# IRVLab/so_dso_place_recognition

Hardware: AMD Instinct MI355X
Metric: queries/sec over 100k-signature DB (SC 20x60, z-score fusion, top-1) (higher is better)
Workload: dtype f16x2 (fp32 carried as f16 hi + lo, fp32 accumulate); binary intensity channel: one f16 product per term, rounded to its exact integer count; 1 GPU; sc_match_100k; db_signatures=100000, descriptor=SC 20x60 x 2 channels, mask_width=0, k=1, db_rows_per_gpu=100000

## Files before the change

include/place_recognition.h:

```cpp
#ifndef PLACE_RECOGNITION_H
#define PLACE_RECOGNITION_H

#include <stdint.h>

#ifdef __cplusplus
extern "C" {
#endif

typedef struct pr_ctx pr_ctx;
typedef struct pr_sigset pr_sigset;
typedef struct pr_clouds pr_clouds;
typedef struct pr_bow_vocab pr_bow_vocab;
typedef struct pr_bow_db pr_bow_db;

enum { PR_OK = 0, PR_EINVAL = -1, PR_ENOMEM = -2, PR_EHIP = -3, PR_EIO = -4, PR_ENAN = -5 };
enum { PR_TYPE_SC = 0, PR_TYPE_M2DP = 1, PR_TYPE_DELIGHT = 2, PR_TYPE_GIST = 3, PR_TYPE_BOW = 4 };
enum { PR_ROLE_QUERY = 0, PR_ROLE_DB = 1 };
enum { PR_F64 = 0, PR_F32 = 1, PR_U8 = 2 };
enum { PR_HOST = 0, PR_DEVICE = 1 };
#define PR_F16_DISTANCE_BOUND 2e-3
#define PR_F16_SIGMA_REL 2e-4
#define PR_F16_DIST_ERR 2e-4
#define PR_F32_SIGMA_REL 5e-7
#define PR_F32_DIST_ERR 2e-7
// ... 64 lines not shown
int pr_match_topk(pr_ctx* ctx, int type, const double* h1, int32_t m, const double* h2, int32_t n,
                  int32_t mask_width, double p_weight, int32_t k, int32_t* idx, float* score);
int pr_match_topk_f64(pr_ctx* ctx, int type, const double* h1, int32_t m, const double* h2, int32_t n,
                      int32_t mask_width, double p_weight, int32_t k, int32_t* idx, double* score);

int pr_gist_distance(pr_ctx* ctx, const double* h1, int32_t m, const double* h2, int32_t n, int32_t cols, float* dist);
int pr_bow_distance(pr_ctx* ctx, const double* h1, int32_t m, const double* h2, int32_t n, int32_t cols, float* dist);
int pr_match_topk_cols(pr_ctx* ctx, int type, const double* h1, int32_t m, const double* h2, int32_t n, int32_t cols,
                       int32_t mask_width, int32_t k, int32_t* idx, float* score);

int pr_bow_db_create(pr_ctx* ctx, int32_t max_sigs, int32_t cols, int32_t n_words, int64_t max_postings, pr_bow_db** out);
void pr_bow_db_destroy(pr_ctx* ctx, pr_bow_db* db);
int pr_bow_db_set(pr_ctx* ctx, pr_bow_db* db, const double* rows, int where, int32_t n);
int pr_bow_db_append(pr_ctx* ctx, pr_bow_db* db, const double* rows, int where, int32_t n_new);
int32_t pr_bow_db_count(const pr_bow_db* db);
int pr_bow_match_topk_dev(pr_ctx* ctx, const pr_bow_db* db, const double* q, int32_t m, int32_t q_row0, int32_t db_row0,
                          int32_t mask_width, int32_t k, int32_t* idx, double* score);
int pr_bow_match_topk_f64(pr_ctx* ctx, const double* h1, int32_t m, const double* h2, int32_t n, int32_t cols,
                          int32_t mask_width, int32_t k, int32_t* idx, double* score);
int pr_bow_distance_f64(pr_ctx* ctx, const double* h1, int32_t m, const double* h2, int32_t n, int32_t cols, double* dist);

typedef struct pr_gist_db pr_gist_db;
int pr_gist_db_create(pr_ctx* ctx, int32_t max_sigs, int32_t cols, pr_gist_db** out);
void pr_gist_db_destroy(pr_ctx* ctx, pr_gist_db* db);
int pr_gist_db_set(pr_ctx* ctx, pr_gist_db* db, const double* rows, int where, int32_t n);
int pr_gist_db_append(pr_ctx* ctx, pr_gist_db* db, const double* rows, int where, int32_t n_new);
int32_t pr_gist_db_count(const pr_gist_db* db);
int64_t pr_gist_db_bytes(const pr_gist_db* db);
void pr_gist_db_set_exact(pr_gist_db* db, int on);
int pr_gist_match_topk_dev(pr_ctx* ctx, const pr_gist_db* db, const double* q, int32_t m, int32_t q_row0, int32_t db_row0,
                           int32_t mask_width, int32_t k, int32_t* idx, double* score);
int pr_gist_flagged_count(pr_ctx* ctx, int32_t m, int32_t* count);
int pr_gist_match_topk_f64(pr_ctx* ctx, const double* h1, int32_t m, const double* h2, int32_t n, int32_t cols,
                           int32_t mask_width, int32_t k, int32_t* idx, double* score);
int pr_gist_distance_f64(pr_ctx* ctx, const double* h1, int32_t m, const double* h2, int32_t n, int32_t cols, double* dist);

typedef struct pr_delight_db pr_delight_db;
int pr_delight_db_create(pr_ctx* ctx, int32_t max_sigs, pr_delight_db** out);
void pr_delight_db_destroy(pr_ctx* ctx, pr_delight_db* db);
int pr_delight_db_set(pr_ctx* ctx, pr_delight_db* db, const double* rows, int where, int32_t n);
int pr_delight_db_append(pr_ctx* ctx, pr_delight_db* db, const double* rows, int where, int32_t n_new);
int32_t pr_delight_db_count(const pr_delight_db* db);
int64_t pr_delight_db_bytes(const pr_delight_db* db);
void pr_delight_db_set_exact(pr_delight_db* db, int on);
int pr_delight_match_topk_dev(pr_ctx* ctx, const pr_delight_db* db, const double* q, int32_t m, int32_t q_row0, int32_t db_row0,
                              int32_t mask_width, int32_t k, int32_t* idx, double* score);
int pr_delight_flagged_count(pr_ctx* ctx, int32_t m, int32_t* count);
int pr_delight_match_topk_f64(pr_ctx* ctx, const double* h1, int32_t m, const double* h2, int32_t n, int32_t mask_width, int32_t k,
                              int32_t* idx, double* score);
int pr_delight_distance_f64(pr_ctx* ctx, const double* h1, int32_t m, const double* h2, int32_t n, double* dist);

int pr_match_topk_fused(pr_ctx* ctx, const double* sc1, const double* m2dp1, int32_t m, const double* sc2, const double* m2dp2,
                        int32_t n, int32_t mask_width, double p_weight, int32_t k, int32_t* idx, float* score);
int pr_match_topk_fused_f64(pr_ctx* ctx, const double* sc1, const double* m2dp1, int32_t m, const double* sc2, const double* m2dp2,
                            int32_t n, int32_t mask_width, double p_weight, int32_t k, int32_t* idx, double* score);
int pr_match_align(pr_ctx* ctx, int type, const double* h1, int32_t m, const double* h2, int32_t n, int32_t k, const int32_t* idx,
                   int32_t* variant, double* dist);
int pr_match_align_fused(pr_ctx* ctx, const double* sc1, const double* m2dp1, int32_t m, const double* sc2, const double* m2dp2,
                         int32_t n, int32_t k, const int32_t* idx, int32_t* variant, double* dist);
int pr_fuse_select2_dev(pr_ctx* ctx, const float* d_p, const float* d_i, const float* e_p, const float* e_i, int32_t m, int32_t n,
                        const double* mom_all, const double* mom2_all, int32_t G, int32_t q_row0, int32_t db_row0,
                        int32_t mask_width, double p_weight, int32_t k, int32_t* idx, float* score);


#define PR_MAX_SIGS 4000000
int pr_sigset_create(pr_ctx* ctx, int type, int role, int32_t max_sigs, pr_sigset** out);
void pr_sigset_destroy(pr_ctx* ctx, pr_sigset* s);
int pr_sigset_pack(pr_ctx* ctx, pr_sigset* s, const void* sig, int dtype, int where, int32_t n_sigs);
int32_t pr_sigset_count(const pr_sigset* s);
int pr_sigset_reserve(pr_ctx* ctx, pr_sigset* s);
int pr_sigset_append(pr_ctx* ctx, pr_sigset* s, const void* sig, int dtype, int where, int32_t n_new);
int pr_sigset_image(const pr_sigset* s, const void** image, size_t* bytes, int32_t* channel_stride_groups);

int pr_distances_dev(pr_ctx* ctx, const pr_sigset* q, const pr_sigset* db, float* d_p, float* d_i);

int pr_row_moments_dev(pr_ctx* ctx, const float* d_p, const float* d_i, int32_t m, int32_t n, double* mom);

int pr_fuse_select_dev(pr_ctx* ctx, const float* d_p, const float* d_i, int32_t m, int32_t n,
                       const double* mom_all, int32_t G, int32_t q_row0, int32_t db_row0, int32_t mask_width,
                       double p_weight, int32_t k, int32_t* idx, float* score);
int pr_fuse_select_f64_dev(pr_ctx* ctx, const float* d_p, const float* d_i, int32_t m, int32_t n,
                           const double* mom_all, int32_t G, int32_t q_row0, int32_t db_row0, int32_t mask_width,
                           double p_weight, int32_t k, int32_t* idx, float* score, double* score64);
int pr_fuse_select2_f64_dev(pr_ctx* ctx, const float* d_p, const float* d_i, const float* e_p, const float* e_i, int32_t m, int32_t n,
                            const double* mom_all, const double* mom2_all, int32_t G, int32_t q_row0, int32_t db_row0,
                            int32_t mask_width, double p_weight, int32_t k, int32_t* idx, float* score, double* score64);

int pr_rerank_width(const pr_ctx* ctx, int32_t k);
int pr_f16_margin_dev(pr_ctx* ctx, const double* mom_sc, const double* mom_m2, int32_t m, int32_t G, double p_weight, int32_t k_in,
                      const double* cand_score, int32_t k, const double* score, int32_t* flags, int32_t* count);
int pr_rerank_dev(pr_ctx* ctx, const void* q_sc, const void* db_sc, int sc_dtype, const void* q_m2, const void* db_m2, int m2_dtype,
                  const double* mom_sc, const double* mom_m2, int32_t m, int32_t n_local, int32_t G, int32_t q_row0, int32_t db_row0,
                  int32_t mask_width, double p_weight, int32_t k_in, const int32_t* idx_in, const double* score_in, int32_t k, int32_t* idx,
                  double* score);
int pr_rerank_partial_dev(pr_ctx* ctx, const void* q_sc, const void* db_sc, int sc_dtype, const void* q_m2, const void* db_m2, int m2_dtype,
                          const double* mom_sc, const double* mom_m2, int32_t m, int32_t n_local, int32_t G, int32_t q_row0, int32_t db_row0,
                          int32_t mask_width, double p_weight, int32_t k_in, const int32_t* cand_idx, const double* cand_score, int32_t k,
                          double* p5);
int pr_rerank_finish_dev(pr_ctx* ctx, const double* mom_sc, const double* mom_m2, int32_t G_mom, const int32_t* cand_idx, const double* cand_score,
                         const double* p5_all, int32_t G, int32_t m, int32_t k_in, int32_t k, double p_weight, int32_t* idx, double* score);
int pr_order_resolve_async_dev(pr_ctx* ctx, const void* q_sc, const void* db_sc, int sc_dtype, const void* q_m2, const void* db_m2, int m2_dtype,
                               double* mom_sc, double* mom_m2, int32_t m, int32_t n, int32_t q_row0, int32_t mask_width, double p_weight,
                               int32_t k, int32_t* idx, double* score);
int pr_order_resolve_dev(pr_ctx* ctx, const void* q_sc, const void* db_sc, int sc_dtype, const void* q_m2, const void* db_m2, int m2_dtype,
                         double* mom_sc, double* mom_m2, int32_t m, int32_t n, int32_t q_row0, int32_t mask_width, double p_weight, int32_t k,
                         int32_t* idx, double* score, int32_t* resolved);
int pr_order_flagged_count(pr_ctx* ctx, int32_t m, int32_t* count);
int pr_order_exact_moments_dev(pr_ctx* ctx, const void* q_sc, const void* db_sc, int sc_dtype, const void* q_m2, const void* db_m2, int m2_dtype,
                               const double* mom_sc, const double* mom_m2, int32_t G_mom, int32_t m, int32_t n_local, int32_t offset,
                               int32_t last_pass , double* exact);
int pr_order_exact_select_dev(pr_ctx* ctx, const double* exact_all, int32_t G, int32_t m, int32_t n_local, int32_t q_row0, int32_t db_row0,
                              int32_t mask_width, double p_weight, int has_sc, int has_m2, int32_t k, int32_t offset, double* sel);
int pr_order_exact_merge_dev(pr_ctx* ctx, const double* sel_all, int32_t G, int32_t m, int32_t k, int32_t offset, int32_t* idx, double* score);
int pr_widen_scores_dev(pr_ctx* ctx, const float* score32, int64_t count, double* score64);
int pr_merge_topk_dev(pr_ctx* ctx, const int32_t* idx_all, const double* score_all, int32_t G, int32_t m, int32_t k,
                      int32_t* idx, double* score);
int pr_align_pairs_dev(pr_ctx* ctx, const void* q_sc, const void* db_sc, int sc_dtype, const void* q_m2, const void* db_m2, int m2_dtype,
                       int32_t m, int32_t n_local, int32_t db_row0, int32_t k, const int32_t* idx, int32_t* variant, double* dist);
int pr_delight_align_pairs_dev(pr_ctx* ctx, const void* q, const void* db, int dtype, int32_t m, int32_t n_local, int32_t db_row0, int32_t k,
                               const int32_t* idx, int32_t* variant, double* dist);

typedef struct pr_group pr_group;
int pr_group_create(const int32_t* device_ids, int32_t G, pr_group** out);
void pr_group_destroy(pr_group* g);
const char* pr_group_last_error(const pr_group* g);
int32_t pr_group_size(const pr_group* g);
int pr_group_uses_rccl(const pr_group* g);
int32_t pr_group_rccl_ranks(const pr_group* g);
int pr_group_set_exact_statistics(pr_group* g, int on);
int32_t pr_group_last_flagged(const pr_group* g);
#define PR_GROUP_PHASES 10
int pr_group_set_timing(pr_group* g, int on);
int pr_group_last_timing(pr_group* g, float* ms, int32_t cap);
int pr_group_set_database(pr_group* g, int type, const double* h2, int32_t n);
int pr_group_set_database_growable(pr_group* g, int type, const double* h2, int32_t n, int32_t extra_capacity);
int pr_group_append_database(pr_group* g, const double* hist_new, int32_t n_new);
int32_t pr_group_database_rows(const pr_group* g);
int pr_group_take_warnings(pr_group* g);
int pr_group_match_topk(pr_group* g, const double* h1, int32_t m, int32_t mask_width, double p_weight, int32_t k, int32_t* idx,
                        double* score);

int pr_sc_generate_dev(pr_ctx* ctx, const double* xyz, const float* inten, const int64_t* offs, int32_t N,
                       double max_rho, double* out);
int pr_m2dp_generate_dev(pr_ctx* ctx, const double* xyz, const float* inten, const int64_t* offs, int32_t N,
                         double max_rho, double* out);
int pr_delight_generate_dev(pr_ctx* ctx, const double* xyz, const float* inten, const int64_t* offs, int32_t N, double* out);
int pr_cloud_frames_dev(pr_ctx* ctx, const double* xyz, const float* inten , const int64_t* offs, int32_t N, double* frames);
int pr_sc_generate_frames_dev(pr_ctx* ctx, const double* xyz, const float* inten, const int64_t* offs, int32_t N, double max_rho,
                              const double* frames, int frames_have_ave, double* out);
int pr_m2dp_generate_frames_dev(pr_ctx* ctx, const double* xyz, const float* inten, const int64_t* offs, int32_t N, double max_rho,
                                const double* frames, int frames_have_ave, double* out);
int pr_delight_generate_frames_dev(pr_ctx* ctx, const double* xyz, const float* inten, const int64_t* offs, int32_t N,
                                   const double* frames, double* out);

int pr_sc_relative_pose(const double* frames_q, const double* frames_db, const int32_t* variant, int32_t c, double* T);

int pr_pts_preprocess(const char* poses_file, const char* pts_file, const char* incoming_id_file, double lidarRange,
                      int polar_filter, int verbose, pr_clouds** out);
int pr_pts_preprocess_gpu(pr_ctx* ctx, const char* poses_file, const char* pts_file, const char* incoming_id_file,
                          double lidarRange, int polar, int verbose, pr_clouds** out);
int pr_hash_order(const int32_t* keys, int32_t K, int32_t* order);
int64_t pr_clouds_count(const pr_clouds* c);
const int64_t* pr_clouds_offs(const pr_clouds* c);
const double* pr_clouds_xyz(const pr_clouds* c);
const float* pr_clouds_inten(const pr_clouds* c);
const int32_t* pr_clouds_ids(const pr_clouds* c);
// ... 191 lines not shown
```

so_dso_place_recognition_amd/_lib.py:

```python
from __future__ import annotations

import ctypes as C
import os

PR_OK, PR_EINVAL, PR_ENOMEM, PR_EHIP, PR_EIO, PR_ENAN = 0, -1, -2, -3, -4, -5
TYPE_SC, TYPE_M2DP, TYPE_DELIGHT, TYPE_GIST, TYPE_BOW = 0, 1, 2, 3, 4
SC_ARITH_F16X2, SC_ARITH_F32, SC_ARITH_F16 = 0, 1, 2
NAN_EXCLUDE, NAN_FAIL = 0, 1
WARN_NAN_ROWS, WARN_M2DP_SVD, WARN_F16_FALLBACK, WARN_ORDER_RESOLVED, WARN_ORDER_UNRESOLVED = 1, 2, 4, 8, 16
WARN_BOW_TRUNCATED = 32
WARN_BOW_ROWS = 64
ROLE_QUERY, ROLE_DB = 0, 1
F64, F32 = 0, 1
U8 = 2
HOST, DEVICE = 0, 1
ICP_CONVERGED, ICP_MAX_ITER, ICP_TOO_FEW, ICP_DEGENERATE, ICP_NO_PAIR = 0, 1, 2, 3, 4
ICP_SEARCH_BRUTE, ICP_SEARCH_GRID = 0, 1
POSE_SC, POSE_M2DP, POSE_DELIGHT = 0, 1, 2
WINDOW_OVERFLOW, WINDOW_ORDER_GLOBAL = 1, 2
MAP_OVERFLOW, MAP_DROPPED = 1, 2
ONLINE_OVERFLOW = 1
ONLINE_NB = 512
ONLINESET_FUSED, ONLINESET_DELIGHT = 0, 1
ONLINESET_NB_FUSED, ONLINESET_NB_DELIGHT = 512, 64
# ... 48 lines not shown
    "pr_group_last_flagged": (_i32, [_vp]),
    "pr_group_set_exact_statistics": (C.c_int, [_vp, C.c_int]),
    "pr_group_set_timing": (C.c_int, [_vp, C.c_int]),
    "pr_group_last_timing": (C.c_int, [_vp, _vp, _i32]),
    "pr_group_set_database": (C.c_int, [_vp, C.c_int, _vp, _i32]),
    "pr_group_set_database_growable": (C.c_int, [_vp, C.c_int, _vp, _i32, _i32]),
    "pr_group_append_database": (C.c_int, [_vp, _vp, _i32]),
    "pr_group_database_rows": (_i32, [_vp]),
    "pr_group_take_warnings": (C.c_int, [_vp]),
    "pr_group_match_topk": (C.c_int, [_vp, _vp, _i32, _i32, _dbl, _i32, _vp, _vp]),
    "pr_destroy": (None, [_vp]),
    "pr_last_error": (C.c_char_p, [_vp]),
    "pr_version": (C.c_char_p, []),
    "pr_set_sc_arith": (C.c_int, [_vp, C.c_int]),
    "pr_get_sc_arith": (C.c_int, [_vp]),
    "pr_sync": (C.c_int, [_vp]),
    "pr_stream": (_vp, [_vp]),
    "pr_sc_generate": (C.c_int, [_vp, _vp, _vp, _vp, _i32, _dbl, _vp]),
    "pr_m2dp_generate": (C.c_int, [_vp, _vp, _vp, _vp, _i32, _dbl, _vp]),
    "pr_m2dp_svd_rows": (C.c_int, [_vp, _vp, _i32, _vp]),
    "pr_delight_generate": (C.c_int, [_vp, _vp, _vp, _vp, _i32, _vp]),
    "pr_gist_signature_size": (C.c_int, [_i32, _i32, _vp]),
    "pr_gist_generate": (C.c_int, [_vp, _vp, C.c_int, _i32, _i32, _i32, _i32, _i32, _vp, _vp]),
    "pr_gist_generate_dev": (C.c_int, [_vp, _vp, C.c_int, _i32, _i32, _i32, _i32, _i32, _vp, _vp]),
    "pr_bow_vocab_load": (C.c_int, [C.c_char_p, C.POINTER(_vp)]),
    "pr_bow_vocab_save_bin": (C.c_int, [_vp, C.c_char_p]),
    "pr_bow_vocab_create": (C.c_int, [_i32, _i32, _i32, _i32, C.c_int64, _vp, _vp, _vp, _vp, C.POINTER(_vp)]),
    "pr_bow_vocab_info": (C.c_int, [_vp, _vp, C.POINTER(C.c_int64), C.POINTER(C.c_int64)]),
    "pr_bow_vocab_export": (C.c_int, [_vp, _vp, _vp, _vp, _vp]),
    "pr_bow_vocab_destroy": (None, [_vp]),
    "pr_bow_generate": (C.c_int, [_vp, _vp, _vp, _vp, _i32, _i32, _vp, _vp]),
    "pr_bow_generate_dev": (C.c_int, [_vp, _vp, _vp, C.c_int64, _vp, _i32, _i32, _vp, _vp, _vp]),
    "pr_delight_distance": (C.c_int, [_vp, _vp, _i32, _vp, _i32, _vp]),
    "pr_gist_distance": (C.c_int, [_vp, _vp, _i32, _vp, _i32, _i32, _vp]),
    "pr_bow_distance": (C.c_int, [_vp, _vp, _i32, _vp, _i32, _i32, _vp]),
    "pr_match_topk_fused": (C.c_int, [_vp, _vp, _vp, _i32, _vp, _vp, _i32, _i32, _dbl, _i32, _vp, _vp]),
    "pr_fuse_select2_dev": (C.c_int, [_vp, _vp, _vp, _vp, _vp, _i32, _i32, _vp, _vp, _i32, _i32, _i32, _i32, _dbl, _i32, _vp, _vp]),
    "pr_fuse_select2_f64_dev": (C.c_int, [_vp, _vp, _vp, _vp, _vp, _i32, _i32, _vp, _vp, _i32, _i32, _i32, _i32, _dbl, _i32, _vp, _vp, _vp]),
    "pr_fuse_select_f64_dev": (C.c_int, [_vp, _vp, _vp, _i32, _i32, _vp, _i32, _i32, _i32, _i32, _dbl, _i32, _vp, _vp, _vp]),
    "pr_match_topk_cols": (C.c_int, [_vp, C.c_int, _vp, _i32, _vp, _i32, _i32, _i32, _i32, _vp, _vp]),
    "pr_bow_db_create": (C.c_int, [_vp, _i32, _i32, _i32, C.c_int64, C.POINTER(_vp)]),
    "pr_bow_db_destroy": (None, [_vp, _vp]),
    "pr_bow_db_set": (C.c_int, [_vp, _vp, _vp, C.c_int, _i32]),
    "pr_bow_db_append": (C.c_int, [_vp, _vp, _vp, C.c_int, _i32]),
    "pr_bow_db_count": (_i32, [_vp]),
    "pr_bow_match_topk_dev": (C.c_int, [_vp, _vp, _vp, _i32, _i32, _i32, _i32, _i32, _vp, _vp]),
    "pr_bow_match_topk_f64": (C.c_int, [_vp, _vp, _i32, _vp, _i32, _i32, _i32, _i32, _vp, _vp]),
    "pr_bow_distance_f64": (C.c_int, [_vp, _vp, _i32, _vp, _i32, _i32, _vp]),
    "pr_gist_db_create": (C.c_int, [_vp, _i32, _i32, C.POINTER(_vp)]),
    "pr_gist_db_destroy": (None, [_vp, _vp]),
    "pr_gist_db_set": (C.c_int, [_vp, _vp, _vp, C.c_int, _i32]),
    "pr_gist_db_append": (C.c_int, [_vp, _vp, _vp, C.c_int, _i32]),
    "pr_gist_db_count": (_i32, [_vp]),
    "pr_gist_db_bytes": (C.c_int64, [_vp]),
    "pr_gist_db_set_exact": (None, [_vp, C.c_int]),
    "pr_gist_match_topk_dev": (C.c_int, [_vp, _vp, _vp, _i32, _i32, _i32, _i32, _i32, _vp, _vp]),
    "pr_gist_flagged_count": (C.c_int, [_vp, _i32, C.POINTER(_i32)]),
    "pr_gist_match_topk_f64": (C.c_int, [_vp, _vp, _i32, _vp, _i32, _i32, _i32, _i32, _vp, _vp]),
    "pr_gist_distance_f64": (C.c_int, [_vp, _vp, _i32, _vp, _i32, _i32, _vp]),
    "pr_delight_db_create": (C.c_int, [_vp, _i32, C.POINTER(_vp)]),
    "pr_delight_db_destroy": (None, [_vp, _vp]),
    "pr_delight_db_set": (C.c_int, [_vp, _vp, _vp, C.c_int, _i32]),
    "pr_delight_db_append": (C.c_int, [_vp, _vp, _vp, C.c_int, _i32]),
    "pr_delight_db_count": (_i32, [_vp]),
    "pr_delight_db_bytes": (C.c_int64, [_vp]),
    "pr_delight_db_set_exact": (None, [_vp, C.c_int]),
    "pr_delight_match_topk_dev": (C.c_int, [_vp, _vp, _vp, _i32, _i32, _i32, _i32, _i32, _vp, _vp]),
    "pr_delight_flagged_count": (C.c_int, [_vp, _i32, C.POINTER(_i32)]),
    "pr_delight_match_topk_f64": (C.c_int, [_vp, _vp, _i32, _vp, _i32, _i32, _i32, _vp, _vp]),
    "pr_delight_distance_f64": (C.c_int, [_vp, _vp, _i32, _vp, _i32, _vp]),
    "pr_delight_generate_dev": (C.c_int, [_vp, _vp, _vp, _vp, _i32, _vp]),
    "pr_sc_distance": (C.c_int, [_vp, _vp, _i32, _vp, _i32, _vp, _vp]),
    "pr_m2dp_distance": (C.c_int, [_vp, _vp, _i32, _vp, _i32, _vp, _vp]),
    "pr_match_topk": (C.c_int, [_vp, C.c_int, _vp, _i32, _vp, _i32, _i32, _dbl, _i32, _vp, _vp]),
    "pr_sigset_create": (C.c_int, [_vp, C.c_int, C.c_int, _i32, C.POINTER(_vp)]),
    "pr_sigset_destroy": (None, [_vp, _vp]),
    "pr_sigset_pack": (C.c_int, [_vp, _vp, _vp, C.c_int, C.c_int, _i32]),
    "pr_sigset_count": (_i32, [_vp]),
    "pr_sigset_reserve": (C.c_int, [_vp, _vp]),
    "pr_sigset_append": (C.c_int, [_vp, _vp, _vp, C.c_int, C.c_int, _i32]),
    "pr_sigset_image": (C.c_int, [_vp, C.POINTER(_vp), C.POINTER(C.c_size_t), C.POINTER(_i32)]),
    "pr_distances_dev": (C.c_int, [_vp, _vp, _vp, _vp, _vp]),
    "pr_row_moments_dev": (C.c_int, [_vp, _vp, _vp, _i32, _i32, _vp]),
    "pr_fuse_select_dev": (C.c_int, [_vp, _vp, _vp, _i32, _i32, _vp, _i32, _i32, _i32, _i32, _dbl, _i32, _vp, _vp]),
    "pr_sc_generate_dev": (C.c_int, [_vp, _vp, _vp, _vp, _i32, _dbl, _vp]),
    "pr_m2dp_generate_dev": (C.c_int, [_vp, _vp, _vp, _vp, _i32, _dbl, _vp]),
    "pr_cloud_frames_dev": (C.c_int, [_vp, _vp, _vp, _vp, _i32, _vp]),
    "pr_sc_generate_frames_dev": (C.c_int, [_vp, _vp, _vp, _vp, _i32, _dbl, _vp, C.c_int, _vp]),
    "pr_m2dp_generate_frames_dev": (C.c_int, [_vp, _vp, _vp, _vp, _i32, _dbl, _vp, C.c_int, _vp]),
    "pr_delight_generate_frames_dev": (C.c_int, [_vp, _vp, _vp, _vp, _i32, _vp, _vp]),
    "pr_generate_clouds": (C.c_int, [_vp, C.c_int, _vp, _dbl, _vp]),
    "pr_clouds_dev_xyz": (_vp, [_vp]),
    "pr_clouds_dev_inten": (_vp, [_vp]),
    "pr_clouds_dev_offs": (_vp, [_vp]),
    "pr_clouds_dev_frames": (_vp, [_vp]),
    "pr_pts_preprocess": (C.c_int, [C.c_char_p, C.c_char_p, C.c_char_p, _dbl, C.c_int, C.c_int, C.POINTER(_vp)]),
    "pr_pts_preprocess_gpu": (C.c_int, [_vp, C.c_char_p, C.c_char_p, C.c_char_p, _dbl, C.c_int, C.c_int, C.POINTER(_vp)]),
    "pr_hash_order": (C.c_int, [_vp, _i32, _vp]),
    "pr_window_create": (C.c_int, [_vp, _dbl, C.c_int, _i32, _i32, _i32, C.POINTER(_vp)]),
    "pr_window_destroy": (None, [_vp]),
    "pr_window_reset": (C.c_int, [_vp]),
    "pr_window_count": (C.c_int, [_vp, C.POINTER(_i32)]),
    "pr_window_push_dev": (C.c_int, [_vp, _vp, _vp, _vp, _vp, _i32, _vp, _vp, _vp, _vp, _vp]),
    "pr_window_push": (C.c_int, [_vp, _vp, _vp, _vp, _i32, _vp, _vp, C.POINTER(_i32), _vp, _vp]),
    "pr_clouds_avg_ms": (C.c_double, [_vp]),
    "pr_clouds_avg_pts": (C.c_double, [_vp]),
    "pr_clouds_count": (C.c_int64, [_vp]),
    "pr_clouds_offs": (C.POINTER(C.c_int64), [_vp]),
    "pr_clouds_xyz": (C.POINTER(C.c_double), [_vp]),
    "pr_clouds_inten": (C.POINTER(C.c_float), [_vp]),
    "pr_clouds_ids": (C.POINTER(C.c_int32), [_vp]),
    "pr_clouds_free": (None, [_vp]),
    "pr_write_signatures": (C.c_int, [C.c_char_p, _vp, C.c_int64, C.c_int64]),
    "pr_read_signatures": (C.c_int, [C.c_char_p, C.POINTER(_vp), C.POINTER(C.c_int64), C.POINTER(C.c_int64)]),
    "pr_free": (None, [_vp]),
    "pr_write_signatures_bin": (C.c_int, [C.c_char_p, _vp, C.c_int64, C.c_int64, C.c_int]),
    "pr_read_signatures_bin": (C.c_int, [C.c_char_p, C.POINTER(_vp), C.POINTER(C.c_int64), C.POINTER(C.c_int64)]),
    "pr_write_poses": (C.c_int, [C.c_char_p, _vp, _vp, C.c_int64]),
    "pr_write_points": (C.c_int, [C.c_char_p, _vp, _vp, _vp, C.c_int64]),
    "pr_precision_recall": (C.c_int, [_vp, _vp, _i32, _vp, _vp, _i32, _i32, _dbl, _i32, C.POINTER(_dbl), C.POINTER(_dbl), _vp,
                                      C.POINTER(_i32)]),
    "pr_ground_truth_pairs_dev": (C.c_int, [_vp, _vp, _i32, _vp, _i32, _i32, _dbl, _i32, _vp, _vp, _vp, _vp]),
    "pr_precision_recall_dev": (C.c_int, [_vp, _vp, _vp, _i32, _i32, _vp, _vp, _i32, _i32, _dbl, _i32, _vp, _vp, _vp, _vp, _vp]),
    "pr_trapz_dev": (C.c_int, [_vp, _vp, _vp, _i32, _vp]),
    "pr_ground_truth_pairs": (C.c_int, [_vp, _vp, _i32, _vp, _i32, _i32, _dbl, _i32, _vp, _vp, _vp, _vp]),
    "pr_precision_recall_gpu": (C.c_int, [_vp, _vp, _vp, _i32, _vp, _vp, _i32, _i32, _dbl, _i32, C.POINTER(_dbl), C.POINTER(_dbl), _vp,
                                          C.POINTER(_i32), _vp, C.POINTER(_i32), _vp, _vp]),
    "pr_eval_tile_rows": (_i32, []),
    "pr_set_eval_path": (C.c_int, [_vp, C.c_int, C.c_int]),
    "pr_icp_nn_dev": (C.c_int, [_vp, _vp, _vp, _i32, _vp, _vp, _i32, _vp, _vp, _i32, _vp, _i32, _i32, _vp, _vp, _vp]),
    "pr_icp_pairs_dev": (C.c_int, [_vp, _vp, _vp, _i32, _vp, _vp, _i32, _vp, _vp, _i32, _vp, _i32, _i32, _i32, _dbl, _dbl, _dbl, _i32, _vp, _vp]),
    "pr_icp_nn": (C.c_int, [_vp, _vp, _vp, _i32, _vp, _vp, _i32, _vp, _vp, _i32, _vp, _vp, _vp, _vp]),
    "pr_icp_pairs": (C.c_int, [_vp, _vp, _vp, _i32, _vp, _vp, _i32, _vp, _vp, _i32, _vp, _i32, _dbl, _dbl, _dbl, _i32, _vp, _vp]),
    "pr_icp_tile_rows": (_i32, []),
    "pr_set_icp_path": (C.c_int, [_vp, C.c_int]),
    "pr_set_icp_search": (C.c_int, [_vp, C.c_int]),
    "pr_get_icp_search": (C.c_int, [_vp]),
    "pr_icp_nn_radius_dev": (C.c_int, [_vp, _vp, _vp, _i32, _vp, _vp, _i32, _vp, _vp, _i32, _vp, _i32, _i32, _dbl, _vp, _vp, _vp]),
    "pr_icp_nn_radius": (C.c_int, [_vp, _vp, _vp, _i32, _vp, _vp, _i32, _vp, _vp, _i32, _vp, _dbl, _vp, _vp, _vp]),
    "pr_relative_pose": (C.c_int, [C.c_int, _vp, _vp, _vp, _i32, _vp]),
    "pr_relative_pose_dev": (C.c_int, [_vp, C.c_int, _vp, _i32, _vp, _i32, _i32, _i32, _vp, _vp, _i32, _i32, _vp, _vp, _vp]),
    "pr_verify_select_dev": (C.c_int, [_vp, _vp, _vp, _i32, _i32, _dbl, _dbl, _vp, _vp, _vp, _vp]),
    "pr_verify_pairs_dev": (C.c_int, [_vp, C.c_int, _vp, _vp, _i32, _vp, _vp, _i32, _vp, _vp, _i32, _i32, _i32, _i32, _vp, _vp, _i32, _i32, _i32, _i32,
                                      _i32, _dbl, _dbl, _dbl, _i32, _dbl, _dbl, _vp, _vp, _vp, _vp]),
    "pr_map_create": (C.c_int, [_vp, _vp, _i32, C.c_int64, _i32, _i32, C.POINTER(_vp)]),
    "pr_map_destroy": (None, [_vp]),
    "pr_map_reset": (C.c_int, [_vp]),
    "pr_map_count": (C.c_int, [_vp, C.POINTER(_i32), C.POINTER(C.c_int64), C.POINTER(_i32)]),
    "pr_map_append_dev": (C.c_int, [_vp, _vp, _vp, _vp, _vp, _vp, _vp, _vp, _i32, C.c_int64, _vp]),
    "pr_map_append": (C.c_int, [_vp, _vp, _vp, _vp, _vp, _vp, _vp, _vp, _i32, _vp]),
    "pr_map_verify_dev": (C.c_int, [_vp, C.c_int, _vp, _vp, _i32, _vp, _i32, _i32, _vp, _vp, _i32, _i32, _i32, _i32, _dbl, _dbl, _dbl, _i32, _dbl,
                                    _dbl, _vp, _vp, _vp, _vp]),
    "pr_online_create": (C.c_int, [_vp, C.c_int, _vp, _i32, _i32, C.POINTER(_vp)]),
    "pr_online_destroy": (None, [_vp]),
    "pr_online_reset": (C.c_int, [_vp]),
    "pr_online_count": (C.c_int, [_vp, C.POINTER(_i32), C.POINTER(_i32)]),
    "pr_online_match_dev": (C.c_int, [_vp, _vp, _vp, _i32, _dbl, _i32, _vp, _vp, _vp]),
    "pr_online_append_dev": (C.c_int, [_vp, _vp, _vp, _vp]),
    "pr_online_append": (C.c_int, [_vp, _vp, _vp]),
    "pr_onlineset_create": (C.c_int, [_vp, C.c_int, _vp, _i32, _i32, C.POINTER(_vp)]),
    "pr_onlineset_destroy": (None, [_vp]),
    "pr_onlineset_reset": (C.c_int, [_vp]),
    "pr_onlineset_count": (C.c_int, [_vp, C.POINTER(_i32), C.POINTER(_i32)]),
    "pr_onlineset_match_dev": (C.c_int, [_vp, _vp, _vp, _vp, _vp, _i32, _dbl, _i32, _vp, _vp, _vp]),
    "pr_onlineset_append_dev": (C.c_int, [_vp, _vp, _vp, _vp, _vp, _vp]),
    "pr_onlineset_append": (C.c_int, [_vp, _vp, _vp, _vp, _vp]),
# ... 110 lines not shown
```

so_dso_place_recognition_amd/csrc/fuse_select.hip:

```cpp
#include <cstdlib>

#include "div_rn.hpp"
#include "kernels.hpp"

namespace pr {
namespace {

typedef float f32x4 __attribute__((ext_vector_type(4)));

__device__ __forceinline__ double block_sum(double v, double* red, int tid) {
  red[tid] = v;
  __syncthreads();
  for (int s = 128; s > 0; s >>= 1) {
    if (tid < s) red[tid] += red[tid + s];
    __syncthreads();
  }
  double r = red[0];
  __syncthreads();
  return r;
}

__global__ __launch_bounds__(256) void row_moments_kernel(const float* __restrict__ d_p, const float* __restrict__ d_i,
                                                           int n, double* __restrict__ mom) {
  __shared__ double red[256];
  const int tid = threadIdx.x, q = blockIdx.x;
  for (int ch = 0; ch < 2; ch++) {
    const float* row = (ch ? d_i : d_p) + (size_t)q * n;
    const float r0 = row[0];
    const double c = (r0 == r0) ? (double)r0 : 0.5;
    double s1 = 0.0, s2 = 0.0, cnt = 0.0;
    auto acc = [&](float v) { if (v == v) { const double d = (double)v - c; s1 += d; s2 += d * d; cnt += 1.0; } };
    int head = (int)((4 - ((reinterpret_cast<size_t>(row) >> 2) & 3)) & 3);
    if (head > n) head = n;
    const int nv = (n - head) >> 2;
    if (tid < head) acc(row[tid]);
    const f32x4* rv4 = reinterpret_cast<const f32x4*>(row + head);
    int j = tid;
    for (; j + 768 < nv; j += 1024) {
      const f32x4 a = rv4[j], b = rv4[j + 256], c4 = rv4[j + 512], d4 = rv4[j + 768];
      acc(a[0]); acc(a[1]); acc(a[2]); acc(a[3]);
      acc(b[0]); acc(b[1]); acc(b[2]); acc(b[3]);
      acc(c4[0]); acc(c4[1]); acc(c4[2]); acc(c4[3]);
      acc(d4[0]); acc(d4[1]); acc(d4[2]); acc(d4[3]);
    }
    for (; j < nv; j += 256) { const f32x4 a = rv4[j]; acc(a[0]); acc(a[1]); acc(a[2]); acc(a[3]); }
    for (int t = head + 4 * nv + tid; t < n; t += 256) acc(row[t]);
    const double S1 = block_sum(s1, red, tid);
    const double S2 = block_sum(s2, red, tid);
    const double N = block_sum(cnt, red, tid);
    if (tid == 0) {
      double* o = mom + ((size_t)q * 2 + ch) * 3;
      o[0] = N;
      o[1] = N > 0.0 ? c + S1 / N : 0.0;
      o[2] = N > 0.0 ? S2 - S1 * S1 / N : 0.0;
    }
  }
}

__global__ __launch_bounds__(256) void row_moments_slice_kernel(const float* __restrict__ d_p, const float* __restrict__ d_i, int n, int m, int P,
                                                                 double* __restrict__ part ) {
  __shared__ double red[6][256];
  const int tid = threadIdx.x, q = blockIdx.x, sl = blockIdx.y;
  const int c0 = (int)((long long)n * sl / P), c1 = (int)((long long)n * (sl + 1) / P);
  const float* rp = d_p + (size_t)q * n;
  const float* ri = d_i + (size_t)q * n;
  const float p0 = rp[0], i0 = ri[0];
  const double cp = (p0 == p0) ? (double)p0 : 0.5, ci = (i0 == i0) ? (double)i0 : 0.5;
  double s[6] = {0.0, 0.0, 0.0, 0.0, 0.0, 0.0};
  auto acc = [&](float v, double c, int o) { if (v == v) { const double d = (double)v - c; s[o] += d; s[o + 1] += d * d; s[o + 2] += 1.0; } };
  int j = c0 + tid;
  for (; j + 768 < c1; j += 1024) {
    const float a0 = rp[j], a1 = rp[j + 256], a2 = rp[j + 512], a3 = rp[j + 768];
    const float b0 = ri[j], b1 = ri[j + 256], b2 = ri[j + 512], b3 = ri[j + 768];
    acc(a0, cp, 0); acc(a1, cp, 0); acc(a2, cp, 0); acc(a3, cp, 0);
    acc(b0, ci, 3); acc(b1, ci, 3); acc(b2, ci, 3); acc(b3, ci, 3);
  }
  for (; j < c1; j += 256) { acc(rp[j], cp, 0); acc(ri[j], ci, 3); }
#pragma unroll
  for (int o = 0; o < 6; o++) red[o][tid] = s[o];
  __syncthreads();
  for (int st = 128; st > 0; st >>= 1) {
    if (tid < st) {
#pragma unroll
      for (int o = 0; o < 6; o++) red[o][tid] += red[o][tid + st];
    }
    __syncthreads();
  }
  if (tid < 2) {
    double* o = part + (((size_t)sl * m + q) * 2 + tid) * 3;
    o[0] = red[3 * tid + 2][0]; o[1] = red[3 * tid][0]; o[2] = red[3 * tid + 1][0];
  }
}
__global__ __launch_bounds__(64) void moments_finish_kernel(const float* __restrict__ d_p, const float* __restrict__ d_i, int n, int m, int P,
                                                             const double* __restrict__ part, double* __restrict__ mom) {
  const int t = blockIdx.x * 64 + threadIdx.x;
  if (t >= 2 * m) return;
  const int q = t >> 1, ch = t & 1;
  const float r0 = ((ch ? d_i : d_p) + (size_t)q * n)[0];
  const double c = (r0 == r0) ? (double)r0 : 0.5;
  double N = 0.0, S1 = 0.0, S2 = 0.0;
  const size_t step = (size_t)m * 6;
  const double* o = part + ((size_t)q * 2 + ch) * 3;
  int sl = 0;
  for (; sl + 8 <= P; sl += 8) {
    double a[8][3];
#pragma unroll
    for (int u = 0; u < 8; u++) { a[u][0] = o[(sl + u) * step]; a[u][1] = o[(sl + u) * step + 1]; a[u][2] = o[(sl + u) * step + 2]; }
#pragma unroll
    for (int u = 0; u < 8; u++) { N += a[u][0]; S1 += a[u][1]; S2 += a[u][2]; }
  }
  for (; sl < P; sl++) { N += o[sl * step]; S1 += o[sl * step + 1]; S2 += o[sl * step + 2]; }
  double* w = mom + ((size_t)q * 2 + ch) * 3;
  w[0] = N;
  w[1] = N > 0.0 ? c + S1 / N : 0.0;
  w[2] = N > 0.0 ? S2 - S1 * S1 / N : 0.0;
}

__device__ __forceinline__ bool cand_less(double av, int aj, double bv, int bj) {
  return av < bv || (av == bv && aj < bj);
}

__device__ __forceinline__ void block_argmin(double* rv, int* rj, int tid) {
  double v = rv[tid];
  int j = rj[tid];
#pragma unroll
  for (int s = 32; s > 0; s >>= 1) {
    const double ov = __shfl_xor(v, s, 64);
    const int oj = __shfl_xor(j, s, 64);
    if (oj >= 0 && (j < 0 || cand_less(ov, oj, v, j))) { v = ov; j = oj; }
  }
  __syncthreads();
  if ((tid & 63) == 0) { rv[tid >> 6] = v; rj[tid >> 6] = j; }
  __syncthreads();
  if (tid == 0) {
    for (int w = 1; w < 4; w++) {
      const int oj = rj[w];
      if (oj >= 0 && (j < 0 || cand_less(rv[w], oj, v, j))) { v = rv[w]; j = oj; }
    }
// ... 17 lines not shown
    unsigned long long prefix = 0ull;
    int krem = k, below_total = 0, shd = -1;
    for (int d = 0; d < 8 && shd < 0; d++) {
      const int sh = 56 - 8 * d;
      hist[tid] = 0u;
      __syncthreads();
      for (int s = tid; s < L; s += 256) {
        const unsigned long long key = order_key((double)lv[s]);
        if (d == 0 || (key >> (sh + 8)) == prefix) atomicAdd(&hist[(key >> sh) & 255ull], 1u);
      }
      __syncthreads();
      if (tid < 64) {
        const unsigned c0 = hist[4 * tid], c1 = hist[4 * tid + 1], c2 = hist[4 * tid + 2], c3 = hist[4 * tid + 3];
        const unsigned own = (c0 + c1) + (c2 + c3);
        unsigned incl = own;
#pragma unroll
        for (int o = 1; o < 64; o <<= 1) {
          const unsigned up = __shfl_up(incl, o, 64);
          if (tid >= o) incl += up;
        }
        const unsigned excl = incl - own;
        if (excl < (unsigned)krem && (unsigned)krem <= incl) {
          unsigned b = excl;
          int bin = 4 * tid;
          unsigned cb = c0;
          if (b + c0 < (unsigned)krem) { b += c0; bin++; cb = c1;
            if (b + c1 < (unsigned)krem) { b += c1; bin++; cb = c2;
              if (b + c2 < (unsigned)krem) { b += c2; bin++; cb = c3; } } }
          ctl[0] = bin; ctl[1] = (int)b; ctl[2] = (int)cb;
        }
      }
      __syncthreads();
      prefix = (prefix << 8) | (unsigned long long)ctl[0];
      below_total += ctl[1];
      krem -= ctl[1];
      if (below_total + ctl[2] <= 256) shd = sh;
      __syncthreads();
    }
    if (shd < 0) return false;
    if (tid == 0) ctl[3] = 0;
    __syncthreads();
    for (int s = tid; s < L; s += 256) {
      const double v = (double)lv[s];
      if ((order_key(v) >> shd) <= prefix) {
        const int slot = atomicAdd(&ctl[3], 1);
        rv[slot] = v; rj[slot] = lj[s];
      }
    }
    __syncthreads();
    C = ctl[3];
  } else {
    if (tid < L) { rv[tid] = (double)lv[tid]; rj[tid] = lj[tid]; }
  }
  if (tid >= C) { rv[tid] = __builtin_inf(); rj[tid] = NONE_J; }
  __syncthreads();
  for (int size = 2; size <= 256; size <<= 1)
    for (int stride = size >> 1; stride > 0; stride >>= 1) {
      if (tid < 128) {
        const int pos = 2 * tid - (tid & (stride - 1)), par = pos + stride;
        const bool up = (pos & size) == 0;
        const double a = rv[pos], b = rv[par];
        const int aj = rj[pos], bj = rj[par];
        if (cand_less(b, bj, a, aj) == up) { rv[pos] = b; rj[pos] = bj; rv[par] = a; rj[par] = aj; }
      }
      __syncthreads();
    }
  return true;
}

template <int CAP>
struct SelLds {
  double st[8];
  double rv[256];
  int rj[256];
  double lv[CAP];
  int lj[CAP];
  int lcnt;
  unsigned hist[256];
  int ctl[4];
  double tau_s;
  int last;
};

template <int CAP>
__device__ __forceinline__ void select_row(const float* __restrict__ d_p, const float* __restrict__ d_i,
                                           const float* __restrict__ e_p, const float* __restrict__ e_i,
                                           const double* __restrict__ mom2_all,
                                           int m, int n, const double* __restrict__ mom_all, int G,
                                           int q_row0, int db_row0, int mask_width, double p_weight,
                                           int k, int32_t* __restrict__ idx, float* __restrict__ score, int P,
                                           double* __restrict__ score64, SelLds<CAP>& W) {
  double* st = W.st;
  double* rv = W.rv;
  int* rj = W.rj;
  double* lv = W.lv;
  int* lj = W.lj;
  int& lcnt = W.lcnt;
  unsigned* hist = W.hist;
  int* ctl = W.ctl;
  const int tid = threadIdx.x, q = blockIdx.x;
  const bool plain = (d_i == nullptr);
  const bool two = (e_p != nullptr);
  if (!plain && tid < (two ? 4 : 2)) {
    double cn = 0.0, mean = 0.0, m2 = 0.0;
    for (int g = 0; g < G; g++) {
      const double* o = (tid < 2 ? mom_all : mom2_all) + (((size_t)g * m + q) * 2 + (tid & 1)) * 3;
      const double nb = o[0], mb = o[1], m2b = o[2];
      if (nb <= 0.0) continue;
      const double tot = cn + nb, delta = mb - mean;
      mean += delta * (nb / tot);
      m2 += m2b + delta * delta * (cn * nb / tot);
      cn = tot;
    }
    st[tid * 2] = mean;
    st[tid * 2 + 1] = sqrt(m2 / (cn - 1.0));
  }
  if (tid == 0) lcnt = 0;
  __syncthreads();
  const double mp = plain ? 0.0 : st[0], sp = plain ? 1.0 : st[1], mi = plain ? 0.0 : st[2], si = plain ? 1.0 : st[3];
  const int n_row = n;
  if (P > 1) {
    const int c0 = (int)((long long)n_row * blockIdx.y / P), c1 = (int)((long long)n_row * (blockIdx.y + 1) / P);
    const size_t ro = (size_t)q * n_row + c0;
    d_p += ro - (size_t)q * (c1 - c0);
    if (d_i) d_i += ro - (size_t)q * (c1 - c0);
    if (e_p) { e_p += ro - (size_t)q * (c1 - c0); e_i += ro - (size_t)q * (c1 - c0); }
    db_row0 += c0;
    n = c1 - c0;
    idx += (size_t)blockIdx.y * m * k;
    score += (size_t)blockIdx.y * m * k;
  }
  const float* rp = d_p + (size_t)q * n;
  const float* ri = plain ? rp : d_i + (size_t)q * n;
  const int ig = q_row0 + q;
  const bool fastdiv = !plain && sp > 1e-290 && sp < 1e290 && si > 1e-290 && si < 1e290;
  const double rsp = 1.0 / sp, rsi = 1.0 / si;
  const bool fastdiv2 = two && st[5] > 1e-290 && st[5] < 1e290 && st[7] > 1e-290 && st[7] < 1e290;
  const double m2p = two ? st[4] : 0.0, s2p = two ? st[5] : 1.0, m2i = two ? st[6] : 0.0, s2i = two ? st[7] : 1.0;
  const double rs2p = 1.0 / s2p, rs2i = 1.0 / s2i;
  int head = (int)((4 - ((reinterpret_cast<size_t>(rp) >> 2) & 3)) & 3);
  if (head > n) head = n;
  const bool coaligned = !((reinterpret_cast<size_t>(rp) ^ reinterpret_cast<size_t>(ri)) & 15) &&
                         !(e_p && (((reinterpret_cast<size_t>(rp) ^ reinterpret_cast<size_t>(e_p + (size_t)q * n)) |
                                    (reinterpret_cast<size_t>(rp) ^ reinterpret_cast<size_t>(e_i + (size_t)q * n))) & 15));
  if (!coaligned) head = 0;
  const int nv = coaligned ? (n - head) >> 2 : 0;
  const f32x4* rp4 = reinterpret_cast<const f32x4*>(rp + head);
  const f32x4* ri4 = reinterpret_cast<const f32x4*>(ri + head);

  const float* rep = two ? e_p + (size_t)q * n : rp;
  const float* rei = two ? e_i + (size_t)q * n : rp;
  auto fused4 = [&](float vp, float vi, float wp, float wi, int j) -> double {
    const int jg = db_row0 + j;
    double f;
    if (plain) f = (double)vp;
    else if (fastdiv) f = p_weight * div_rn((double)vp - mp, sp, rsp) + div_rn((double)vi - mi, si, rsi);
    else f = p_weight * (((double)vp - mp) / sp) + ((double)vi - mi) / si;
    if (two) {
      const double xp = (double)wp - m2p, xi = (double)wi - m2i;
      f += fastdiv2 ? p_weight * div_rn(xp, s2p, rs2p) + div_rn(xi, s2i, rs2i) : p_weight * (xp / s2p) + xi / s2i;
    }
    int dij = ig - jg;
    if (dij < 0) dij = -dij;
    if (dij < mask_width) f = __builtin_inf();
    return f;
  };
  auto fused = [&](float vp, float vi, int j) -> double { return fused4(vp, vi, two ? rep[j] : 0.f, two ? rei[j] : 0.f, j); };
  const f32x4* ep4 = reinterpret_cast<const f32x4*>(rep + head);
  const f32x4* ei4 = reinterpret_cast<const f32x4*>(rei + head);
  auto sweep_if = [&](auto&& maybe, auto&& visit) {
    if (tid < head && maybe(rp[tid], ri[tid], two ? rep[tid] : 0.f, two ? rei[tid] : 0.f)) visit(tid, fused(rp[tid], ri[tid], tid));
    const f32x4 z4 = {0.f, 0.f, 0.f, 0.f};
    auto four = [&](const f32x4& a, const f32x4& b, const f32x4& c, const f32x4& d, int j) {
      const int j0 = head + 4 * j;
#pragma unroll
      for (int e = 0; e < 4; e++)
        if (maybe(a[e], b[e], c[e], d[e])) visit(j0 + e, fused4(a[e], b[e], c[e], d[e], j0 + e));
    };
    int j = tid;
    if (two) {
      for (; j + 768 < nv; j += 1024) {
        const f32x4 a0 = rp4[j], a1 = rp4[j + 256], a2 = rp4[j + 512], a3 = rp4[j + 768];
        const f32x4 b0 = ri4[j], b1 = ri4[j + 256], b2 = ri4[j + 512], b3 = ri4[j + 768];
        const f32x4 c0 = ep4[j], c1 = ep4[j + 256], c2 = ep4[j + 512], c3 = ep4[j + 768];
        const f32x4 d0 = ei4[j], d1 = ei4[j + 256], d2 = ei4[j + 512], d3 = ei4[j + 768];
        four(a0, b0, c0, d0, j); four(a1, b1, c1, d1, j + 256); four(a2, b2, c2, d2, j + 512); four(a3, b3, c3, d3, j + 768);
// ... 45 lines not shown
    double mv = 0.0;
    int mj = -1;
    const int r = k + 7 > 16 ? k + 7 : 16;
    long long want = (long long)n * r / 1024;
    const int ns = (int)(want < 4096 ? (n < 4096 ? n : 4096) : (want < n ? want : n));
    auto take = [&](float vp, float vi, int j) {
      const double f = fused(vp, vi, j);
      const int jg = db_row0 + j;
      if (f == f && (mj < 0 || cand_less(f, jg, mv, mj))) { mv = f; mj = jg; }
    };
    int j = tid;
    for (; j + 768 < ns; j += 1024) {
      const float p0 = rp[j], p1 = rp[j + 256], p2 = rp[j + 512], p3 = rp[j + 768];
      const float i0 = ri[j], i1 = ri[j + 256], i2 = ri[j + 512], i3 = ri[j + 768];
      take(p0, i0, j); take(p1, i1, j + 256); take(p2, i2, j + 512); take(p3, i3, j + 768);
    }
    for (; j < ns; j += 256) take(rp[j], ri[j], j);
    rv[tid] = mv; rj[tid] = mj;
    __syncthreads();
    int before = 0;
    for (int u = 0; u < 256; u++) {
      const int oj = rj[u];
      if (oj >= 0 && (mj < 0 || cand_less(rv[u], oj, mv, mj))) before++;
    }
    if (tid == 0) W.tau_s = __builtin_inf();
    __syncthreads();
    if (mj >= 0 && before == r - 1) W.tau_s = mv;
    __syncthreads();
    tau = W.tau_s;
  }
  const bool whole = n <= CAP && !(tau < __builtin_inf());
  if (whole)
    sweep([&](int j, double f) {
      const bool ok = f == f;
      lv[j] = ok ? f : __builtin_inf();
      lj[j] = ok ? db_row0 + j : NONE_J;
    });
  else {
    const bool pre = !plain && fastdiv && (!two || fastdiv2) && tau < __builtin_inf();
    const double a1 = p_weight / sp, b1 = 1.0 / si, c1 = -(p_weight * mp / sp + mi / si);
    const double a2 = two ? p_weight / s2p : 0.0, b2 = two ? 1.0 / s2i : 0.0, c2 = two ? -(p_weight * m2p / s2p + m2i / s2i) : 0.0;
    const double tauE = tau + 1e-10 * (1.0 + fabs(a1) + fabs(b1) + fabs(c1) + fabs(a2) + fabs(b2) + fabs(c2) + fabs(tau));
    auto collect = [&](int j, double f) {
      if (f <= tau) {
        const int slot = atomicAdd(&lcnt, 1);
        if (slot < CAP) { lv[slot] = f; lj[slot] = db_row0 + j; }
      }
    };
    if (pre)
      sweep_if([&](float vp, float vi, float wp, float wi) {
        double fa = __builtin_fma(a1, (double)vp, __builtin_fma(b1, (double)vi, c1));
        if (two) fa += __builtin_fma(a2, (double)wp, __builtin_fma(b2, (double)wi, c2));
        return fa <= tauE;
      }, collect);
    else
      sweep(collect);
  }
  __syncthreads();
  const int L = whole ? n : lcnt;
  if (L <= CAP && (k > 12 || whole)) {
    if (k <= 249 && list_topk(lv, lj, L, k, rv, rj, hist, ctl, tid)) {
      for (int t = tid; t < k; t += 256) emit(t, rv[t], rj[t] == NONE_J ? -1 : rj[t]);
      return;
    }
    int N = 2;
    while (N < L) N <<= 1;
    for (int s = L + tid; s < N; s += 256) { lv[s] = __builtin_inf(); lj[s] = NONE_J; }
    __syncthreads();
    for (int size = 2; size <= N; size <<= 1)
      for (int stride = size >> 1; stride > 0; stride >>= 1) {
        for (int i = tid; i < (N >> 1); i += 256) {
          const int pos = 2 * i - (i & (stride - 1)), par = pos + stride;
          const bool up = (pos & size) == 0;
          const double a = lv[pos], b = lv[par];
          const int aj = lj[pos], bj2 = lj[par];
          if (cand_less(b, bj2, a, aj) == up) { lv[pos] = b; lj[pos] = bj2; lv[par] = a; lj[par] = aj; }
        }
        __syncthreads();
      }
    for (int t = tid; t < k; t += 256) emit(t, lv[t < L ? t : 0], (t < L && lj[t] != NONE_J) ? lj[t] : -1);
    return;
  }
  if (L <= CAP) {
    for (int t = 0; t < k; t++) {
      double cv = 0.0;
      int cj = -1, cs = -1;
      for (int s = tid; s < L; s += 256)
        if (lj[s] >= 0 && (cj < 0 || cand_less(lv[s], lj[s], cv, cj))) { cv = lv[s]; cj = lj[s]; cs = s; }
      rv[tid] = cv; rj[tid] = cj;
      block_argmin(rv, rj, tid);
      const double wv = rv[0];
      const int wj = rj[0];
      __syncthreads();
      if (cs >= 0 && cj == wj) lj[cs] = -1;
      if (tid == 0) emit(t, wv, wj);
      if (wj < 0) {
        if (tid == 0) for (int u = t + 1; u < k; u++) emit(u, 0.0, -1);
        break;
      }
      __syncthreads();
    }
    return;
  }
  double pv = -__builtin_inf(), bv = 0.0;
  int pj = -1, bj = -1;
  for (int t = 0; t < k; t++) {
    bv = 0.0; bj = -1;
    sweep([&](int j, double f) {
      const int jg = db_row0 + j;
      if (f != f) return;
      if (!cand_less(pv, pj, f, jg)) return;
      if (bj < 0 || cand_less(f, jg, bv, bj)) { bv = f; bj = jg; }
    });
    rv[tid] = bv; rj[tid] = bj;
    block_argmin(rv, rj, tid);
    pv = rv[0];
    pj = rj[0];
    __syncthreads();
    if (tid == 0) emit(t, pv, pj);
    if (pj < 0) {
      if (tid == 0) for (int u = t + 1; u < k; u++) emit(u, 0.0, -1);
      break;
    }
  }
}

constexpr int WS_CAP = 1024;
__device__ __forceinline__ void wave_argmin(double& v, int& j) {
#pragma unroll
  for (int s2 = 32; s2 > 0; s2 >>= 1) {
    const double ov = __shfl_xor(v, s2, 64);
    const int oj = __shfl_xor(j, s2, 64);
    if (oj >= 0 && (j < 0 || cand_less(ov, oj, v, j))) { v = ov; j = oj; }
  }
}
__global__ __launch_bounds__(256) void fuse_select_wave_kernel(const float* __restrict__ d_p, const float* __restrict__ d_i, int m, int n,
                                                                const double* __restrict__ mom_all, int G, int q_row0, int db_row0,
                                                                int mask_width, double p_weight, int k, int32_t* __restrict__ idx,
                                                                float* __restrict__ score, double* __restrict__ score64) {
  __shared__ double lv_[4][WS_CAP];
  __shared__ int lj_[4][WS_CAP];
  const int lane = threadIdx.x & 63, w = threadIdx.x >> 6;
  const int q = blockIdx.x * 4 + w;
  if (q >= m) return;
  double* lv = lv_[w];
  int* lj = lj_[w];
  const bool plain = (d_i == nullptr);
  double st0 = 0.0, st1 = 1.0;
  if (!plain && lane < 2) {
    double cn = 0.0, mean = 0.0, m2 = 0.0;
    for (int g = 0; g < G; g++) {
      const double* o = mom_all + (((size_t)g * m + q) * 2 + lane) * 3;
      const double nb = o[0], mb = o[1], m2b = o[2];
      if (nb <= 0.0) continue;
      const double tot = cn + nb, delta = mb - mean;
      mean += delta * (nb / tot);
      m2 += m2b + delta * delta * (cn * nb / tot);
      cn = tot;
    }
    st0 = mean;
    st1 = sqrt(m2 / (cn - 1.0));
  }
  const double mp = plain ? 0.0 : __shfl(st0, 0, 64), sp = plain ? 1.0 : __shfl(st1, 0, 64);
  const double mi = plain ? 0.0 : __shfl(st0, 1, 64), si = plain ? 1.0 : __shfl(st1, 1, 64);
  const float* rp = d_p + (size_t)q * n;
  const float* ri = plain ? rp : d_i + (size_t)q * n;
  const int ig = q_row0 + q;
  const bool fastdiv = !plain && sp > 1e-290 && sp < 1e290 && si > 1e-290 && si < 1e290;
  const double rsp = 1.0 / sp, rsi = 1.0 / si;
  auto fusedw = [&](float vp, float vi, int j) -> double {
    const int jg = db_row0 + j;
    double f;
    if (plain) f = (double)vp;
    else if (fastdiv) f = p_weight * div_rn((double)vp - mp, sp, rsp) + div_rn((double)vi - mi, si, rsi);
    else f = p_weight * (((double)vp - mp) / sp) + ((double)vi - mi) / si;
    int dij = ig - jg;
    if (dij < 0) dij = -dij;
    if (dij < mask_width) f = __builtin_inf();
    return f;
  };
  auto emit = [&](int t, double v, int jg) {
    idx[(size_t)q * k + t] = jg;
    const float f32 = (jg >= 0) ? (float)v : __builtin_nanf("");
    score[(size_t)q * k + t] = f32;
// ... 105 lines not shown
    });
    wave_argmin(bv, bj);
    if (lane == 0) emit(t, bv, bj);
    if (bj < 0) {
      if (lane == 0) for (int u = t + 1; u < k; u++) emit(u, 0.0, -1);
      break;
    }
    pv = bv; pj = bj;
  }
}

__device__ void merge_slices(const int32_t* sidx, const float* sscore, int P, int m, int k, int q, float* lv, int* lj, double* rv, int* rj,
                             unsigned* hist, int* ctl, int32_t* __restrict__ idx, float* __restrict__ score, double* __restrict__ score64,
                             int tid) {
  const int T = P * k;
  int N = 2;
  while (N < T) N <<= 1;
  for (int s = tid; s < N; s += 256) {
    int j = -1;
    float v = 0.f;
    if (s < T) {
      const size_t o = ((size_t)(s / k) * m + q) * k + (s % k);
      j = sidx[o]; v = sscore[o];
    }
    const bool ok = j >= 0 && v == v;
    lv[s] = ok ? v : __builtin_inff();
    lj[s] = ok ? j : NONE_J;
  }
  __syncthreads();
  auto put = [&](int t, bool ok, float v, int j) {
    idx[(size_t)q * k + t] = ok ? j : -1;
    const float f32 = ok ? v : __builtin_nanf("");
    score[(size_t)q * k + t] = f32;
    if (score64) score64[(size_t)q * k + t] = (double)f32;
  };
  if (k <= 249 && list_topk(lv, lj, T, k, rv, rj, hist, ctl, tid)) {
    for (int t = tid; t < k; t += 256) put(t, rj[t] != NONE_J, (float)rv[t], rj[t]);
    return;
  }
  for (int size = 2; size <= N; size <<= 1)
    for (int stride = size >> 1; stride > 0; stride >>= 1) {
      for (int i = tid; i < (N >> 1); i += 256) {
        const int pos = 2 * i - (i & (stride - 1)), par = pos + stride;
        const bool up = (pos & size) == 0;
        const float a = lv[pos], b = lv[par];
        const int aj = lj[pos], bj = lj[par];
        if (cand_less((double)b, bj, (double)a, aj) == up) { lv[pos] = b; lj[pos] = bj; lv[par] = a; lj[par] = aj; }
      }
      __syncthreads();
    }
  for (int t = tid; t < k; t += 256) put(t, lj[t] != NONE_J, lv[t], lj[t]);
}

__global__ __launch_bounds__(256) void slice_merge_kernel(const int32_t* __restrict__ sidx, const float* __restrict__ sscore, int P, int m, int k,
                                                           int32_t* __restrict__ idx, float* __restrict__ score, double* __restrict__ score64) {
  extern __shared__ __attribute__((aligned(8))) char smem[];
  int N = 2;
  while (N < P * k) N <<= 1;
  __shared__ double rv[256];
  __shared__ int rj[256];
  __shared__ unsigned hist[256];
  __shared__ int ctl[4];
  merge_slices(sidx, sscore, P, m, k, blockIdx.x, reinterpret_cast<float*>(smem), reinterpret_cast<int*>(smem) + N, rv, rj, hist, ctl, idx, score,
                      score64, threadIdx.x);
}

template <int CAP>
#ifdef FS_NOLB
#define FS_BOUNDS __launch_bounds__(256)
#else
#define FS_BOUNDS __launch_bounds__(256, 3)
#endif
__global__ FS_BOUNDS void fuse_select_kernel(const float* __restrict__ d_p, const float* __restrict__ d_i,
                                                           const float* __restrict__ e_p, const float* __restrict__ e_i,
                                                           const double* __restrict__ mom2_all,
                                                           int m, int n, const double* __restrict__ mom_all, int G,
                                                           int q_row0, int db_row0, int mask_width, double p_weight,
                                                           int k, int32_t* __restrict__ idx, float* __restrict__ score, int P,
                                                           double* __restrict__ score64) {
  __shared__ SelLds<CAP> L;
  select_row<CAP>(d_p, d_i, e_p, e_i, mom2_all, m, n, mom_all, G, q_row0, db_row0, mask_width, p_weight, k, idx, score, P, score64, L);
}

}

int select_slices(int m, int n) {
  if (m > 64 || n < 16384) return 1;
  static const int forced = getenv("PR_SLICE_COLS") ? atoi(getenv("PR_SLICE_COLS")) : 0;
  const int cols = forced > 0 ? forced : (m <= 8 ? FS_CAP / 2 : FS_CAP);
  int P = (n + cols - 1) / cols;
  if (P > 64) P = 64;
  while (P > 1 && m * P > 1024) P >>= 1;
  return P;
}
size_t select_scratch_bytes() { return (size_t)64 * 16 * 128 * 8 + (size_t)64 * 16 * 6 * 8; }

void launch_row_moments(hipStream_t st, const float* d_p, const float* d_i, int m, int n, double* mom, void* scratch) {
  if (m <= 0) return;
  const int P = scratch ? select_slices(m, n) : 1;
  if (P > 1) {
    double* part = reinterpret_cast<double*>(static_cast<char*>(scratch) + (size_t)64 * 16 * 128 * 8);
    hipLaunchKernelGGL(row_moments_slice_kernel, dim3(m, P), dim3(256), 0, st, d_p, d_i, n, m, P, part);
    hipLaunchKernelGGL(moments_finish_kernel, dim3((2 * m + 63) / 64), dim3(64), 0, st, d_p, d_i, n, m, P, part, mom);
    return;
  }
  hipLaunchKernelGGL(row_moments_kernel, dim3(m), dim3(256), 0, st, d_p, d_i, n, mom);
}

void launch_fuse_select(hipStream_t st, const float* d_p, const float* d_i, int m, int n, const double* mom_all,
                        int G, int q_row0, int db_row0, int mask_width, double p_weight, int k, int32_t* idx,
                        float* score, const float* e_p, const float* e_i, const double* mom2_all, void* scratch, double* score64) {
  if (m <= 0) return;
  int P = (scratch && k <= 128) ? select_slices(m, n) : 1;
  if ((size_t)P * m * k > (size_t)64 * 16 * 128) P = 1;
  if (P > 1) {
    int32_t* sidx = static_cast<int32_t*>(scratch);
    float* ssc = reinterpret_cast<float*>(sidx + (size_t)64 * 16 * 128);
    int N = 2;
    while (N < P * k) N <<= 1;
    hipLaunchKernelGGL(fuse_select_kernel<FS_CAP>, dim3(m, P), dim3(256), 0, st, d_p, d_i, e_p, e_i, mom2_all, m, n, mom_all, G, q_row0, db_row0,
                       mask_width, p_weight, k, sidx, ssc, P, nullptr);
    if ((size_t)N * 8 > 40 * 1024)
      (void)hipFuncSetAttribute(reinterpret_cast<const void*>(slice_merge_kernel), hipFuncAttributeMaxDynamicSharedMemorySize, (int)((size_t)N * 8));
    hipLaunchKernelGGL(slice_merge_kernel, dim3(m), dim3(256), (size_t)N * 8, st, sidx, ssc, P, m, k, idx, score, score64);
    return;
  }
  static const bool wave_rows = !(getenv("PR_SELECT_WAVE") && atoi(getenv("PR_SELECT_WAVE")) == 0);
  static const int wave_max_n = getenv("PR_SELECT_WAVE_N") ? atoi(getenv("PR_SELECT_WAVE_N")) : 32768;
  if (wave_rows && !e_p && n <= wave_max_n && k <= 16 && m >= 64) {
    hipLaunchKernelGGL(fuse_select_wave_kernel, dim3((m + 3) / 4), dim3(256), 0, st, d_p, d_i, m, n, mom_all, G, q_row0, db_row0, mask_width,
                       p_weight, k, idx, score, score64);
    return;
  }
  hipLaunchKernelGGL(fuse_select_kernel<FS_CAP>, dim3(m), dim3(256), 0, st, d_p, d_i, e_p, e_i, mom2_all, m, n, mom_all, G, q_row0, db_row0,
                     mask_width, p_weight, k, idx, score, 1, score64);
}

}
```

so_dso_place_recognition_amd/csrc/kernels.hpp:

```cpp
#pragma once
#include <hip/hip_runtime.h>
#include <stdint.h>

struct pr_ctx;

namespace pr {

constexpr int SC_NF = 31;
constexpr int SC_NSLOT = 16;
constexpr int SC_QIMG = SC_NF * 320;
constexpr int SC_DSTEP = 640;
constexpr int SC_DIMG = 2 * SC_NSLOT * SC_DSTEP;
__host__ __device__ inline int sc_fpos(int f) { return f == 0 ? 0 : (f == 30 ? 1 : f + 1); }
constexpr int SCH_QROW = 80;
constexpr int SCH_QBLK = 16 * SCH_QROW;
constexpr int SCH_QIMG = SC_NF * SCH_QBLK;
__host__ __device__ constexpr int sch_qrow_pos(int row) { return (int)((0xedbafc9865327410ull >> (4 * row)) & 15); }
__host__ __device__ constexpr int sch_qrow_byte(int row) { return SCH_QROW * sch_qrow_pos(row); }
static_assert(SCH_QROW % 16 == 0 && SCH_QBLK % 16 == 0 && SCH_QIMG % 16 == 0, "ds_read_b128 needs 16-byte aligned query tiles");
constexpr int SCH_DTILE = 768;
constexpr int SCH_DFREQ = 4 * SCH_DTILE;
constexpr int SCH_DIMG = SC_NF * SCH_DFREQ;
__host__ __device__ constexpr int sch_qlo_byte(int ring) { return 40 + ((ring + 4) % 20) * 2; }
__host__ __device__ constexpr int sch_a1_byte(int k) { return k == 3 ? 0 : 16 * k; }
__host__ __device__ constexpr int sch_a2_byte(int k) { return k == 0 ? 48 : k == 1 ? 64 : k == 2 ? 32 : 16; }
__host__ __device__ constexpr int sch_b1_byte(int lane) { return lane < 48 ? lane * 16 : SCH_DTILE + (lane - 48) * 16; }
__host__ __device__ constexpr int sch_b2_byte(int lane) { return lane < 32 ? lane * 16 : lane < 48 ? SCH_DTILE + lane * 16 : SCH_DTILE + (lane - 32) * 16; }
constexpr int SCF_QBLK = 640;
constexpr int SCF_QIMG = SC_NF * SCF_QBLK;
constexpr int SCF_DFREQ = 2 * SCH_DTILE;
constexpr int SCF_DIMG = SC_NF * SCF_DFREQ;
constexpr int M2_TILE = 96 * 64;

inline int sc_qgroups8(int m) { return ((m + 31) / 32) * 4; }
inline int sc_qgroups8_f16(int m) { return ((m + 63) / 64) * 8; }
inline int sc_dgroups(int n) { return (n + 15) / 16; }
inline int m2_tiles(int sigs) { return (sigs + 7) / 8; }
inline int m2_qtiles(int sigs) { return ((m2_tiles(sigs) + 11) / 12) * 12; }

constexpr int SC_BSTAT_INTS = 8;
struct ScBin {
  const int* qstat; const int* dstat;
  const float* qinfo; const float* dinfo;
  int* viol;
  int gen;
  float bconst;
  float pair_scale;
  int gate;
  int chsel;
};
#ifdef __HIPCC__
__device__ __forceinline__ bool sc_bin_bound(const ScBin& b, float& bound) {
  const int q0 = b.qstat[0], q1 = b.qstat[1], d0 = b.dstat[0], d1 = b.dstat[1];
  const float eq = __builtin_sqrtf(((__int_as_float(b.qstat[2]) + __int_as_float(b.qstat[3])) + __int_as_float(b.qstat[4])) + __int_as_float(b.qstat[5]));
  const float ed = __builtin_sqrtf(((__int_as_float(b.dstat[2]) + __int_as_float(b.dstat[3])) + __int_as_float(b.dstat[4])) + __int_as_float(b.dstat[5]));
  bound = (eq + ed + eq * ed + b.bconst * (1.f + eq) * (1.f + ed)) * 1.001f;
  return q0 == 0 && d0 == 0 && bound * __builtin_sqrtf((float)q1 * (float)d1) < 0.72f;
}
#endif
void launch_sc_pack(hipStream_t st, const void* sig, int dtype, int rows, int role, float* packed, int groups,
                    const double* twiddle, int* flags, int* bad);
void launch_sc_match(hipStream_t st, const float* qpk, int m, const float* dpk, int n, const float* cst,
                     float* d_p, float* d_i, int nsplit_override);
size_t sc_match_lds_bytes();
void launch_zero_ints(hipStream_t st, int* p, int n);
void launch_fill_ints(hipStream_t st, int* p, int n, int v);
void launch_sc_pack_h(hipStream_t st, const void* sig, int dtype, int rows, int role, void* packed, int groups,
                      const double* twiddle, int* flags, int* bad, int single = 0,
                      float* binfo = nullptr, int* bstat = nullptr);
void launch_sc_pack_h_rows(hipStream_t st, const void* sig, int dtype, int rows, int row0, void* packed, int groups, const double* twiddle,
                           int* flags, int* bad, int single, float* binfo, int* bstat);
void launch_sc_match_h(hipStream_t st, const void* qpk, int m, const void* dpk, int n, const void* cst, float* d_p,
                       float* d_i, int nsplit_override, const struct ScBin* bin = nullptr);
size_t sc_match_h_lds_bytes();
void launch_sc_match_e(hipStream_t st, const void* qpk, int m, const void* dpk, int n, const void* cst, float* d_p, float* d_i,
                       int nsplit_override, int single, int dgs = 0 );
void launch_sc_match_e_bin(hipStream_t st, const void* qpk, int m, const void* dpk, int n, const void* cst, float* d_p, float* d_i,
                           int nsplit_override, ScBin bin, hipEvent_t* ev, int online_h = 0 , int dgs = 0 );

void launch_m2dp_pack(hipStream_t st, const void* sig, int dtype, int sigs, float* packed, int tiles);
void launch_m2dp_match(hipStream_t st, const float* qpk, int m, const float* dpk, int n, float* d_p, float* d_i);
void launch_m2dp_pack_h(hipStream_t st, const void* sig, int dtype, int sigs, void* packed, int tiles, int sg0 = 0 );
void launch_m2dp_match_h(hipStream_t st, const void* qpk, int m, const void* dpk, int n, float* d_p, float* d_i, int single = 0 ,
                         int dts = 0 );

size_t select_scratch_bytes();
void launch_row_moments(hipStream_t st, const float* d_p, const float* d_i, int m, int n, double* mom, void* scratch = nullptr);
void launch_fuse_select(hipStream_t st, const float* d_p, const float* d_i, int m, int n, const double* mom_all,
                        int G, int q_row0, int db_row0, int mask_width, double p_weight, int k, int32_t* idx,
                        float* score, const float* e_p = nullptr, const float* e_i = nullptr, const double* mom2_all = nullptr, void* scratch = nullptr,
                        double* score64 = nullptr );

void launch_nan_fixup(hipStream_t st, float* d_p, float* d_i, int m, int n, const int* qbad, const int* dbad);
void launch_rerank(hipStream_t st, const void* q_sc, const void* db_sc, int sc_dt, const void* q_m2, const void* db_m2, int m2_dt,
                   const double* mom_sc, const double* mom_m2, int m, int n_local, int G, int q_row0, int db_row0, int mask_width,
                   double p_weight, int kin, const int32_t* idx_in, double* p5, unsigned* tick , size_t tick_cap , int k, int32_t* idx, double* score,
                   float* score32, const double* cand_sc32, double eps_d = 0.0, double order_floor = 0.0,
                   double order_noise = 0.0, int32_t* order_flags = nullptr);
void launch_rerank_partial(hipStream_t st, const void* q_sc, const void* db_sc, int sc_dt, const void* q_m2, const void* db_m2, int m2_dt,
                           const double* mom_sc, const double* mom_m2, int m, int n_local, int G, int q_row0, int db_row0, int mask_width,
                           double p_weight, int kin, const int32_t* idx_in, double* p5, unsigned* tick, size_t tick_cap, const double* cand_sc32, int k,
                           double eps_d = 0.0);
void launch_margin_check(hipStream_t st, const double* mom_sc, const double* mom_m2, int G, int m, double p_weight, int kin,
                         const double* cand_sc, int k, const double* score, double eps_d, int32_t* flags, int32_t* count,
                         const int32_t* order_flags, double eps_floor, double noise );
void launch_order_check(hipStream_t st, const double* mom_sc, const double* mom_m2, int Gmom, const int32_t* cand_idx, const double* p5_all,
                        int G, int m, int kin, int k, const int32_t* idx_sel, double p_weight, double eps_floor, double noise, int32_t* flags,
                        const double* cand_sc = nullptr, const double* score_sel = nullptr);
constexpr int RESOLVE_SLOTS = 64;
constexpr int RESOLVE_NB = 2048;
constexpr int RESOLVE_SMALL_M = 1024;
int exact_partial_blocks(int n_local);
void launch_flag_compact(hipStream_t st, const int32_t* flags, int m, int32_t* list, int32_t* cnt);
void launch_xrow(hipStream_t st, const void* q_sc, const void* db_sc, int sc_dt, const void* q_m2, const void* db_m2, int m2_dt,
                 const double* mom_sc, const double* mom_m2, int G, int m, int n_local, const int32_t* flags, int32_t* list, int32_t* cnt,
                 int offset, bool compacted, double* partial, double* exact, double* rows, unsigned* tick, int* dflags,
                 int last_pass , double* qspec , const double* tw ,
                 int direct );
size_t xrow_qspec_doubles();
hipError_t xrow_set_twiddles(const double* cos60, const double* sin60);
void launch_xrow_select(hipStream_t st, const int32_t* flags, const int32_t* list, const int32_t* cnt, int offset, const double* exact_all, int G,
                        int m, int n_local, int q_row0, int db_row0, int mask_width, double p_weight, int has_sc, int has_m2, int k,
                        const double* rows, double* part , double* sel, int32_t* idx,
                        double* score, double* out_mom_sc, double* out_mom_m2);
size_t xrow_select_part_doubles(int m, int k);
void launch_xrow_merge(hipStream_t st, const int32_t* flags, const int32_t* list, const int32_t* cnt, int offset, const double* sel_all, int G, int m,
                       int k, int32_t* idx, double* score);
void launch_rerank_finish(hipStream_t st, const int32_t* cand_idx, const double* p5_all, int G, int m, int kin, int k, int32_t* idx,
                          double* score);
void launch_widen(hipStream_t st, const float* a, long long n, double* b);
void launch_merge_topk(hipStream_t st, const int32_t* idx_all, const double* score_all, int G, int m, int k, int32_t* idx, double* score);

void launch_align(hipStream_t st, const void* q_sc, const void* db_sc, int sc_dt, const void* q_m2, const void* db_m2, int m2_dt, int m,
                  int n_local, int db_row0, int k, const int32_t* idx, int32_t* variant , double* dist );
void launch_delight_align(hipStream_t st, const void* q, const void* db, int dt, int m, int n_local, int db_row0, int k, const int32_t* idx,
                          int32_t* variant , double* dist );

void launch_ave_chain(hipStream_t st, const float* inten, const int64_t* offs, int N, float* ave ,
                      double* frames = nullptr );
void launch_cloud_frames(hipStream_t st, const double* xyz, const int64_t* offs, int N, double* frames);
constexpr int SC_MAX_W = 16;
constexpr int SC_MAX_SPLIT_CLOUDS = 1024;
constexpr size_t SC_SCRATCH_PER_STREAM = (size_t)2 * SC_MAX_SPLIT_CLOUDS * 4 + (size_t)SC_MAX_SPLIT_CLOUDS * SC_MAX_W * 9 * 8 +
                                         (size_t)768 * (1200 * 4 + 3 * 1200 * 8);
size_t sc_generate_scratch_bytes();
void launch_sc_batch(hipStream_t st, const double* xyz, const float* inten, const int64_t* offs, int c0, int c1, int W, double max_rho,
                     double* frames, char* scratch, double* out);
size_t sc_cluster_scratch_bytes(int ncl, int CW);
int sc_cluster_points_per_workgroup();
int* launch_sc_cluster(hipStream_t st, const double* xyz, const float* inten, const int64_t* offs, int N, double max_rho, int CW, int ncu,
                       char* scratch, double* frames, double* out);
void launch_sc_finish(hipStream_t st, const float* ave, int N, double* out);
void launch_sc_bin(hipStream_t st, const double* xyz, const float* inten, const int64_t* offs, int N, double max_rho,
                   const double* frames, const float* ave , double* out,
                   int ave_in_frames = 0 );
void launch_m2dp_bin_svd(hipStream_t st, const double* xyz, const float* inten, const int64_t* offs, int N,
                         double max_rho, const double* frames, const float* ave, const double* planes, double* mats,
                         double* out, int* flags ,
                         int* svd_rows ,
                         hipStream_t st2 = nullptr, hipEvent_t* ev_bin = nullptr, hipEvent_t* ev_svd = nullptr );
constexpr int M2DP_SVD_ROWS_CAP = 1024;
constexpr double M2DP_SVD_TIE_TRACE = 1.001;
size_t m2dp_generate_scratch_bytes(int N);

void launch_gist_distance(hipStream_t st, const double* h1, int m, const double* h2, int n, int cols, float* dist);
void launch_bow_distance(hipStream_t st, const double* h1, int m, const double* h2, int n, int cols, float* dist);
void launch_delight_gen(hipStream_t st, const double* xyz, const float* inten, const int64_t* offs, int N,
                        const double* frames, double* out);
void launch_delight_pack(hipStream_t st, const void* sig, int dtype, int sigs, float* packed, unsigned* mask);
void launch_delight_match(hipStream_t st, const float* q, int m, const float* db, const unsigned* dbmask, int n, float* dist);
constexpr int GIST_LD = 272;
constexpr int GIST_PAIRS = 128;
size_t gist_scratch_floats(int chunk, int nf, int nb);
void launch_gist(hipStream_t st, const void* img, bool u8, int n, int nb, int nf, const float* circ, const float* gabor,
// ... 196 lines not shown
```

so_dso_place_recognition_amd/csrc/pr_api.cpp:

```cpp
#include <hip/hip_runtime.h>

#include <cmath>
#include <algorithm>
#include <cstdio>
#include <cstdlib>
#include <cstring>
#include <new>
#include <string>
#include <type_traits>
#include <vector>

#include "../../include/place_recognition.h"
#include "../../include/pr_m2dp_table.h"
#include "kernels.hpp"
#include "hash_order.hpp"
#include "records.hpp"
#include <chrono>
#include <unordered_map>

struct pr_ctx {
  int device = -1;
  hipStream_t stream = nullptr;
  bool own_stream = true;
  int nan_policy = PR_NAN_EXCLUDE;
  int warnings = 0;
  hipStream_t side = nullptr;
  hipStream_t side2 = nullptr;
  hipEvent_t ev_b = nullptr;
  char* sc_scratch = nullptr;
  void* sel_scratch = nullptr;
  double* rr_scratch = nullptr;
  size_t rr_cap = 0;
  hipEvent_t ev_fork = nullptr, ev_join = nullptr;
  hipEvent_t ev_m2[4] = {nullptr, nullptr, nullptr, nullptr};
  std::string err;
  int* d_svd_rows = nullptr;
  int* d_flags = nullptr;
  bool sc_online_h = false;
  double* d_twiddle = nullptr;
  float* d_cst = nullptr;
  int32_t* d_margin = nullptr;
  int32_t* d_order = nullptr;
  size_t order_cap = 0;
  int32_t order_m = -1;
  unsigned* rr_tick = nullptr;
  size_t tick_cap = 0;
  double* res_partial = nullptr;
  double* res_exact = nullptr;
  size_t res_exact_cap = 0;
  double* xrows = nullptr;
  size_t xrows_cap = 0;
  double* xqspec = nullptr;
  double* xpart = nullptr;
  size_t xpart_cap = 0;
  bool xrow_direct = false;
  void* d_cst_h = nullptr;
  int sc_kernel = 2;
  int sc_mode = PR_SC_ARITH_F16X2;
  double* d_planes = nullptr;
  int sc_nsplit = 0;
  bool force_order = false;
  bool sc_binary = true;
  float sc_bconst = 0.f;
  int bin_gen = 0;
  float sc_pair_scale = 1.f;
  bool timing = false;
  hipEvent_t ev_t[4] = {nullptr, nullptr, nullptr, nullptr};
  int timing_valid = 0;
  void* gist = nullptr;
  void* bow = nullptr;
  void* eval = nullptr;
  void* icp = nullptr;
  void* pose = nullptr;
};

struct pr_sigset {
  int type = 0, role = 0;
  int32_t max_sigs = 0, count = 0;
  int groups = 0;
  int sc_mode = 0;
  float* packed = nullptr;
  size_t floats = 0;
  int* bad = nullptr;
  float* binfo = nullptr;
  int32_t hw = 0;
  int packed_groups = -1;
  bool cap_geom = false;
};

static thread_local std::string g_err;

#define PR_FAIL(ctx, code, ...)                                   \
  do {                                                            \
    char _b[512];                                                 \
    snprintf(_b, sizeof _b, __VA_ARGS__);                         \
    if (ctx) (ctx)->err = _b; else g_err = _b;                    \
    return (code);                                                \
  } while (0)

#define PR_HIP(ctx, call)                                                                     \
  do {                                                                                        \
    hipError_t _e = (call);                                                                   \
    if (_e != hipSuccess) PR_FAIL(ctx, (_e == hipErrorOutOfMemory ? PR_ENOMEM : PR_EHIP),     \
                                  "%s failed: %s", #call, hipGetErrorString(_e));            \
  } while (0)

namespace {

thread_local pr_ctx* g_scope_ctx = nullptr;
struct DevScope {
  pr_ctx* prev;
  explicit DevScope(pr_ctx* c) : prev(g_scope_ctx) { g_scope_ctx = c; }
  ~DevScope() { g_scope_ctx = prev; }
// ... 35 lines not shown
    *groups = pr::sc_dgroups(max_sigs);
    return (size_t)(2 * *groups + 9) * pr::SCF_DIMG / 4;
  }
  if (type == PR_TYPE_SC && sc_mode == 0) {
    if (role == PR_ROLE_QUERY) { *groups = pr::sc_qgroups8(max_sigs); return (size_t)2 * *groups * pr::SCH_QIMG / 4; }
    *groups = pr::sc_dgroups(max_sigs);
    return (size_t)(2 * *groups + 9) * pr::SCH_DIMG / 4;
  }
  if (type == PR_TYPE_SC) {
    if (role == PR_ROLE_QUERY) { *groups = pr::sc_qgroups8(max_sigs); return (size_t)2 * *groups * pr::SC_QIMG; }
    *groups = pr::sc_dgroups(max_sigs);
    return (size_t)2 * *groups * pr::SC_DIMG + 16 * pr::SC_DSTEP;
  }
  if (role == PR_ROLE_QUERY) { *groups = pr::m2_qtiles(max_sigs); return (size_t)2 * *groups * pr::M2_TILE; }
  *groups = pr::m2_tiles(max_sigs);
  return (size_t)(2 * *groups + 16) * pr::M2_TILE;
}

int check_flags(pr_ctx* ctx) {
  int h[7];
  PR_HIP(ctx, hipMemcpyAsync(h, ctx->d_flags, sizeof h, hipMemcpyDeviceToHost, ctx->stream));
  PR_HIP(ctx, hipStreamSynchronize(ctx->stream));
  if (h[0] || h[1] || h[2] || h[3]) PR_HIP(ctx, hipMemsetAsync(ctx->d_flags, 0, 4 * sizeof(int), ctx->stream));
  if (h[5]) {
    PR_HIP(ctx, hipMemsetAsync(ctx->d_flags + 5, 0, sizeof(int), ctx->stream));
    ctx->warnings |= PR_WARN_BOW_TRUNCATED;
  }
  if (h[6]) {
    PR_HIP(ctx, hipMemsetAsync(ctx->d_flags + 6, 0, sizeof(int), ctx->stream));
    ctx->warnings |= PR_WARN_BOW_ROWS;
  }
  if (h[1]) ctx->warnings |= PR_WARN_M2DP_SVD;
  if (h[2]) ctx->warnings |= PR_WARN_ORDER_RESOLVED;
  if (h[3]) ctx->warnings |= PR_WARN_ORDER_UNRESOLVED;
  if (h[0]) {
    if (ctx->nan_policy == PR_NAN_FAIL)
      PR_FAIL(ctx, PR_ENAN, "a signature row has zero L2 norm (MATLAB would produce NaN distances, processSC.m:16,19)");
    ctx->warnings |= PR_WARN_NAN_ROWS;
  }
  return PR_OK;
}

}

extern "C" {

const char* pr_version(void) { return "so_dso_place_recognition_amd 0.1 (gfx950)"; }

const char* pr_last_error(const pr_ctx* ctx) { return ctx ? ctx->err.c_str() : g_err.c_str(); }

static int create_common(int device_id, hipStream_t external, bool use_external, pr_ctx** out) {
  if (!out) PR_FAIL((pr_ctx*)nullptr, PR_EINVAL, "pr_create: out is NULL");
  *out = nullptr;
  int ndev = 0;
  hipError_t e = hipGetDeviceCount(&ndev);
  if (e != hipSuccess || ndev <= 0)
    PR_FAIL((pr_ctx*)nullptr, PR_EHIP, "pr_create: no HIP device available (%s); this library has no CPU fallback",
            e == hipSuccess ? "device count is 0" : hipGetErrorString(e));
  if (device_id < 0 || device_id >= ndev) PR_FAIL((pr_ctx*)nullptr, PR_EINVAL, "pr_create: device %d out of range [0,%d)", device_id, ndev);
  hipDeviceProp_t prop;
  PR_HIP((pr_ctx*)nullptr, hipGetDeviceProperties(&prop, device_id));
  if (strncmp(prop.gcnArchName, "gfx950", 6) != 0)
    PR_FAIL((pr_ctx*)nullptr, PR_EHIP, "pr_create: device %d is %s, this library is built for gfx950 only", device_id, prop.gcnArchName);
  pr_ctx* ctx = new (std::nothrow) pr_ctx;
  if (!ctx) PR_FAIL((pr_ctx*)nullptr, PR_ENOMEM, "pr_create: out of host memory");
  ctx->device = device_id;
  int rc = PR_OK;
  do {
#define TRY(call) if ((call) != hipSuccess) { g_err = std::string(#call) + " failed"; rc = PR_EHIP; break; }
    TRY(hipSetDevice(device_id));
    if (use_external) { ctx->stream = external; ctx->own_stream = false; }
    else TRY(hipStreamCreateWithFlags(&ctx->stream, hipStreamNonBlocking));
    {
      int plo = 0, phi = 0;
      TRY(hipDeviceGetStreamPriorityRange(&plo, &phi));
      TRY(hipStreamCreateWithPriority(&ctx->side, hipStreamNonBlocking, phi));
    }
    TRY(hipStreamCreateWithFlags(&ctx->side2, hipStreamNonBlocking));
    TRY(hipEventCreateWithFlags(&ctx->ev_b, hipEventDisableTiming));
    TRY(hipEventCreateWithFlags(&ctx->ev_fork, hipEventDisableTiming));
    TRY(hipEventCreateWithFlags(&ctx->ev_join, hipEventDisableTiming));
    for (auto& e : ctx->ev_m2) TRY(hipEventCreateWithFlags(&e, hipEventDisableTiming));
    TRY(hipMalloc(&ctx->sel_scratch, pr::select_scratch_bytes()));
    TRY(hipMalloc((void**)&ctx->d_flags, 8 * sizeof(int)));
    TRY(hipMemset(ctx->d_flags, 0, 8 * sizeof(int)));
    TRY(hipMalloc((void**)&ctx->d_svd_rows, (1 + pr::M2DP_SVD_ROWS_CAP) * sizeof(int)));
    TRY(hipMemset(ctx->d_svd_rows, 0, (1 + pr::M2DP_SVD_ROWS_CAP) * sizeof(int)));
    double tw[120 + 4 * 60 * 8];
    for (int t = 0; t < 60; t++) { tw[t] = std::cos(2.0 * M_PI * t / 60.0); tw[60 + t] = std::sin(2.0 * M_PI * t / 60.0); }
    tw[0] = 1; tw[15] = 0; tw[30] = -1; tw[45] = 0; tw[60] = 0; tw[75] = 1; tw[90] = 0; tw[105] = -1;
    for (int fb = 0; fb < 4; fb++)
      for (int sct = 0; sct < 60; sct++)
        for (int j = 0; j < 4; j++) {
          const int t = ((4 * fb + j) * sct) % 60;
          tw[120 + ((fb * 60 + sct) * 4 + j) * 2] = tw[t];
          tw[120 + ((fb * 60 + sct) * 4 + j) * 2 + 1] = tw[60 + t];
        }
    TRY(hipMalloc((void**)&ctx->d_twiddle, sizeof tw));
    TRY(hipMemcpy(ctx->d_twiddle, tw, sizeof tw, hipMemcpyHostToDevice));
    TRY(pr::xrow_set_twiddles(tw, tw + 60));
    std::vector<float> cst((size_t)pr::SC_NSLOT * 128);
    for (int sl = 0; sl < pr::SC_NSLOT; sl++)
      for (int l = 0; l < 64; l++) {
        const int half = l >> 5;
        int k = l & 31; if (k > 30) k = 0;
        const int f = (sl == 0) ? (half ? 30 : 0) : (sl == pr::SC_NSLOT - 1 ? 29 : 2 * sl - 1 + half);
        const int t = (f * k) % 60;
        const double w = (f == 0 || f == 30) ? 1.0 : 2.0;
        float ce = (float)(w * tw[t]), co = (float)(-w * tw[60 + t]);
        if (sl == pr::SC_NSLOT - 1) { if (half) ce = 0.f; else co = 0.f; }
        cst[(size_t)sl * 128 + l] = ce;
        cst[(size_t)sl * 128 + 64 + l] = co;
      }
    TRY(hipMalloc((void**)&ctx->d_cst, cst.size() * sizeof(float)));
    TRY(hipMemcpy(ctx->d_cst, cst.data(), cst.size() * sizeof(float), hipMemcpyHostToDevice));
    {
      std::vector<_Float16> ch((size_t)8 * 64 * 8);
      for (int eo = 0; eo < 2; eo++)
        for (int half = 0; half < 2; half++)
          for (int l = 0; l < 64; l++)
            for (int e = 0; e < 8; e++) {
              int k = l & 31; if (k > 30) k = 30;
              const int f = 16 * half + 8 * (l >> 5) + e;
              double v = 0.0;
              if (f < pr::SC_NF) {
                const int t = (f * k) % 60;
                const double w = (f == 0 || f == 30) ? 1.0 : 2.0;
                v = (eo == 0 ? w * tw[t] : -w * tw[60 + t]) * 1024.0;
              }
              const _Float16 hi = (_Float16)v;
              const _Float16 lo = (_Float16)(v - (double)hi);
              ch[((((size_t)eo * 2 + half) * 2 + 0) * 64 + l) * 8 + e] = hi;
              ch[((((size_t)eo * 2 + half) * 2 + 1) * 64 + l) * 8 + e] = lo;
            }
      TRY(hipMalloc(&ctx->d_cst_h, ch.size() * sizeof(_Float16)));
      TRY(hipMemcpy(ctx->d_cst_h, ch.data(), ch.size() * sizeof(_Float16), hipMemcpyHostToDevice));
      double gamma = 0.0;
      for (int k = 0; k <= 30; k++)
        for (int f = 0; f < pr::SC_NF; f++) {
          const int t = (f * k) % 60;
          const double w = (f == 0 || f == 30) ? 1.0 : 2.0;
          const double c = w * tw[t] * 1024.0, sn = -w * tw[60 + t] * 1024.0;
          const double dc = c - (double)(_Float16)c, ds = sn - (double)(_Float16)sn;
          gamma = std::max(gamma, std::sqrt(dc * dc + ds * ds) / (w * 1024.0));
        }
      const double u = 0x1p-11;
      ctx->sc_bconst = (float)(((u + gamma) * (1.0 + u) + 7e-5) * (1.0 + 1e-6));
    }
    double pl[2][64][3];
    for (int k = 0; k < 64; k++) {
      float nf[3]; memcpy(nf, PR_M2DP_VECN_BITS[k], 12);
      const double n[3] = {nf[0], nf[1], nf[2]};
      const double d = (1.0 * n[0] + 0.0 * n[1]) + 0.0 * n[2];
      const double xa[3] = {1.0, 0.0, 0.0};
      for (int a = 0; a < 3; a++) pl[0][k][a] = xa[a] - d * n[a];
      pl[1][k][0] = n[1] * pl[0][k][2] - n[2] * pl[0][k][1];
      pl[1][k][1] = n[2] * pl[0][k][0] - n[0] * pl[0][k][2];
      pl[1][k][2] = n[0] * pl[0][k][1] - n[1] * pl[0][k][0];
    }
    TRY(hipMalloc((void**)&ctx->d_planes, sizeof pl));
    TRY(hipMemcpy(ctx->d_planes, pl, sizeof pl, hipMemcpyHostToDevice));
#undef TRY
  } while (0);
  if (rc != PR_OK) { pr_destroy(ctx); return rc; }
  if (const char* s = getenv("PR_SC_NSPLIT")) ctx->sc_nsplit = atoi(s);
  if (const char* s = getenv("PR_FORCE_ORDER_FLAGS")) ctx->force_order = atoi(s) != 0;
  if (const char* s = getenv("PR_SC_MATCH")) ctx->sc_mode = (strcmp(s, "f32") == 0) ? PR_SC_ARITH_F32 : (strcmp(s, "f16") == 0) ? PR_SC_ARITH_F16 : PR_SC_ARITH_F16X2;
  if (const char* s = getenv("PR_ICP_SEARCH")) (void)pr_set_icp_search(ctx, strcmp(s, "grid") == 0 ? PR_ICP_SEARCH_GRID : PR_ICP_SEARCH_BRUTE);
  if (const char* s = getenv("PR_SC_KERNEL")) ctx->sc_kernel = (strcmp(s, "h") == 0) ? 0 : 2;
  if (const char* s = getenv("PR_SC_BINARY")) ctx->sc_binary = atoi(s) != 0;
  if (const char* s = getenv("PR_SC_BINARY_PAIR_SCALE")) ctx->sc_pair_scale = (float)atof(s);
  if (const char* s = getenv("PR_XROW")) ctx->xrow_direct = strcmp(s, "direct") == 0;
  if (const char* s = getenv("PR_SC_ONLINE")) ctx->sc_online_h = strcmp(s, "h") == 0;
  *out = ctx;
  return PR_OK;
}

int pr_create(int device_id, pr_ctx** out) { return create_common(device_id, nullptr, false, out); }

int pr_create_on_stream(int device_id, void* hip_stream, pr_ctx** out) {
  return create_common(device_id, static_cast<hipStream_t>(hip_stream), true, out);
}

void pr_destroy(pr_ctx* ctx) {
  if (!ctx) return;
  (void)hipSetDevice(ctx->device);
  if (ctx->stream || !ctx->own_stream) { (void)hipStreamSynchronize(ctx->stream); if (ctx->own_stream) (void)hipStreamDestroy(ctx->stream); }
  if (ctx->side) { (void)hipStreamSynchronize(ctx->side); (void)hipStreamDestroy(ctx->side); }
  if (ctx->side2) { (void)hipStreamSynchronize(ctx->side2); (void)hipStreamDestroy(ctx->side2); }
  if (ctx->ev_b) (void)hipEventDestroy(ctx->ev_b);
  if (ctx->sc_scratch) (void)hipFree(ctx->sc_scratch);
  if (ctx->rr_scratch) (void)hipFree(ctx->rr_scratch);
  if (ctx->d_order) (void)hipFree(ctx->d_order);
  if (ctx->rr_tick) (void)hipFree(ctx->rr_tick);
  if (ctx->res_partial) (void)hipFree(ctx->res_partial);
  if (ctx->res_exact) (void)hipFree(ctx->res_exact);
  if (ctx->xrows) (void)hipFree(ctx->xrows);
  if (ctx->xqspec) (void)hipFree(ctx->xqspec);
  if (ctx->xpart) (void)hipFree(ctx->xpart);
  if (ctx->sel_scratch) (void)hipFree(ctx->sel_scratch);
  if (ctx->ev_fork) (void)hipEventDestroy(ctx->ev_fork);
  if (ctx->ev_join) (void)hipEventDestroy(ctx->ev_join);
  for (auto& e : ctx->ev_m2) if (e) (void)hipEventDestroy(e);
  for (auto& e : ctx->ev_t) if (e) (void)hipEventDestroy(e);
  if (ctx->d_flags) (void)hipFree(ctx->d_flags);
  if (ctx->d_svd_rows) (void)hipFree(ctx->d_svd_rows);
  if (ctx->d_twiddle) (void)hipFree(ctx->d_twiddle);
  if (ctx->d_cst) (void)hipFree(ctx->d_cst);
  if (ctx->d_cst_h) (void)hipFree(ctx->d_cst_h);
  if (ctx->d_planes) (void)hipFree(ctx->d_planes);
  pr::gist_release(ctx->gist);
  pr::bow_release(ctx->bow);
  pr::eval_release(ctx->eval);
  pr::icp_release(ctx->icp);
  pr::pose_release(ctx->pose);
  delete ctx;
}

int pr_set_sc_arith(pr_ctx* ctx, int arith) {
  if (!ctx) return PR_EINVAL;
  if (arith != PR_SC_ARITH_F16X2 && arith != PR_SC_ARITH_F32 && arith != PR_SC_ARITH_F16) PR_FAIL(ctx, PR_EINVAL, "pr_set_sc_arith: unknown arithmetic %d", arith);
  ctx->sc_mode = arith;
  return PR_OK;
}

int pr_get_sc_arith(const pr_ctx* ctx) { return ctx ? ctx->sc_mode : PR_EINVAL; }

int pr_set_nan_policy(pr_ctx* ctx, int policy) {
  if (!ctx) return PR_EINVAL;
  if (policy != PR_NAN_EXCLUDE && policy != PR_NAN_FAIL) PR_FAIL(ctx, PR_EINVAL, "pr_set_nan_policy: unknown policy %d", policy);
  ctx->nan_policy = policy;
  return PR_OK;
}

int pr_get_nan_policy(const pr_ctx* ctx) { return ctx ? ctx->nan_policy : PR_EINVAL; }

int pr_set_exact_statistics(pr_ctx* ctx, int on) {
  if (!ctx) return PR_EINVAL;
  ctx->force_order = on != 0;
  return PR_OK;
}

int pr_take_warnings(pr_ctx* ctx) {
  if (!ctx) return 0;
  if (set_device(ctx) == PR_OK) (void)check_flags(ctx);
  const int w = ctx->warnings;
  ctx->warnings = 0;
  return w;
}

void* pr_stream(pr_ctx* ctx) { return ctx ? (void*)ctx->stream : nullptr; }

int pr_sync(pr_ctx* ctx) {
  if (!ctx) return PR_EINVAL;
  if (int rc = set_device(ctx)) return rc;
  PR_HIP(ctx, hipStreamSynchronize(ctx->stream));
  PR_HIP(ctx, hipGetLastError());
  return check_flags(ctx);
}


int pr_hash_order(const int32_t* keys, int32_t K, int32_t* order) {
  if (K < 0 || (K > 0 && (!keys || !order))) return PR_EINVAL;
  std::vector<int> cnt, nb;
  pr::probe_bucket_schedule(K, cnt, nb);
  std::vector<int> next((size_t)K + 1), bkt(nb.empty() ? 1 : (size_t)nb.back());
  pr::hash_order(keys, K, cnt.data(), nb.data(), (int)cnt.size(), next.data(), bkt.data(), order);
  return PR_OK;
}

int pr_pts_preprocess_gpu(pr_ctx* ctx, const char* poses_file, const char* pts_file, const char* incoming_id_file,
                          double lidarRange, int polar, int verbose, pr_clouds** out) {
  if (!ctx) return PR_EINVAL;
  if (!poses_file || !pts_file || !out || !(lidarRange > 0)) PR_FAIL(ctx, PR_EINVAL, "pr_pts_preprocess_gpu: bad arguments");
  if (int rc = set_device(ctx)) return rc;
  std::vector<pr_rec::PoseRec> poses;
  pr_rec::History h;
  pr_rec::read_records(poses_file, pts_file, poses, h);
  FILE* idf = nullptr;
  if (incoming_id_file) {
    idf = fopen(incoming_id_file, "w");
    if (!idf) PR_FAIL(ctx, PR_EIO, "cannot write %s", incoming_id_file);
  }
// ... 331 lines not shown
  return PR_OK;
}

int pr_set_kernel_timing(pr_ctx* ctx, int on) {
  if (!ctx) return PR_EINVAL;
  if (int rc = set_device(ctx)) return rc;
  if (on) for (auto& e : ctx->ev_t) if (!e) PR_HIP(ctx, hipEventCreate(&e));
  ctx->timing = on != 0;
  ctx->timing_valid = 0;
  return PR_OK;
}

int pr_last_distance_timing(pr_ctx* ctx, float* ms) {
  if (!ctx || !ms) return PR_EINVAL;
  if (!ctx->timing || !ctx->timing_valid) PR_FAIL(ctx, PR_EINVAL, "pr_last_distance_timing: no timed pr_distances_dev call (pr_set_kernel_timing)");
  if (int rc = set_device(ctx)) return rc;
  PR_HIP(ctx, hipEventSynchronize(ctx->ev_t[3]));
  ms[0] = ms[1] = ms[2] = 0.f;
  if (ctx->timing_valid == 3) {
    PR_HIP(ctx, hipEventElapsedTime(&ms[0], ctx->ev_t[0], ctx->ev_t[1]));
    PR_HIP(ctx, hipEventElapsedTime(&ms[1], ctx->ev_t[1], ctx->ev_t[2]));
    PR_HIP(ctx, hipEventElapsedTime(&ms[2], ctx->ev_t[2], ctx->ev_t[3]));
  } else {
    PR_HIP(ctx, hipEventElapsedTime(&ms[0], ctx->ev_t[0], ctx->ev_t[3]));
  }
  return PR_OK;
}

int pr_sc_binary_state(pr_ctx* ctx, const pr_sigset* q, const pr_sigset* db, int32_t* state) {
  if (!ctx || !q || !db || !state) return PR_EINVAL;
  if (int rc = set_device(ctx)) return rc;
  *state = 0;
  if (!q->binfo || !db->binfo || !ctx->sc_binary) return PR_OK;
  int hq[pr::SC_BSTAT_INTS], hd[pr::SC_BSTAT_INTS];
  PR_HIP(ctx, hipMemcpyAsync(hq, sigset_bstat(q), sizeof hq, hipMemcpyDeviceToHost, ctx->stream));
  PR_HIP(ctx, hipMemcpyAsync(hd, sigset_bstat(db), sizeof hd, hipMemcpyDeviceToHost, ctx->stream));
  PR_HIP(ctx, hipStreamSynchronize(ctx->stream));
  auto fl = [](int b) { float f; memcpy(&f, &b, 4); return f; };
  const float eq = std::sqrt(((fl(hq[2]) + fl(hq[3])) + fl(hq[4])) + fl(hq[5])), ed = std::sqrt(((fl(hd[2]) + fl(hd[3])) + fl(hd[4])) + fl(hd[5]));
  const float bound = (eq + ed + eq * ed + ctx->sc_bconst * (1.f + eq) * (1.f + ed)) * 1.001f;
  if (getenv("PR_AMD_VERBOSE"))
    fprintf(stderr, "pr_sc_binary_state: queries {nonbinary %d, max ones %d, eps %.3g} db {nonbinary %d, max ones %d, eps %.3g} bound %.4g x %.1f\n",
            hq[0], hq[1], eq, hd[0], hd[1], ed, bound, std::sqrt((float)hq[1] * (float)hd[1]));
  *state = (hq[0] == 0 && hd[0] == 0 && bound * std::sqrt((float)hq[1] * (float)hd[1]) < 0.72f) ? 1 : 0;
  if (*state) {
    int viol = 0;
    PR_HIP(ctx, hipMemcpyAsync(&viol, ctx->d_flags + 4, sizeof viol, hipMemcpyDeviceToHost, ctx->stream));
    PR_HIP(ctx, hipStreamSynchronize(ctx->stream));
    if (viol != 0) *state = 2;
  }
  return PR_OK;
}

int pr_row_moments_dev(pr_ctx* ctx, const float* d_p, const float* d_i, int32_t m, int32_t n, double* mom) {
  if (!ctx || !d_p || !d_i || !mom || m < 0 || n < 1) return PR_EINVAL;
  if (int rc = set_device(ctx)) return rc;
  pr::launch_row_moments(ctx->stream, d_p, d_i, m, n, mom, ctx->sel_scratch);
  PR_HIP(ctx, hipGetLastError());
  return PR_OK;
}

static int fuse_select_impl(pr_ctx* ctx, const float* d_p, const float* d_i, int32_t m, int32_t n, const double* mom_all,
                            int32_t G, int32_t q_row0, int32_t db_row0, int32_t mask_width, double p_weight, int32_t k,
                            int32_t* idx, float* score, double* score64) {
  if (!ctx || !d_p || (d_i && !mom_all) || !idx || !score || m < 0 || n < 1 || G < 1 || k < 1)
    return PR_EINVAL;
  if (int rc = set_device(ctx)) return rc;
  pr::launch_fuse_select(ctx->stream, d_p, d_i, m, n, mom_all, G, q_row0, db_row0, mask_width, p_weight, k, idx, score, nullptr, nullptr, nullptr, ctx->sel_scratch, score64);
  PR_HIP(ctx, hipGetLastError());
  return PR_OK;
}
int pr_fuse_select_dev(pr_ctx* ctx, const float* d_p, const float* d_i, int32_t m, int32_t n, const double* mom_all,
                       int32_t G, int32_t q_row0, int32_t db_row0, int32_t mask_width, double p_weight, int32_t k,
                       int32_t* idx, float* score) {
  return fuse_select_impl(ctx, d_p, d_i, m, n, mom_all, G, q_row0, db_row0, mask_width, p_weight, k, idx, score, nullptr);
}
int pr_fuse_select_f64_dev(pr_ctx* ctx, const float* d_p, const float* d_i, int32_t m, int32_t n, const double* mom_all,
                           int32_t G, int32_t q_row0, int32_t db_row0, int32_t mask_width, double p_weight, int32_t k,
                           int32_t* idx, float* score, double* score64) {
  if (!score64) return PR_EINVAL;
  return fuse_select_impl(ctx, d_p, d_i, m, n, mom_all, G, q_row0, db_row0, mask_width, p_weight, k, idx, score, score64);
}

static int fuse_select2_impl(pr_ctx* ctx, const float* d_p, const float* d_i, const float* e_p, const float* e_i, int32_t m, int32_t n,
                             const double* mom_all, const double* mom2_all, int32_t G, int32_t q_row0, int32_t db_row0,
                             int32_t mask_width, double p_weight, int32_t k, int32_t* idx, float* score, double* score64) {
  if (!ctx || !d_p || !d_i || !e_p || !e_i || !mom_all || !mom2_all || !idx || !score || m < 0 || n < 1 || G < 1 || k < 1) return PR_EINVAL;
  if (int rc = set_device(ctx)) return rc;
  pr::launch_fuse_select(ctx->stream, d_p, d_i, m, n, mom_all, G, q_row0, db_row0, mask_width, p_weight, k, idx, score, e_p, e_i, mom2_all, ctx->sel_scratch, score64);
  PR_HIP(ctx, hipGetLastError());
  return PR_OK;
}
int pr_fuse_select2_dev(pr_ctx* ctx, const float* d_p, const float* d_i, const float* e_p, const float* e_i, int32_t m, int32_t n,
                        const double* mom_all, const double* mom2_all, int32_t G, int32_t q_row0, int32_t db_row0,
                        int32_t mask_width, double p_weight, int32_t k, int32_t* idx, float* score) {
  return fuse_select2_impl(ctx, d_p, d_i, e_p, e_i, m, n, mom_all, mom2_all, G, q_row0, db_row0, mask_width, p_weight, k, idx, score, nullptr);
}
int pr_fuse_select2_f64_dev(pr_ctx* ctx, const float* d_p, const float* d_i, const float* e_p, const float* e_i, int32_t m, int32_t n,
                            const double* mom_all, const double* mom2_all, int32_t G, int32_t q_row0, int32_t db_row0,
                            int32_t mask_width, double p_weight, int32_t k, int32_t* idx, float* score, double* score64) {
  if (!score64) return PR_EINVAL;
  return fuse_select2_impl(ctx, d_p, d_i, e_p, e_i, m, n, mom_all, mom2_all, G, q_row0, db_row0, mask_width, p_weight, k, idx, score, score64);
}

static int rerank_width(int k, int mode) { const int w = k + (mode == PR_SC_ARITH_F16 ? 56 : 8); return w > 128 ? 128 : w; }

static double pass_eps(const pr_ctx* ctx) { return ctx->sc_mode == PR_SC_ARITH_F16 ? PR_F16_DISTANCE_BOUND : 0.0; }

int pr_f16_margin_dev(pr_ctx* ctx, const double* mom_sc, const double* mom_m2, int32_t m, int32_t G, double p_weight, int32_t k_in,
                      const double* cand_score, int32_t k, const double* score, int32_t* flags, int32_t* count) {
  if (!ctx) return PR_EINVAL;
  if ((!mom_sc && !mom_m2) || !cand_score || !score || !flags || !count || m < 0 || G < 1 || k < 1 || k_in < k || k_in > 128)
    PR_FAIL(ctx, PR_EINVAL, "pr_f16_margin_dev: bad arguments (m=%d, G=%d, k=%d, k_in=%d)", m, G, k, k_in);
  if (int rc = set_device(ctx)) return rc;
  pr::launch_zero_ints(ctx->stream, count, 1);
  pr::launch_margin_check(ctx->stream, mom_sc, mom_m2, G, m, p_weight, k_in, cand_score, k, score, PR_F16_DISTANCE_BOUND, flags, count,
                          ctx->order_m == m ? ctx->d_order : nullptr, PR_F16_SIGMA_REL, PR_F16_DIST_ERR);
  ctx->order_m = -1;
  PR_HIP(ctx, hipGetLastError());
  return PR_OK;
}

static int rerank_scratch(pr_ctx* ctx, size_t need, int32_t m) {
  if (need > ctx->rr_cap) {
    if (ctx->rr_scratch) { PR_HIP(ctx, hipStreamSynchronize(ctx->stream)); PR_HIP(ctx, hipFree(ctx->rr_scratch)); ctx->rr_scratch = nullptr; ctx->rr_cap = 0; }
    PR_HIP(ctx, hipMalloc((void**)&ctx->rr_scratch, need * sizeof(double)));
    ctx->rr_cap = need;
  }
  if ((size_t)m > ctx->order_cap) {
    if (ctx->d_order) { PR_HIP(ctx, hipStreamSynchronize(ctx->stream)); PR_HIP(ctx, hipFree(ctx->d_order)); ctx->d_order = nullptr; ctx->order_cap = 0; }
    PR_HIP(ctx, hipMalloc((void**)&ctx->d_order, ((size_t)2 * m + 2) * sizeof(int32_t)));
    ctx->order_cap = (size_t)m;
  }
  return PR_OK;
}
static int rerank_ticks(pr_ctx* ctx, size_t pairs) {
  if (pairs > ctx->tick_cap) {
    if (ctx->rr_tick) { PR_HIP(ctx, hipStreamSynchronize(ctx->stream)); PR_HIP(ctx, hipFree(ctx->rr_tick)); ctx->rr_tick = nullptr; ctx->tick_cap = 0; }
    PR_HIP(ctx, hipMalloc((void**)&ctx->rr_tick, (2 * pairs + 1) * sizeof(unsigned)));
    PR_HIP(ctx, hipMemsetAsync(ctx->rr_tick, 0, (2 * pairs + 1) * sizeof(unsigned), ctx->stream));
    ctx->tick_cap = pairs;
  }
  return PR_OK;
}
static int32_t* res_list(pr_ctx* ctx) { return ctx->d_order + ctx->order_cap; }
static int32_t* res_cnt(pr_ctx* ctx) { return ctx->d_order + 2 * ctx->order_cap; }
static unsigned* res_tick(pr_ctx* ctx) { return reinterpret_cast<unsigned*>(ctx->res_partial + (size_t)pr::RESOLVE_SLOTS * pr::RESOLVE_NB * 12); }
static int resolve_scratch_base(pr_ctx* ctx, int32_t m_exact) {
  if (!ctx->res_partial) {
    PR_HIP(ctx, hipMalloc((void**)&ctx->res_partial, ((size_t)pr::RESOLVE_SLOTS * pr::RESOLVE_NB * 12 + 1) * sizeof(double)));
    PR_HIP(ctx, hipMemsetAsync(ctx->res_partial + (size_t)pr::RESOLVE_SLOTS * pr::RESOLVE_NB * 12, 0, sizeof(double), ctx->stream));
  }
  if (!ctx->xqspec) PR_HIP(ctx, hipMalloc((void**)&ctx->xqspec, pr::xrow_qspec_doubles() * sizeof(double)));
  if ((size_t)m_exact > ctx->res_exact_cap) {
    if (ctx->res_exact) { PR_HIP(ctx, hipStreamSynchronize(ctx->stream)); PR_HIP(ctx, hipFree(ctx->res_exact)); ctx->res_exact = nullptr; ctx->res_exact_cap = 0; }
    PR_HIP(ctx, hipMalloc((void**)&ctx->res_exact, (size_t)m_exact * 12 * sizeof(double)));
    ctx->res_exact_cap = (size_t)m_exact;
  }
  return PR_OK;
}
static int resolve_scratch_rows(pr_ctx* ctx, int32_t slots, int32_t n_local) {
  const size_t need = (size_t)(slots < pr::RESOLVE_SLOTS ? slots : pr::RESOLVE_SLOTS) * 4 * (size_t)n_local;
  if (need > ctx->xrows_cap) {
    if (ctx->xrows) { PR_HIP(ctx, hipStreamSynchronize(ctx->stream)); PR_HIP(ctx, hipFree(ctx->xrows)); ctx->xrows = nullptr; ctx->xrows_cap = 0; }
    size_t cap = need + need / 8;
    if (hipMalloc((void**)&ctx->xrows, cap * sizeof(double)) != hipSuccess) { (void)hipGetLastError(); cap = need; PR_HIP(ctx, hipMalloc((void**)&ctx->xrows, cap * sizeof(double))); }
// ... 211 lines not shown
  return PR_OK;
}

int pr_widen_scores_dev(pr_ctx* ctx, const float* score32, int64_t count, double* score64) {
  if (!ctx) return PR_EINVAL;
  if (count < 0 || (count > 0 && (!score32 || !score64))) PR_FAIL(ctx, PR_EINVAL, "pr_widen_scores_dev: bad arguments");
  if (int rc = set_device(ctx)) return rc;
  pr::launch_widen(ctx->stream, score32, count, score64);
  PR_HIP(ctx, hipGetLastError());
  return PR_OK;
}

int pr_merge_topk_dev(pr_ctx* ctx, const int32_t* idx_all, const double* score_all, int32_t G, int32_t m, int32_t k, int32_t* idx,
                      double* score) {
  if (!ctx) return PR_EINVAL;
  if (!idx_all || !score_all || !idx || !score || G < 1 || G > 64 || m < 0 || k < 1 || k > 128)
    PR_FAIL(ctx, PR_EINVAL, "pr_merge_topk_dev: bad arguments (G=%d, m=%d, k=%d; G <= 64, k <= 128)", G, m, k);
  if (int rc = set_device(ctx)) return rc;
  pr::launch_merge_topk(ctx->stream, idx_all, score_all, G, m, k, idx, score);
  PR_HIP(ctx, hipGetLastError());
  return PR_OK;
}

int pr_align_pairs_dev(pr_ctx* ctx, const void* q_sc, const void* db_sc, int sc_dtype, const void* q_m2, const void* db_m2, int m2_dtype,
                       int32_t m, int32_t n_local, int32_t db_row0, int32_t k, const int32_t* idx, int32_t* variant, double* dist) {
  if (!ctx) return PR_EINVAL;
  const bool sc = q_sc || db_sc, m2 = q_m2 || db_m2;
  if ((!sc && !m2) || (sc && (!q_sc || !db_sc)) || (m2 && (!q_m2 || !db_m2)) || !idx || !variant || !dist || m < 0 || n_local < 0 ||
      db_row0 < 0 || k < 1 || (int64_t)m * k * 4 > INT32_MAX || (sc && sc_dtype != PR_F64 && sc_dtype != PR_F32) ||
      (m2 && m2_dtype != PR_F64 && m2_dtype != PR_F32))
    PR_FAIL(ctx, PR_EINVAL, "pr_align_pairs_dev: bad arguments (m=%d, n_local=%d, db_row0=%d, k=%d)", m, n_local, db_row0, k);
  if (m == 0) return PR_OK;
  if (int rc = set_device(ctx)) return rc;
  pr::launch_align(ctx->stream, q_sc, db_sc, sc_dtype, q_m2, db_m2, m2_dtype, m, n_local, db_row0, k, idx, variant, dist);
  PR_HIP(ctx, hipGetLastError());
  return PR_OK;
}

int pr_delight_align_pairs_dev(pr_ctx* ctx, const void* q, const void* db, int dtype, int32_t m, int32_t n_local, int32_t db_row0, int32_t k,
                               const int32_t* idx, int32_t* variant, double* dist) {
  if (!ctx) return PR_EINVAL;
  if (!q || !db || !idx || !variant || !dist || m < 0 || n_local < 0 || db_row0 < 0 || k < 1 || (int64_t)m * k > INT32_MAX ||
      (dtype != PR_F64 && dtype != PR_F32))
    PR_FAIL(ctx, PR_EINVAL, "pr_delight_align_pairs_dev: bad arguments (m=%d, n_local=%d, db_row0=%d, k=%d)", m, n_local, db_row0, k);
  if (m == 0) return PR_OK;
  if (int rc = set_device(ctx)) return rc;
  pr::launch_delight_align(ctx->stream, q, db, dtype, m, n_local, db_row0, k, idx, variant, dist);
  PR_HIP(ctx, hipGetLastError());
  return PR_OK;
}

}

namespace {

enum { CREATE, UPLOAD, PACK, DISTANCES, MOMENTS };

struct Desc {
  int type = -1;
  const double *hq = nullptr, *hdb = nullptr;
  const void* db = nullptr;
  SigSet sq, sdb;
  DevBuf rq, rdb, dp, di, mom;
  int step(pr_ctx* ctx, int s, int32_t m, int32_t n) {
    const size_t sig = sig_doubles(type);
    switch (s) {
      case CREATE:
        if (int rc = sq.create(ctx, type, PR_ROLE_QUERY, m)) return rc;
        return sdb.create(ctx, type, PR_ROLE_DB, n);
      case UPLOAD:
        PR_HIP(ctx, rq.alloc((size_t)m * sig * 8));
        PR_HIP(ctx, hipMemcpyAsync(rq.p, hq, (size_t)m * sig * 8, hipMemcpyHostToDevice, ctx->stream));
        if (!hdb) return PR_OK;
        PR_HIP(ctx, rdb.alloc((size_t)n * sig * 8));
        PR_HIP(ctx, hipMemcpyAsync(rdb.p, hdb, (size_t)n * sig * 8, hipMemcpyHostToDevice, ctx->stream));
        db = rdb.p;
        return PR_OK;
      case PACK:
        if (int rc = pr_sigset_pack(ctx, sq.s, rq.p, PR_F64, PR_DEVICE, m)) return rc;
        return pr_sigset_pack(ctx, sdb.s, db, PR_F64, PR_DEVICE, n);
      case DISTANCES:
        PR_HIP(ctx, dp.alloc((size_t)m * n * 4));
        if (type != PR_TYPE_DELIGHT) PR_HIP(ctx, di.alloc((size_t)m * n * 4));
        return pr_distances_dev(ctx, sq.s, sdb.s, dp.as<float>(), di.as<float>());
    }
    PR_HIP(ctx, mom.alloc((size_t)m * 6 * 8));
    return pr_row_moments_dev(ctx, dp.as<float>(), di.as<float>(), m, n, mom.as<double>());
  }
};

struct Types {
  Desc t[2];
  Desc& add(int type, const double* hq, const double* hdb) {
    Desc& d = t[type == PR_TYPE_M2DP ? 1 : 0];
    d.type = type; d.hq = hq; d.hdb = hdb;
    return d;
  }
  int prepare(pr_ctx* ctx, int32_t m, int32_t n, int last) {
    for (int s = CREATE; s <= last; s++)
      for (Desc& d : t)
        if (int rc = d.type < 0 ? PR_OK : d.step(ctx, s, m, n)) return rc;
    return PR_OK;
  }
  double* mom(int i, int32_t i0) { return t[i].type < 0 ? nullptr : t[i].mom.as<double>() + (size_t)i0 * 6; }
  template <typename F, typename... R> int dev(F f, pr_ctx* ctx, int32_t i0, R... rest) {
    const void* q[2] = {nullptr, nullptr};
    for (int i = 0; i < 2; i++)
      if (t[i].type >= 0) q[i] = t[i].rq.as<double>() + (size_t)i0 * sig_doubles(t[i].type);
    return f(ctx, q[0], t[0].db, PR_F64, q[1], t[1].db, PR_F64, mom(0, i0), mom(1, i0), rest...);
  }
};

struct TopkBufs {
  DevBuf idx, sc, sw, kidx, ksc;
  int alloc(pr_ctx* ctx, size_t rows, int width, int k) {
    PR_HIP(ctx, idx.alloc(rows * width * 4));
    PR_HIP(ctx, sc.alloc(rows * width * 4));
    PR_HIP(ctx, sw.alloc(rows * width * 8));
    PR_HIP(ctx, kidx.alloc(rows * k * 4));
    PR_HIP(ctx, ksc.alloc(rows * k * 8));
    return PR_OK;
  }
};

struct ArithScope {
  pr_ctx* ctx;
  int prev;
  ArithScope(pr_ctx* c, int mode) : ctx(c), prev(c->sc_mode) { c->sc_mode = mode; }
  ~ArithScope() { ctx->sc_mode = prev; }
};

template <typename I, typename S> int no_candidate(size_t count, I* idx, S* score) {
  for (size_t i = 0; i < count; i++) { idx[i] = -1; score[i] = NAN; }
  return PR_OK;
}

template <typename D, typename H> int download_topk(pr_ctx* ctx, const int32_t* didx, const D* dscore, size_t count, int32_t* idx, H* score) {
  constexpr bool direct = std::is_same<D, H>::value;
  std::vector<D> tmp(direct ? 0 : count);
  hipError_t e = hipMemcpyAsync(idx, didx, count * 4, hipMemcpyDeviceToHost, ctx->stream);
  if (e == hipSuccess) e = hipMemcpyAsync(direct ? (void*)score : (void*)tmp.data(), dscore, count * sizeof(D), hipMemcpyDeviceToHost, ctx->stream);
  if (e != hipSuccess) {
    (void)hipStreamSynchronize(ctx->stream);
    PR_FAIL(ctx, PR_EHIP, "top-k download failed: %s", hipGetErrorString(e));
  }
  if (int rc = pr_sync(ctx)) return rc;
  for (size_t i = 0; i < tmp.size(); i++) score[i] = (H)tmp[i];
  return PR_OK;
}

template <typename H>
int plain_topk(pr_ctx* ctx, const float* dist, int32_t m, int32_t n, int32_t mask_width, double p_weight, int32_t k, int32_t* idx, H* score) {
  DevBuf didx, dsc;
  PR_HIP(ctx, didx.alloc((size_t)m * k * 4));
  PR_HIP(ctx, dsc.alloc((size_t)m * k * 4));
  if (int rc = pr_fuse_select_dev(ctx, dist, nullptr, m, n, nullptr, 1, 0, 0, mask_width, p_weight, k, didx.as<int32_t>(), dsc.as<float>())) return rc;
  return download_topk(ctx, didx.as<int32_t>(), dsc.as<float>(), (size_t)m * k, idx, score);
}

int topk_core(pr_ctx* ctx, Types& T, int32_t i0, int32_t len, int32_t n, int32_t q_row0, int32_t mask_width, double p_weight, int32_t k,
              TopkBufs& b) {
  const int kin = rerank_width(k, ctx->sc_mode);
  const size_t o = (size_t)i0 * n;
  Desc &sc = T.t[0], &m2 = T.t[1], &one = sc.type >= 0 ? sc : m2;
  int rc = sc.type >= 0 && m2.type >= 0
      ? pr_fuse_select2_dev(ctx, sc.dp.as<float>() + o, sc.di.as<float>() + o, m2.dp.as<float>() + o, m2.di.as<float>() + o, len, n, T.mom(0, i0),
                            T.mom(1, i0), 1, q_row0, 0, mask_width, p_weight, kin, b.idx.as<int32_t>(), b.sc.as<float>())
      : pr_fuse_select_dev(ctx, one.dp.as<float>() + o, one.di.as<float>() + o, len, n, one.mom.as<double>() + (size_t)i0 * 6, 1, q_row0, 0,
                           mask_width, p_weight, kin, b.idx.as<int32_t>(), b.sc.as<float>());
  if (rc) return rc;
  if ((rc = pr_widen_scores_dev(ctx, b.sc.as<float>(), (int64_t)len * kin, b.sw.as<double>()))) return rc;
  if ((rc = T.dev(pr_rerank_dev, ctx, i0, len, n, 1, q_row0, 0, mask_width, p_weight, kin, b.idx.as<int32_t>(), b.sw.as<double>(), k,
                  b.kidx.as<int32_t>(), b.ksc.as<double>())))
    return rc;
  if (ctx->sc_mode == PR_SC_ARITH_F16) return PR_OK;
  return T.dev(pr_order_resolve_dev, ctx, i0, len, n, q_row0, mask_width, p_weight, k, b.kidx.as<int32_t>(), b.ksc.as<double>(), nullptr);
}

int f16_fallback(pr_ctx* ctx, Types& T, int32_t m, int32_t n, int32_t mask_width, double p_weight, int32_t k, TopkBufs& top) {
  int32_t cnt = 0;
  std::vector<int32_t> fl(m), F;
  std::vector<double> rows[2];
  DevBuf dflags, dcount;
  PR_HIP(ctx, dflags.alloc((size_t)m * 4));
  PR_HIP(ctx, dcount.alloc(4));
  if (int rc = pr_f16_margin_dev(ctx, T.mom(0, 0), T.mom(1, 0), m, 1, p_weight, rerank_width(k, ctx->sc_mode), top.sw.as<double>(), k,
                                 top.ksc.as<double>(), dflags.as<int32_t>(), dcount.as<int32_t>()))
    return rc;
  PR_HIP(ctx, hipMemcpyAsync(&cnt, dcount.p, 4, hipMemcpyDeviceToHost, ctx->stream));
  PR_HIP(ctx, hipStreamSynchronize(ctx->stream));
  if (cnt == 0) return PR_OK;
  PR_HIP(ctx, hipMemcpyAsync(fl.data(), dflags.p, (size_t)m * 4, hipMemcpyDeviceToHost, ctx->stream));
  PR_HIP(ctx, hipStreamSynchronize(ctx->stream));
  for (int32_t q = 0; q < m; q++) if (fl[q]) F.push_back(q);
  const int32_t mf = (int32_t)F.size();
  ctx->warnings |= PR_WARN_F16_FALLBACK;
  ArithScope split_(ctx, PR_SC_ARITH_F16X2);
  Types R;
  for (int i = 0; i < 2; i++) {
    if (T.t[i].type < 0) continue;
    const size_t sig = sig_doubles(T.t[i].type);
    rows[i].resize((size_t)mf * sig);
    for (int32_t r = 0; r < mf; r++) memcpy(rows[i].data() + (size_t)r * sig, T.t[i].hq + (size_t)F[r] * sig, sig * 8);
    Desc& d = R.add(T.t[i].type, rows[i].data(), nullptr);
    d.db = T.t[i].db;
    for (int s = CREATE; s <= MOMENTS; s++)
      if (int rc = d.step(ctx, s, mf, n)) return rc;
  }
  std::vector<int32_t> run_end;
  for (int32_t i = 1; i <= mf; i++)
    if (i == mf || (mask_width > 0 && F[i] != F[i - 1] + 1)) run_end.push_back(i);
  int32_t longest = 0;
  for (size_t r = 0, a0 = 0; r < run_end.size(); a0 = run_end[r++]) longest = std::max<int32_t>(longest, run_end[r] - (int32_t)a0);
  TopkBufs b;
  if (int rc = b.alloc(ctx, longest, rerank_width(k, ctx->sc_mode), k)) return rc;
  for (size_t r = 0, a0 = 0; r < run_end.size(); a0 = run_end[r++]) {
    const int32_t i0 = (int32_t)a0, len = run_end[r] - i0;
    if (int rc = topk_core(ctx, R, i0, len, n, mask_width > 0 ? F[i0] : 0, mask_width, p_weight, k, b)) return rc;
    for (int32_t i = 0; i < len;) {
      int32_t j = i + 1;
      while (j < len && F[i0 + j] == F[i0 + j - 1] + 1) j++;
      const size_t to = (size_t)F[i0 + i] * k, from = (size_t)i * k, nk = (size_t)(j - i) * k;
      PR_HIP(ctx, hipMemcpyAsync(top.kidx.as<int32_t>() + to, b.kidx.as<int32_t>() + from, nk * 4, hipMemcpyDeviceToDevice, ctx->stream));
      PR_HIP(ctx, hipMemcpyAsync(top.ksc.as<double>() + to, b.ksc.as<double>() + from, nk * 8, hipMemcpyDeviceToDevice, ctx->stream));
      i = j;
    }
  }
  PR_HIP(ctx, hipStreamSynchronize(ctx->stream));
  return PR_OK;
}

template <typename H>
int topk_host(pr_ctx* ctx, const char* who, int type, const double* a1, const double* b1, int32_t m, const double* a2, const double* b2,
              int32_t n, int32_t mask_width, double p_weight, int32_t k, int32_t* idx, H* score) {
  if (!ctx) return PR_EINVAL;
  const bool fused = type < 0, plain = type == PR_TYPE_DELIGHT;
  if (fused && (m < 0 || n < 2 || k < 1 || k > 120 || !idx || !score || (m > 0 && (!a1 || !b1)) || !a2 || !b2))
    PR_FAIL(ctx, PR_EINVAL, "%s: bad arguments (m=%d, n=%d, k=%d)", who, m, n, k);
  if (!fused) {
    if (type != PR_TYPE_SC && type != PR_TYPE_M2DP && !plain) PR_FAIL(ctx, PR_EINVAL, "%s: unknown type %d", who, type);
    if (!score) PR_FAIL(ctx, PR_EINVAL, "%s: score is NULL", who);
    if (m < 0 || n < 0 || (m > 0 && !a1) || (n > 0 && !a2)) PR_FAIL(ctx, PR_EINVAL, "%s: bad signature buffers (m=%d, n=%d)", who, m, n);
    if (k < 1 || (!plain && k > 120) || !idx)
      PR_FAIL(ctx, PR_EINVAL, "%s needs 1 <= k <= 120 (SC, M2DP) and output buffers", who);
    if (n == 0) return no_candidate((size_t)m * k, idx, score);
    if (!plain && n < 2) PR_FAIL(ctx, PR_EINVAL, "%s needs n >= 2 (N-1 standard deviation)", who);
  }
  if (m == 0) return PR_OK;
  if (int rc = set_device(ctx)) return rc;
  DevScope scope_(ctx);
  Types T;
  T.add(fused ? PR_TYPE_SC : type, a1, a2);
  if (fused) T.add(PR_TYPE_M2DP, b1, b2);
  if (int rc = T.prepare(ctx, m, n, plain ? DISTANCES : MOMENTS)) return rc;
  if (plain) return plain_topk(ctx, T.t[0].dp.as<float>(), m, n, mask_width, p_weight, k, idx, score);
  TopkBufs top;
  if (int rc = top.alloc(ctx, m, rerank_width(k, ctx->sc_mode), k)) return rc;
  if (int rc = topk_core(ctx, T, 0, m, n, 0, mask_width, p_weight, k, top)) return rc;
  if (ctx->sc_mode == PR_SC_ARITH_F16)
    if (int rc = f16_fallback(ctx, T, m, n, mask_width, p_weight, k, top)) return rc;
  return download_topk(ctx, top.kidx.as<int32_t>(), top.ksc.as<double>(), (size_t)m * k, idx, score);
}

int distance_host(pr_ctx* ctx, const char* who, int type, const double* h1, int32_t m, const double* h2, int32_t n, float* out_p, float* out_i) {
  if (!ctx) return PR_EINVAL;
  if (m < 0 || n < 0 || (m > 0 && !h1) || (n > 0 && !h2)) PR_FAIL(ctx, PR_EINVAL, "%s: bad signature buffers (m=%d, n=%d)", who, m, n);
  if (m == 0 || n == 0) return PR_OK;
  if (int rc = set_device(ctx)) return rc;
  DevScope scope_(ctx);
  Types T;
  Desc& d = T.add(type, h1, h2);
  if (int rc = T.prepare(ctx, m, n, DISTANCES)) return rc;
  if (out_p) PR_HIP(ctx, hipMemcpyAsync(out_p, d.dp.p, (size_t)m * n * 4, hipMemcpyDeviceToHost, ctx->stream));
  if (out_i && d.di.p) PR_HIP(ctx, hipMemcpyAsync(out_i, d.di.p, (size_t)m * n * 4, hipMemcpyDeviceToHost, ctx->stream));
  return pr_sync(ctx);
}

}

extern "C" {

int pr_sc_distance(pr_ctx* ctx, const double* h1, int32_t m, const double* h2, int32_t n, float* d_struct, float* d_int) {
  return distance_host(ctx, "pr_sc_distance", PR_TYPE_SC, h1, m, h2, n, d_struct, d_int);
}

int pr_m2dp_distance(pr_ctx* ctx, const double* h1, int32_t m, const double* h2, int32_t n, float* d_cnt, float* d_int) {
  return distance_host(ctx, "pr_m2dp_distance", PR_TYPE_M2DP, h1, m, h2, n, d_cnt, d_int);
}

int pr_delight_distance(pr_ctx* ctx, const double* h1, int32_t m, const double* h2, int32_t n, float* dist) {
  return distance_host(ctx, "pr_delight_distance", PR_TYPE_DELIGHT, h1, m, h2, n, dist, nullptr);
}

int pr_match_topk(pr_ctx* ctx, int type, const double* h1, int32_t m, const double* h2, int32_t n, int32_t mask_width,
                  double p_weight, int32_t k, int32_t* idx, float* score) {
  return topk_host(ctx, "pr_match_topk", type, h1, nullptr, m, h2, nullptr, n, mask_width, p_weight, k, idx, score);
}

int pr_match_topk_f64(pr_ctx* ctx, int type, const double* h1, int32_t m, const double* h2, int32_t n, int32_t mask_width,
                      double p_weight, int32_t k, int32_t* idx, double* score) {
  return topk_host(ctx, "pr_match_topk_f64", type, h1, nullptr, m, h2, nullptr, n, mask_width, p_weight, k, idx, score);
}

int pr_match_topk_fused(pr_ctx* ctx, const double* sc1, const double* m2dp1, int32_t m, const double* sc2, const double* m2dp2,
                        int32_t n, int32_t mask_width, double p_weight, int32_t k, int32_t* idx, float* score) {
  return topk_host(ctx, "pr_match_topk_fused", -1, sc1, m2dp1, m, sc2, m2dp2, n, mask_width, p_weight, k, idx, score);
}

int pr_match_topk_fused_f64(pr_ctx* ctx, const double* sc1, const double* m2dp1, int32_t m, const double* sc2, const double* m2dp2,
                            int32_t n, int32_t mask_width, double p_weight, int32_t k, int32_t* idx, double* score) {
  return topk_host(ctx, "pr_match_topk_fused_f64", -1, sc1, m2dp1, m, sc2, m2dp2, n, mask_width, p_weight, k, idx, score);
}

static int align_host(pr_ctx* ctx, const char* who, int type, const double* a1, const double* b1, int32_t m, const double* a2, const double* b2,
                      int32_t n, int32_t k, const int32_t* idx, int32_t* var_out, double* dist_out) {
  if (!ctx) return PR_EINVAL;
  const bool fused = type < 0;
  if (!fused && type != PR_TYPE_SC && type != PR_TYPE_M2DP && type != PR_TYPE_DELIGHT) PR_FAIL(ctx, PR_EINVAL, "%s: type must be SC, M2DP or DELIGHT", who);
  if (m < 0 || n < 0 || k < 1 || (int64_t)m * k * 4 > INT32_MAX || (m > 0 && (!idx || !var_out || !dist_out || !a1 || (fused && !b1))))
    PR_FAIL(ctx, PR_EINVAL, "%s: bad arguments (m=%d, n=%d, k=%d)", who, m, n, k);
  const size_t mk = (size_t)m * k;
  std::vector<int32_t> rows;
  rows.reserve(mk);
  for (size_t i = 0; i < mk; i++) {
    if (idx[i] < -1 || idx[i] >= n) PR_FAIL(ctx, PR_EINVAL, "%s: idx[%zu] = %d is outside [-1, %d)", who, i, idx[i], n);
    if (idx[i] >= 0) rows.push_back(idx[i]);
  }
  std::sort(rows.begin(), rows.end());
  rows.erase(std::unique(rows.begin(), rows.end()), rows.end());
  const int S = fused ? 4 : 2;
  if (rows.empty()) return no_candidate(mk * S, var_out, dist_out);
  if (!a2 || (fused && !b2)) PR_FAIL(ctx, PR_EINVAL, "%s: the DB signatures are NULL", who);
  std::vector<int32_t> lidx(mk);
  for (size_t i = 0; i < mk; i++)
    lidx[i] = idx[i] < 0 ? -1 : (int32_t)(std::lower_bound(rows.begin(), rows.end(), idx[i]) - rows.begin());
  if (int rc = set_device(ctx)) return rc;
  const int32_t u = (int32_t)rows.size();
// ... 453 lines not shown
```

so_dso_place_recognition_amd/csrc/pr_group.cpp:

```cpp
#include <dlfcn.h>
#include <hip/hip_runtime.h>
#include <rccl/rccl.h>

#include <cstdio>
#include <cstdlib>
#include <cstring>
#include <new>
#include <string>
#include <vector>

#include "../../include/place_recognition.h"

namespace {

enum { PH_PACK = 0, PH_MATCH, PH_MOMENTS, PH_GATHER_A, PH_SELECT, PH_GATHER_B, PH_RERANK, PH_GATHER_C, PH_FINISH, PH_EXACT };

struct Rccl {
  void* h = nullptr;
  ncclResult_t (*CommInitAll)(ncclComm_t*, int, const int*) = nullptr;
  ncclResult_t (*CommDestroy)(ncclComm_t) = nullptr;
  ncclResult_t (*CommCount)(const ncclComm_t, int*) = nullptr;
  ncclResult_t (*AllGather)(const void*, void*, size_t, ncclDataType_t, ncclComm_t, hipStream_t) = nullptr;
  ncclResult_t (*GroupStart)() = nullptr;
  ncclResult_t (*GroupEnd)() = nullptr;
// ... 272 lines not shown

static int set_database_impl(pr_group* g, int type, const double* h2, int32_t n, int32_t extra) {
  g->type = -1; g->q_cap = 0; g->k_cap = 0;
  if ((type != PR_TYPE_SC && type != PR_TYPE_M2DP) || n < 2 || !h2 || extra < 0) G_FAIL(g, PR_EINVAL, "pr_group_set_database: type must be SC or M2DP, n >= 2, extra >= 0");
  const size_t row_doubles = type == PR_TYPE_SC ? PR_SC_SIG_LEN : (size_t)4 * PR_M2DP_SIG_LEN;
  for (int r = 0; r < g->G; r++) {
    Shard& sh = g->s[r];
    G_HIP(g, hipSetDevice(sh.device));
    if (sh.db) { pr_sigset_destroy(sh.ctx, sh.db); sh.db = nullptr; }
    if (sh.raw_db) { (void)hipFree(sh.raw_db); sh.raw_db = nullptr; }
    free_match_buffers(sh);
    sh.row0 = (int32_t)((int64_t)n * r / g->G);
    sh.rows = (int32_t)((int64_t)n * (r + 1) / g->G) - sh.row0;
    if (sh.rows < 1) G_FAIL(g, PR_EINVAL, "pr_group_set_database: fewer signatures (%d) than shards (%d)", n, g->G);
    sh.cap_rows = sh.rows + (r == g->G - 1 ? extra : 0);
    const size_t bytes = (size_t)sh.rows * row_doubles * 8;
    G_HIP(g, hipMalloc(&sh.raw_db, (size_t)sh.cap_rows * row_doubles * 8));
    G_HIP(g, hipMemcpyAsync(sh.raw_db, h2 + (size_t)sh.row0 * row_doubles, bytes, hipMemcpyHostToDevice, sh.stream));
    G_PR(g, sh, pr_sigset_create(sh.ctx, type, PR_ROLE_DB, sh.cap_rows, &sh.db));
    if (sh.cap_rows > sh.rows) G_PR(g, sh, pr_sigset_reserve(sh.ctx, sh.db));
    G_PR(g, sh, pr_sigset_pack(sh.ctx, sh.db, sh.raw_db, PR_F64, PR_DEVICE, sh.rows));
  }
  for (auto& sh : g->s) { G_HIP(g, hipSetDevice(sh.device)); G_PR(g, sh, pr_sync(sh.ctx)); }
  g->type = type; g->n = n; g->q_cap = 0; g->k_cap = 0;
  return PR_OK;
}

static int match_topk_impl(pr_group* g, const double* h1, int32_t m, int32_t mask_width, double p_weight, int32_t k, int32_t* idx,
                           double* score) {
  if (g->type < 0) G_FAIL(g, PR_EINVAL, "pr_group_match_topk: no database (pr_group_set_database)");
  const int G = g->G;
  if (m < 0 || (m > 0 && !h1) || k < 1 || k > 120 || G > 64 || !idx || !score)
    G_FAIL(g, PR_EINVAL, "pr_group_match_topk: bad arguments (m=%d, k=%d; k <= 120, at most 64 shards)", m, k);
  if (m == 0) return PR_OK;
  const int type = g->type;
  const bool sc = type == PR_TYPE_SC;
  const size_t row_doubles = sc ? PR_SC_SIG_LEN : (size_t)4 * PR_M2DP_SIG_LEN;
  const int kin = k + 8 > 128 ? 128 : k + 8;
  if (m > g->q_cap || k > g->k_cap) {
    const int32_t qc = m > g->q_cap ? m : g->q_cap, kc = k > g->k_cap ? k : g->k_cap;
    const int kinc = kc + 8 > 128 ? 128 : kc + 8;
    g->q_cap = g->k_cap = 0;
    for (auto& sh : g->s) {
      free_match_buffers(sh);
      G_HIP(g, hipSetDevice(sh.device));
      G_PR(g, sh, pr_sigset_create(sh.ctx, type, PR_ROLE_QUERY, qc, &sh.q));
      G_HIP(g, hipMalloc(&sh.raw_q, (size_t)qc * row_doubles * 8));
      G_HIP(g, hipMalloc((void**)&sh.d_p, (size_t)qc * sh.cap_rows * 4));
      G_HIP(g, hipMalloc((void**)&sh.d_i, (size_t)qc * sh.cap_rows * 4));
      G_HIP(g, hipMalloc((void**)&sh.mom, (size_t)qc * 6 * 8));
      G_HIP(g, hipMalloc((void**)&sh.mom_all, (size_t)G * qc * 6 * 8));
      G_HIP(g, hipMalloc((void**)&sh.idx_in, (size_t)qc * kinc * 4));
      G_HIP(g, hipMalloc((void**)&sh.sc32, (size_t)qc * kinc * 4));
      G_HIP(g, hipMalloc((void**)&sh.idx, (size_t)qc * kc * 4));
      G_HIP(g, hipMalloc((void**)&sh.score, (size_t)qc * kc * 8));
      G_HIP(g, hipMalloc((void**)&sh.idx_all, (size_t)G * qc * kinc * 4));
      G_HIP(g, hipMalloc((void**)&sh.score_all, (size_t)G * qc * kinc * 8));
      G_HIP(g, hipMalloc((void**)&sh.sc64, (size_t)qc * kinc * 8));
      G_HIP(g, hipMalloc((void**)&sh.part, (size_t)qc * 5 * kinc * 8));
      G_HIP(g, hipMalloc((void**)&sh.p5_all, (size_t)G * qc * 5 * kinc * 8));
      G_HIP(g, hipMalloc((void**)&sh.exact, (size_t)qc * 12 * 8));
      G_HIP(g, hipMalloc((void**)&sh.exact_all, (size_t)G * qc * 12 * 8));
      G_HIP(g, hipMalloc((void**)&sh.sel, (size_t)64 * 2 * kc * 8));
      G_HIP(g, hipMalloc((void**)&sh.sel_all, (size_t)G * 64 * 2 * kc * 8));
      G_HIP(g, hipMalloc((void**)&sh.dump, (size_t)qc * kinc * 8));
      G_HIP(g, hipMalloc((void**)&sh.cand, (size_t)qc * kinc * 4));
    }
    g->q_cap = qc; g->k_cap = kc;
  }
  g->timed = false;
  auto mark = [&](int phase_end) -> int {
    if (!g->timing) return PR_OK;
    for (auto& sh : g->s) { G_HIP(g, hipSetDevice(sh.device)); G_HIP(g, hipEventRecord(sh.ph[phase_end], sh.stream)); }
    return PR_OK;
  };
  if (int rc = mark(PH_PACK)) return rc;
  for (auto& sh : g->s) {
    G_HIP(g, hipSetDevice(sh.device));
    G_HIP(g, hipMemcpyAsync(sh.raw_q, h1, (size_t)m * row_doubles * 8, hipMemcpyHostToDevice, sh.stream));
    G_PR(g, sh, pr_sigset_pack(sh.ctx, sh.q, sh.raw_q, PR_F64, PR_DEVICE, m));
    if (g->timing) G_HIP(g, hipEventRecord(sh.ph[PH_MATCH], sh.stream));
    G_PR(g, sh, pr_distances_dev(sh.ctx, sh.q, sh.db, sh.d_p, sh.d_i));
    if (g->timing) G_HIP(g, hipEventRecord(sh.ph[PH_MOMENTS], sh.stream));
    G_PR(g, sh, pr_row_moments_dev(sh.ctx, sh.d_p, sh.d_i, m, sh.rows, sh.mom));
  }
  if (int rc = mark(PH_GATHER_A)) return rc;
  std::vector<const void*> src(G);
  std::vector<void*> dst(G);
  for (int r = 0; r < G; r++) { src[r] = g->s[r].mom; dst[r] = g->s[r].mom_all; }
  if (int rc = exchange(g, src, dst, (size_t)m * 6 * 8)) return rc;
  if (int rc = mark(PH_SELECT)) return rc;
  for (auto& sh : g->s) {
    G_HIP(g, hipSetDevice(sh.device));
    G_PR(g, sh, pr_fuse_select_dev(sh.ctx, sh.d_p, sh.d_i, m, sh.rows, sh.mom_all, G, 0, sh.row0, mask_width, p_weight, kin, sh.idx_in, sh.sc32));
    G_PR(g, sh, pr_widen_scores_dev(sh.ctx, sh.sc32, (int64_t)m * kin, sh.sc64));
  }
  if (int rc = mark(PH_GATHER_B)) return rc;
  for (int r = 0; r < G; r++) { src[r] = g->s[r].idx_in; dst[r] = g->s[r].idx_all; }
  if (int rc = exchange(g, src, dst, (size_t)m * kin * 4)) return rc;
  for (int r = 0; r < G; r++) { src[r] = g->s[r].sc64; dst[r] = g->s[r].score_all; }
  if (int rc = exchange(g, src, dst, (size_t)m * kin * 8)) return rc;
  if (int rc = mark(PH_RERANK)) return rc;
  for (auto& sh : g->s) {
    G_HIP(g, hipSetDevice(sh.device));
    G_PR(g, sh, pr_merge_topk_dev(sh.ctx, sh.idx_all, sh.score_all, G, m, kin, sh.cand, sh.dump ));
    G_PR(g, sh, pr_rerank_partial_dev(sh.ctx, sc ? sh.raw_q : nullptr, sc ? sh.raw_db : nullptr, PR_F64, sc ? nullptr : sh.raw_q,
                                      sc ? nullptr : sh.raw_db, PR_F64, sc ? sh.mom_all : nullptr, sc ? nullptr : sh.mom_all, m, sh.rows, G, 0,
                                      sh.row0, mask_width, p_weight, kin, sh.cand, sh.dump, k, sh.part));
  }
  if (int rc = mark(PH_GATHER_C)) return rc;
  for (int r = 0; r < G; r++) { src[r] = g->s[r].part; dst[r] = g->s[r].p5_all; }
  if (int rc = exchange(g, src, dst, (size_t)m * 5 * kin * 8)) return rc;
  if (int rc = mark(PH_FINISH)) return rc;
  for (auto& sh : g->s) {
    G_HIP(g, hipSetDevice(sh.device));
    G_PR(g, sh, pr_rerank_finish_dev(sh.ctx, sc ? sh.mom_all : nullptr, sc ? nullptr : sh.mom_all, G, sh.cand, sh.dump, sh.p5_all, G, m, kin, k,
                                     p_weight, sh.idx, sh.score));
  }
  if (int rc = mark(PH_EXACT)) return rc;
  int32_t flagged = 0;
  {
    Shard& s0 = g->s[0];
    G_HIP(g, hipSetDevice(s0.device));
    G_PR(g, s0, pr_order_flagged_count(s0.ctx, m, &flagged));
  }
  g->last_flagged = flagged;
  for (int32_t off = 0; off < flagged; off += 64) {
    for (auto& sh : g->s) {
      G_HIP(g, hipSetDevice(sh.device));
      G_PR(g, sh, pr_order_exact_moments_dev(sh.ctx, sc ? sh.raw_q : nullptr, sc ? sh.raw_db : nullptr, PR_F64, sc ? nullptr : sh.raw_q,
                                             sc ? nullptr : sh.raw_db, PR_F64, sc ? sh.mom_all : nullptr, sc ? nullptr : sh.mom_all, G, m, sh.rows,
                                             off, off + 64 >= flagged, sh.exact));
    }
    for (int r = 0; r < G; r++) { src[r] = g->s[r].exact; dst[r] = g->s[r].exact_all; }
    if (int rc = exchange(g, src, dst, (size_t)m * 12 * 8)) return rc;
    for (auto& sh : g->s) {
      G_HIP(g, hipSetDevice(sh.device));
      G_PR(g, sh, pr_order_exact_select_dev(sh.ctx, sh.exact_all, G, m, sh.rows, 0, sh.row0, mask_width, p_weight, sc ? 1 : 0, sc ? 0 : 1, k, off, sh.sel));
    }
    for (int r = 0; r < G; r++) { src[r] = g->s[r].sel; dst[r] = g->s[r].sel_all; }
    if (int rc = exchange(g, src, dst, (size_t)64 * 2 * k * 8)) return rc;
    for (auto& sh : g->s) {
      G_HIP(g, hipSetDevice(sh.device));
      G_PR(g, sh, pr_order_exact_merge_dev(sh.ctx, sh.sel_all, G, m, k, off, sh.idx, sh.score));
    }
  }
  if (int rc = mark(PR_GROUP_PHASES)) return rc;
  g->timed = g->timing;
  Shard& s0 = g->s[0];
  G_HIP(g, hipSetDevice(s0.device));
  G_HIP(g, hipMemcpyAsync(idx, s0.idx, (size_t)m * k * 4, hipMemcpyDeviceToHost, s0.stream));
  G_HIP(g, hipMemcpyAsync(score, s0.score, (size_t)m * k * 8, hipMemcpyDeviceToHost, s0.stream));
  for (auto& sh : g->s) { G_HIP(g, hipSetDevice(sh.device)); G_PR(g, sh, pr_sync(sh.ctx)); }
  return PR_OK;
}

static int settle(pr_group* g, int rc) {
  if (rc == PR_OK) return rc;
  const std::string keep = g->err;
  for (auto& sh : g->s) if (sh.ctx) { (void)hipSetDevice(sh.device); (void)hipStreamSynchronize(sh.stream); }
  g->err = keep;
  return rc;
}

int pr_group_set_database(pr_group* g, int type, const double* h2, int32_t n) {
  if (!g) return PR_EINVAL;
  return settle(g, set_database_impl(g, type, h2, n, 0));
}

int pr_group_set_database_growable(pr_group* g, int type, const double* h2, int32_t n, int32_t extra_capacity) {
  if (!g) return PR_EINVAL;
  return settle(g, set_database_impl(g, type, h2, n, extra_capacity));
}

static int append_database_impl(pr_group* g, const double* h_new, int32_t n_new) {
  if (g->type < 0) G_FAIL(g, PR_EINVAL, "pr_group_append_database: no database (pr_group_set_database_growable)");
// ... 38 lines not shown
```

so_dso_place_recognition_amd/matcher.py:

```python
from __future__ import annotations

import ctypes as C
import weakref

import numpy as np
import torch

from . import _lib
from .api import Context


def _dptr(t: torch.Tensor | None):
    if t is None:
        return None
    assert t.is_cuda and t.is_contiguous()
    return C.c_void_p(t.data_ptr())


def _torch_dt(t: torch.Tensor) -> int:
    return {torch.float64: _lib.F64, torch.float32: _lib.F32}[t.dtype]


def _raw_rows(d) -> tuple:
    assert d._q_sig.dtype == d.db_sig.dtype
# ... 42 lines not shown
        else:
            torch.cuda.current_stream(self.dev).synchronize()

    def _leave(self):
        if self._same_stream():
            return
        if self._lib_stream is not None:
            torch.cuda.current_stream(self.dev).wait_stream(self._lib_stream)
        else:
            self.ctx.sync()

    def _buf(self, name, shape, dtype):
        t = self._bufs.get(name)
        if t is None or tuple(t.shape) != tuple(shape) or t.dtype != dtype:
            need = 1
            for d in shape:
                need *= int(d)
            flat = self._flat.get(name)
            if flat is None or flat.dtype != dtype or flat.numel() < need:
                flat = torch.empty(need + (need >> 3 if self._raw is not None else 0), dtype=dtype, device=self.dev)
                self._flat[name] = flat
            t = flat[:need].view(shape)
            self._bufs[name] = t
        return t

    def _slots(self):
        sc = m2 = None
        for d in self.descs:
            if d.type == _lib.TYPE_SC:
                sc = d
            elif d.type == _lib.TYPE_M2DP:
                m2 = d
        return sc, m2

    def _raw6(self) -> tuple:
        sc, m2 = self._slots()
        return (*(_NO_ROWS if sc is None else _raw_rows(sc)), *(_NO_ROWS if m2 is None else _raw_rows(m2)))

    def _moms(self) -> tuple:
        sc, m2 = self._slots()
        return None if sc is None else sc._mom, None if m2 is None else m2._mom

    @property
    def f16(self) -> bool:
        return self.ctx.sc_arith == "f16"

    def _margin(self, mom_sc, mom_m2, G, p_weight, cand_sc: torch.Tensor, k: int, score: torch.Tensor):
        m, kin = cand_sc.shape
        flags = torch.empty((m,), dtype=torch.int32, device=self.dev)
        count = torch.empty((1,), dtype=torch.int32, device=self.dev)
        self._enter()
        self.ctx.check(self.lib.pr_f16_margin_dev(self.ctx.h, _dptr(mom_sc), _dptr(mom_m2), m, G, float(p_weight), kin, _dptr(cand_sc.contiguous()),
                                                  int(k), _dptr(score.contiguous()), _dptr(flags), _dptr(count)))
        self._leave()
        self.f16_flags, self.f16_count = flags, count
        return flags, count

    def _fallback_rows(self, run_rows, idx, score, mask_width, q_row0):
        cnt = int(self.f16_count.item())
        self.f16_fallbacks = cnt
        if cnt == 0:
            return idx, score
        rows = torch.nonzero(self.f16_flags, as_tuple=False).flatten()
        idx, score = idx.clone(), score.clone()
        if mask_width <= 0:
            i2, s2 = run_rows(rows, None)
            idx[rows], score[rows] = i2, s2
        else:
            for r in rows.tolist():
                i2, s2 = run_rows(rows.new_tensor([r]), q_row0 + r)
                idx[r], score[r] = i2[0], s2[0]
        return idx, score

    def _split_twin(self):
        db = self.descs[0].db_sig
        if self._twin is None or self._twin_of is not db:
            if self._twin is not None:
                self._twin.close()
            tw = type(self)(*self._spec, ctx=Context(self.ctx.device, sc_arith="f16x2", stream=self.ctx.stream))
            tw.pack_database(*(d.db_sig for d in self.descs))
            self._twin, self._twin_of = tw, db
        return self._twin

    def local_select(self, mom_all: torch.Tensor, G: int, mask_width, p_weight, k, db_row0, q_row0):
        m, n = self._m, self.n
        stores = self.descs
        if len(stores) == 1:
            stores[0]._mom = mom_all.contiguous()
            select = self.lib.pr_fuse_select_f64_dev
        else:
            for d, t in zip(stores, mom_all.reshape(G, m, 4, 3).split(2, dim=2)):
                d._mom = t.contiguous()
            select = self.lib.pr_fuse_select2_f64_dev
        self._args = (G, q_row0, db_row0, int(mask_width), float(p_weight))
        kin = k if self.plain else int(self.lib.pr_rerank_width(self.ctx.h, int(k)))
        idx_in = self._buf("idx_in", (m, kin), torch.int32)
        sc32 = self._buf("sc32", (m, kin), torch.float32)
        sc64 = self._buf("sc64", (m, kin), torch.float64)
        dists = [_dptr(t) for d in stores for t in (d._bufs["d_p"], d._bufs.get("d_i"))]
        self._enter()
        self.ctx.check(select(self.ctx.h, *dists, m, n, *[_dptr(d._mom) for d in stores], G, q_row0, db_row0, int(mask_width), float(p_weight),
                              int(kin), _dptr(idx_in), _dptr(sc32), _dptr(sc64)))
        self._leave()
        return idx_in, sc64

    def local_rerank(self, cand_idx: torch.Tensor, k: int, partial: bool, cand_sc: torch.Tensor = None):
        m, n = self._m, self.n
        G, q_row0, db_row0, mask_width, p_weight = self._args
        kin = cand_idx.shape[1]
        cand_idx = cand_idx.contiguous()
        cand_sc = None if cand_sc is None else cand_sc.contiguous()
        self._last_cand = (cand_idx, cand_sc)
        rows = (*self._raw6(), *map(_dptr, self._moms()))
        self._enter()
        if partial:
            part = self._buf("part", (m, 5, kin), torch.float64)
            self.ctx.check(self.lib.pr_rerank_partial_dev(self.ctx.h, *rows, m, n, G, q_row0, db_row0, mask_width, p_weight, kin, _dptr(cand_idx),
                                                          _dptr(cand_sc), int(k), _dptr(part)))
            self._leave()
            return part
        idx = self._buf("idx", (m, k), torch.int32)
        score = self._buf("score", (m, k), torch.float64)
        self.ctx.check(self.lib.pr_rerank_dev(self.ctx.h, *rows, m, n, G, q_row0, db_row0, mask_width, p_weight, kin, _dptr(cand_idx),
                                              _dptr(cand_sc), int(k), _dptr(idx), _dptr(score)))
        self._leave()
        return idx, score

    def local_phase2(self, mom_all: torch.Tensor, G: int, mask_width, p_weight, k, db_row0, q_row0):
        idx_in, sc = self.local_select(mom_all, G, mask_width, p_weight, k, db_row0, q_row0)
        if self.plain:
            return idx_in, sc
        return self.local_rerank(idx_in, k, partial=False, cand_sc=sc)

    def merge(self, idx_all: torch.Tensor, sc_all: torch.Tensor, k: int):
        G, m, kk = idx_all.shape
        assert kk == k
        idx = torch.empty((m, k), dtype=torch.int32, device=idx_all.device)
        score = torch.empty((m, k), dtype=torch.float64, device=idx_all.device)
        self._enter()
        self.ctx.check(self.lib.pr_merge_topk_dev(self.ctx.h, _dptr(idx_all.contiguous()), _dptr(sc_all.contiguous()), G, m, k, _dptr(idx),
                                                  _dptr(score)))
        self._leave()
        return idx, score

    def finish(self, cand_idx: torch.Tensor, cand_sc: torch.Tensor | None, part_all: torch.Tensor, k: int):
        G, m, five, kin = part_all.shape
        assert five == 5
        idx = torch.empty((m, k), dtype=torch.int32, device=cand_idx.device)
        score = torch.empty((m, k), dtype=torch.float64, device=cand_idx.device)
        cand_idx = cand_idx.contiguous()
        cand_sc = None if cand_sc is None else cand_sc.contiguous()
        part_all = part_all.contiguous()
        self._enter()
        self.ctx.check(self.lib.pr_rerank_finish_dev(self.ctx.h, *map(_dptr, self._moms()), int(self._args[0]), _dptr(cand_idx), _dptr(cand_sc),
                                                     _dptr(part_all), G, m, kin, k, float(self._args[4]), _dptr(idx), _dptr(score)))
        self._leave()
        return idx, score

    def exact_moments(self, offset: int = 0, last: bool = True):
        m, n = self._m, self.n
        raw6 = self._raw6()
        exact = torch.empty((m, 4, 3), dtype=torch.float64, device=self.dev)
        self._enter()
        self.ctx.check(self.lib.pr_order_exact_moments_dev(self.ctx.h, *raw6, *map(_dptr, self._moms()), int(self._args[0]), m, n, int(offset),
                                                           int(bool(last)), _dptr(exact)))
        self._leave()
        return exact

    def exact_select(self, exact_all: torch.Tensor, k: int, offset: int = 0):
        m, n = self._m, self.n
        _, q_row0, db_row0, mask_width, p_weight = self._args
        mom_sc, mom_m2 = self._moms()
        G = exact_all.shape[0]
        exact_all = exact_all.contiguous()
        sel = torch.empty((RESOLVE_SLOTS, 2, k), dtype=torch.float64, device=self.dev)
        self._enter()
        self.ctx.check(self.lib.pr_order_exact_select_dev(self.ctx.h, _dptr(exact_all), G, m, n, int(q_row0), int(db_row0), int(mask_width),
                                                          float(p_weight), int(mom_sc is not None), int(mom_m2 is not None), int(k), int(offset),
                                                          _dptr(sel)))
        self._leave()
        return sel

    def exact_merge(self, sel_all: torch.Tensor, k: int, idx: torch.Tensor, score: torch.Tensor, offset: int = 0):
        G = sel_all.shape[0]
        sel_all = sel_all.contiguous()
        self._enter()
        self.ctx.check(self.lib.pr_order_exact_merge_dev(self.ctx.h, _dptr(sel_all), G, self._m, int(k), int(offset), _dptr(idx), _dptr(score)))
        self._leave()
        return idx, score

    def _exact_passes(self, exact_order=True):
        m = self._m
        if m <= RESOLVE_SLOTS:
            return 1
        if exact_order == "async":
            return (m + RESOLVE_SLOTS - 1) // RESOLVE_SLOTS
        return (self.flagged_count() + RESOLVE_SLOTS - 1) // RESOLVE_SLOTS

    def _resolve_order(self, k, idx, score, exact_order=True):
        m, n = self._m, self.n
        _, q_row0, _, mask_width, p_weight = self._args
        args = (self.ctx.h, *self._raw6(), *map(_dptr, self._moms()), m, n, int(q_row0), int(mask_width), float(p_weight), int(k), _dptr(idx),
                _dptr(score))
        self._enter()
        if m <= RESOLVE_SLOTS or exact_order == "async":
            self.ctx.check(self.lib.pr_order_resolve_async_dev(*args))
        else:
            cnt = C.c_int32(0)
            self.ctx.check(self.lib.pr_order_resolve_dev(*args, C.byref(cnt)))
            self.resolved = int(cnt.value)
        self._leave()

    def _match(self, queries: tuple, mask_width, p_weight, k, db_row0, q_row0, group, force_exchange, f16_fallback, exact_order, mark):
        G = _world(group)
        f16 = self.f16 and not self.plain
        resolve = ((self.exact_moments, self.exact_select, self.exact_merge, lambda: self._exact_passes(exact_order))
                   if (exact_order and not self.plain and not f16) else None)
        post = (lambda cand_sc, idx, score: self._margin(*self._moms(), self._args[0], p_weight, cand_sc, k, score)) if f16 else None
        idx, score = sharded_topk(lambda: self.local_phase1(*queries),
                                  lambda mom_all, G_: self.local_select(mom_all, G_, mask_width, p_weight, k, db_row0, q_row0),
                                  k, group if (G > 1 or force_exchange) else None, G, merge=self.merge, force_exchange=force_exchange,
                                  rerank=None if self.plain else self.local_rerank, finish=self.finish, post=post, resolve=resolve, mark=mark)
        if f16 and f16_fallback:
            def run_rows(rows, qr0):
                fb = self._split_twin()
                qsel = [q.view(-1, d.rows_per_sig, d.sig_len)[rows].reshape(-1, d.sig_len).contiguous()
                        for d, q in zip(self.descs, queries)]
                return fb._match(qsel, mask_width, p_weight, k, db_row0, q_row0 if qr0 is None else qr0, group, force_exchange, True, exact_order,
                                 None)
            idx, score = self._fallback_rows(run_rows, idx, score, mask_width, q_row0)
        elif resolve is not None and G == 1 and not force_exchange:
            self._resolve_order(k, idx, score, exact_order)
            if mark is not None:
                mark("exact rows (one shard)")
        return idx, score

    def align(self, idx: torch.Tensor, db_row0: int = 0):
        assert all(d.db_sig is not None and d._q_sig is not None for d in self.descs), "match() first"
        idx = idx.to(torch.int32).contiguous()
        m, k = idx.shape
        assert m == self._m
        if self.plain:
            raw = _raw_rows(self)
            v1 = torch.empty((m, k), dtype=torch.int32, device=self.dev)
            d1 = torch.empty((m, k), dtype=torch.float64, device=self.dev)
            self._enter()
            self.ctx.check(self.lib.pr_delight_align_pairs_dev(self.ctx.h, *raw, m, self.n, int(db_row0), k, _dptr(idx), _dptr(v1), _dptr(d1)))
            self._leave()
            return (torch.stack([v1, torch.full_like(v1, -1)], -1), torch.stack([d1, torch.full_like(d1, float("nan"))], -1))
        raw6 = self._raw6()
        var = torch.empty((m, k, 4), dtype=torch.int32, device=self.dev)
        dist = torch.empty((m, k, 4), dtype=torch.float64, device=self.dev)
        self._enter()
        self.ctx.check(self.lib.pr_align_pairs_dev(self.ctx.h, *raw6, m, self.n, int(db_row0), k, _dptr(idx), _dptr(var), _dptr(dist)))
        self._leave()
        ch = slice(0 if raw6[0] is not None else 2, 4 if raw6[3] is not None else 2)
        return var[..., ch], dist[..., ch]

    def evaluate(self, idx: torch.Tensor, score: torch.Tensor, gt1: torch.Tensor, gt2: torch.Tensor, loop_diff: float, mask_width: int = 0,
                 out=None):
        from . import eval as _eval
        self._enter()
        res = _eval.precision_recall_torch(score, idx, gt1, gt2, loop_diff, mask_width, ctx=self.ctx, out=out)
        self._leave()
        return res

    def verify(self, idx: torch.Tensor, clouds_q, clouds_db, frames_q, frames_db, max_src_pts: int, max_dst_pts: int, max_corr: float = 1.0,
               min_fitness: float = 0.5, max_rmse: float = 0.5, max_iter: int = 30, tol_rmse: float = 1e-6, tol_fitness: float = 1e-6,
               min_inliers: int = 3, db_row0: int = 0, search: str | None = None):
        from . import api
        assert getattr(self, "type", None) == _lib.TYPE_SC, "verify() needs an SC matcher: only SC has a relative pose"
        var, _ = self.align(idx, db_row0)
        m, k = idx.shape
        v = var[..., 0].reshape(-1).cpu().numpy()
        ix = idx.reshape(-1).cpu().numpy().astype(np.int64) - int(db_row0)
        has = (v >= 0) & (ix >= 0)
        fq = frames_q.cpu().numpy() if torch.is_tensor(frames_q) else np.asarray(frames_q)
        fd = frames_db.cpu().numpy() if torch.is_tensor(frames_db) else np.asarray(frames_db)
        src = np.where(has, np.repeat(np.arange(m), k), -1).astype(np.int32)
        dst = np.where(has, ix, -1).astype(np.int32)
        T0 = np.tile(np.hstack([np.eye(3), np.zeros((3, 1))]), (m * k, 1, 1))
        if has.any():
            T0[has] = api.sc_relative_pose(fq[src[has]], fd[dst[has]], v[has])
        dT0, dsrc, ddst = (torch.from_numpy(a).to(self.dev) for a in (T0, src, dst))
        self._enter()
        T, stats = api.icp_refine_torch(clouds_q[0], clouds_q[1], clouds_db[0], clouds_db[1], dsrc, ddst, dT0, max_src_pts, max_dst_pts, max_iter,
                                        max_corr, tol_rmse, tol_fitness, min_inliers, ctx=self.ctx, search=search)
        self._leave()
        f64 = stats.view(torch.float64)
        status = stats.view(torch.int32)[:, 6]
        accepted = ((status == _lib.ICP_CONVERGED) | (status == _lib.ICP_MAX_ITER)) & (f64[:, 0] >= min_fitness) & (f64[:, 1] <= max_rmse)
        return T.view(m, k, 3, 4), stats.view(m, k, -1), accepted.view(m, k)

    def verify_dev(self, idx: torch.Tensor, clouds_q, clouds_db, frames_q: torch.Tensor, frames_db: torch.Tensor, max_src_pts: int,
                   max_dst_pts: int, hypotheses: int = 1, seed: str | None = None, max_corr: float = 1.0, min_fitness: float = 0.5,
                   max_rmse: float = 0.5, max_iter: int = 30, tol_rmse: float = 1e-6, tol_fitness: float = 1e-6, min_inliers: int = 3,
                   db_row0: int = 0, out=None, search: str | None = None):
        from . import api
        if isinstance(clouds_db, api.KeyframeMap):
            if frames_db is not None or max_dst_pts is not None or db_row0 != 0:
                raise ValueError("verify_dev: a KeyframeMap brings its frames and bounds: frames_db=None, max_dst_pts=None, db_row0=0")
            return clouds_db.verify_dev(self, idx, clouds_q, frames_q, max_src_pts, hypotheses=hypotheses, seed=seed, max_corr=max_corr,
                                        min_fitness=min_fitness, max_rmse=max_rmse, max_iter=max_iter, tol_rmse=tol_rmse, tol_fitness=tol_fitness,
# ... 19 lines not shown
        if var.shape[-1] == 4 and seed == "m2dp":
            var = var[..., 2:]
        return seed, var, idx.to(torch.int32).contiguous()

    def flagged_count(self) -> int:
        cnt = C.c_int32(0)
        self._enter()
        self.ctx.check(self.lib.pr_order_flagged_count(self.ctx.h, int(self._m), C.byref(cnt)))
        self._leave()
        return int(cnt.value)

    def take_warnings(self) -> int:
        return self.ctx.take_warnings()


class Matcher(_Base):
    def __init__(self, type_: str, max_queries: int, max_db: int, ctx: Context | None = None, device: int | None = None):
        self.type = {"sc": _lib.TYPE_SC, "m2dp": _lib.TYPE_M2DP, "delight": _lib.TYPE_DELIGHT}[type_]
        self.rows_per_sig, self.sig_len = {_lib.TYPE_SC: (1, 2400), _lib.TYPE_M2DP: (4, 384), _lib.TYPE_DELIGHT: (16, 256)}[self.type]
        self.plain = self.type == _lib.TYPE_DELIGHT
        self._init_ctx(ctx, device)
        self._spec = (type_, max_queries, max_db)
        self.q = C.c_void_p()
        self.db = C.c_void_p()
        self.ctx.check(self.lib.pr_sigset_create(self.ctx.h, self.type, _lib.ROLE_QUERY, max_queries, C.byref(self.q)))
        self.ctx.check(self.lib.pr_sigset_create(self.ctx.h, self.type, _lib.ROLE_DB, max_db, C.byref(self.db)))
        self.max_queries, self.max_db = max_queries, max_db
        self.n = 0
        self.db_sig = None
        self._q_sig = None
        self.pre_distances = None
        self.post_distances = None

    @property
    def descs(self):
        return (self,)

    def close(self):
        super().close()
        if self.q:
            self.lib.pr_sigset_destroy(self.ctx.h, self.q)
            self.lib.pr_sigset_destroy(self.ctx.h, self.db)
            self.q = self.db = None

    def _pack(self, handle, sig: torch.Tensor):
        assert sig.is_cuda and sig.is_contiguous() and sig.dim() == 2 and sig.shape[1] == self.sig_len
        assert sig.shape[0] % self.rows_per_sig == 0
        n = sig.shape[0] // self.rows_per_sig
        self.ctx.check(self.lib.pr_sigset_pack(self.ctx.h, handle, _dptr(sig), _torch_dt(sig), _lib.DEVICE, n))
        return n

    def pack_database(self, sig: torch.Tensor):
        self._enter()
        self.n = self._pack(self.db, sig)
        self.db_sig = sig
        self._raw = None

    def reserve_database(self, sig: torch.Tensor | None = None):
        assert self.type in (_lib.TYPE_SC, _lib.TYPE_M2DP)
        self._enter()
        self.ctx.check(self.lib.pr_sigset_reserve(self.ctx.h, self.db))
        self._raw = torch.empty((self.max_db * self.rows_per_sig, self.sig_len), dtype=torch.float64, device=self.dev)
        self.n = 0
        if sig is not None and sig.shape[0]:
            assert sig.dtype == torch.float64
            r = sig.shape[0]
            self._raw[:r].copy_(sig)
            self._enter()
            self.n = self._pack(self.db, self._raw[:r])
        self.db_sig = self._raw[:self.n * self.rows_per_sig]

    def append_database(self, sig: torch.Tensor):
        assert self._raw is not None, "reserve_database() first"
        assert sig.is_cuda and sig.dim() == 2 and sig.shape[1] == self.sig_len and sig.dtype == torch.float64 and sig.shape[0] % self.rows_per_sig == 0
        k, r0 = sig.shape[0] // self.rows_per_sig, self.n * self.rows_per_sig
        assert self.n + k <= self.max_db
        dst = self._raw[r0:r0 + sig.shape[0]]
        dst.copy_(sig)
        self._enter()
        self.ctx.check(self.lib.pr_sigset_append(self.ctx.h, self.db, _dptr(dst), 0, _lib.DEVICE, k))
        self.n += k
        self.db_sig = self._raw[:self.n * self.rows_per_sig]

    def local_phase1(self, queries: torch.Tensor):
        self._enter()
        m = self._pack(self.q, queries)
        n = self.n
        self._q_sig, self._m = queries, m
        d_p = self._buf("d_p", (m, n), torch.float32)
        d_i = None if self.plain else self._buf("d_i", (m, n), torch.float32)
        mom = self._buf("mom", (m, 2, 3), torch.float64)
        lib, h = self.lib, self.ctx.h
        if self.pre_distances:
            self.pre_distances()
        self.ctx.check(lib.pr_distances_dev(h, self.q, self.db, _dptr(d_p), _dptr(d_i)))
        if self.post_distances:
            self.post_distances()
        if self.plain:
            self._leave()
            mom.zero_()
        else:
            self.ctx.check(lib.pr_row_moments_dev(h, _dptr(d_p), _dptr(d_i), m, n, _dptr(mom)))
            self._leave()
        return mom

    def match(self, queries: torch.Tensor, mask_width: int = 0, p_weight: float = 2.0, k: int = 1,
              db_row0: int = 0, q_row0: int = 0, group=None, force_exchange: bool = False, f16_fallback: bool = True,
              exact_order: bool = True, mark=None):
        return self._match((queries,), mask_width, p_weight, k, db_row0, q_row0, group, force_exchange, f16_fallback, exact_order, mark)

    def distances(self):
        return self._bufs["d_p"], self._bufs.get("d_i")

    @classmethod
    def on_new_stream(cls, type_: str, max_queries: int, max_db: int, device: int | None = None):
        return _on_new_stream(cls, device, type_, max_queries, max_db)

    def capture(self, queries: torch.Tensor, mask_width: int = 0, p_weight: float = 2.0, k: int = 1):
        st = self.stream
        eo = True if queries.shape[0] // self.rows_per_sig <= RESOLVE_SLOTS else "async"
        with torch.cuda.stream(st):
            assert self.ctx.stream == int(st.cuda_stream)
            self.match(queries, mask_width, p_weight, k, exact_order=eo)
            st.synchronize()
            g = torch.cuda.CUDAGraph()
            with torch.cuda.graph(g, stream=st):
                idx, score = self.match(queries, mask_width, p_weight, k, exact_order=eo)
        return CapturedMatch(g, st, queries, idx, score)


class CapturedMatch:

    def __init__(self, graph, stream, queries, idx, score):
        self.graph, self.stream, self.queries, self.idx, self.score = graph, stream, queries, idx, score

    check = None

    def run(self, new_queries: torch.Tensor | None = None, sync: bool = True):
        if self.check is not None:
            self.check()
        if new_queries is not None:
            self.stream.wait_stream(torch.cuda.current_stream(new_queries.device))
            new_queries.record_stream(self.stream)
        with torch.cuda.stream(self.stream):
            if new_queries is not None:
                self.queries.copy_(new_queries, non_blocking=True)
            self.graph.replay()
        if sync:
            self.stream.synchronize()
        return self.idx, self.score


class FusedMatcher(_Base):

    def __init__(self, max_queries: int, max_db: int, ctx: Context | None = None, device: int | None = None):
        self._init_ctx(ctx, device)
        self._spec = (max_queries, max_db)
        self.sc = Matcher("sc", max_queries, max_db, self.ctx)
        self.m2 = Matcher("m2dp", max_queries, max_db, self.ctx)
        self.descs = (self.sc, self.m2)

    def close(self):
        super().close()
        self.sc.close(); self.m2.close()

    def pack_database(self, sc_sig: torch.Tensor, m2dp_sig: torch.Tensor):
        self.sc.pack_database(sc_sig); self.m2.pack_database(m2dp_sig)
        assert self.sc.n == self.m2.n, "the two databases must describe the same places"
        self.n = self.sc.n

    def local_phase1(self, sc_queries, m2dp_queries):
        a = self.sc.local_phase1(sc_queries)
        b = self.m2.local_phase1(m2dp_queries)
        assert self.sc._m == self.m2._m
        self._m = self.sc._m
        return torch.cat([a, b], dim=1)

    def match(self, sc_queries: torch.Tensor, m2dp_queries: torch.Tensor, mask_width: int = 0, p_weight: float = 2.0, k: int = 1,
              db_row0: int = 0, q_row0: int = 0, group=None, f16_fallback: bool = True, exact_order: bool = True):
        return self._match((sc_queries, m2dp_queries), mask_width, p_weight, k, db_row0, q_row0, group, False, f16_fallback, exact_order, None)


def _on_new_stream(cls, device, *args, **kw):
    device = torch.cuda.current_device() if device is None else device
    st = torch.cuda.Stream(device)
# ... 286 lines not shown
```

Before: 135,700 queries/s.

## Fuse row moments into single-shard selection with sampled-threshold candidate listing

On single-shard runs, adds a kernel that computes per-row z-score moments and performs top-k selection in one pass over the distance rows, replacing the separate moments kernel, select kernel and score-widen kernel. While streaming both channels it estimates a threshold from a sampled per-wave rank statistic and writes only rows under that threshold into LDS. When the candidate list overflows it falls back to a full path and records the row in a device counter. This removes a second full read of the m×n distance matrices and two launches. The cost is extra ballot and LDS work per element, plus more host-side branching.

```diff
diff --git a/include/place_recognition.h b/include/place_recognition.h
--- a/include/place_recognition.h
+++ b/include/place_recognition.h
@@ -170,6 +170,9 @@
 int pr_fuse_select_f64_dev(pr_ctx* ctx, const float* d_p, const float* d_i, int32_t m, int32_t n,
                            const double* mom_all, int32_t G, int32_t q_row0, int32_t db_row0, int32_t mask_width,
                            double p_weight, int32_t k, int32_t* idx, float* score, double* score64);
+int pr_moments_select_f64_dev(pr_ctx* ctx, const float* d_p, const float* d_i, int32_t m, int32_t n, double* mom, int32_t q_row0,
+                              int32_t db_row0, int32_t mask_width, double p_weight, int32_t k, int32_t* idx, float* score, double* score64);
+int pr_select_fallback_rows(pr_ctx* ctx, int64_t* rows);
 int pr_fuse_select2_f64_dev(pr_ctx* ctx, const float* d_p, const float* d_i, const float* e_p, const float* e_i, int32_t m, int32_t n,
                             const double* mom_all, const double* mom2_all, int32_t G, int32_t q_row0, int32_t db_row0,
                             int32_t mask_width, double p_weight, int32_t k, int32_t* idx, float* score, double* score64);
diff --git a/so_dso_place_recognition_amd/_lib.py b/so_dso_place_recognition_amd/_lib.py
--- a/so_dso_place_recognition_amd/_lib.py
+++ b/so_dso_place_recognition_amd/_lib.py
@@ -154,6 +154,8 @@
     "pr_sigset_image": (C.c_int, [_vp, C.POINTER(_vp), C.POINTER(C.c_size_t), C.POINTER(_i32)]),
     "pr_distances_dev": (C.c_int, [_vp, _vp, _vp, _vp, _vp]),
     "pr_row_moments_dev": (C.c_int, [_vp, _vp, _vp, _i32, _i32, _vp]),
+    "pr_moments_select_f64_dev": (C.c_int, [_vp, _vp, _vp, _i32, _i32, _vp, _i32, _i32, _i32, _dbl, _i32, _vp, _vp, _vp]),
+    "pr_select_fallback_rows": (C.c_int, [_vp, C.POINTER(C.c_int64)]),
     "pr_fuse_select_dev": (C.c_int, [_vp, _vp, _vp, _i32, _i32, _vp, _i32, _i32, _i32, _i32, _dbl, _i32, _vp, _vp]),
     "pr_sc_generate_dev": (C.c_int, [_vp, _vp, _vp, _vp, _i32, _dbl, _vp]),
     "pr_m2dp_generate_dev": (C.c_int, [_vp, _vp, _vp, _vp, _i32, _dbl, _vp]),
diff --git a/so_dso_place_recognition_amd/csrc/fuse_select.hip b/so_dso_place_recognition_amd/csrc/fuse_select.hip
--- a/so_dso_place_recognition_amd/csrc/fuse_select.hip
+++ b/so_dso_place_recognition_amd/csrc/fuse_select.hip
@@ -1,3 +1,4 @@
+#include <cmath>
 #include <cstdlib>
 
 #include "div_rn.hpp"
@@ -20,40 +21,51 @@
   return r;
 }
 
+__device__ __forceinline__ double moments_pivot(float r0) {
+  return (r0 == r0) ? (double)r0 : 0.5;
+}
+__device__ __forceinline__ void moments_acc(float v, double c, double& s1, double& s2, double& cnt) {
+  if (v == v) { const double d = (double)v - c; s1 += d; s2 += d * d; cnt += 1.0; }
+}
+__device__ __forceinline__ void moments_store(double* __restrict__ o, double c, double S1, double S2, double N) {
+  o[0] = N;
+  o[1] = N > 0.0 ? c + S1 / N : 0.0;
+  o[2] = N > 0.0 ? S2 - S1 * S1 / N : 0.0;
+}
+__device__ __forceinline__ void moments_channel(const float* __restrict__ row, int n, double* red, int tid, double& c_out, double& S1, double& S2,
+                                                double& N) {
+  const double c = moments_pivot(row[0]);
+  double s1 = 0.0, s2 = 0.0, cnt = 0.0;
+  auto acc = [&](float v) { moments_acc(v, c, s1, s2, cnt); };
+  int head = (int)((4 - ((reinterpret_cast<size_t>(row) >> 2) & 3)) & 3);
+  if (head > n) head = n;
+  const int nv = (n - head) >> 2;
+  if (tid < head) acc(row[tid]);
+  const f32x4* rv4 = reinterpret_cast<const f32x4*>(row + head);
+  int j = tid;
+  for (; j + 768 < nv; j += 1024) {
+    const f32x4 a = rv4[j], b = rv4[j + 256], c4 = rv4[j + 512], d4 = rv4[j + 768];
+    acc(a[0]); acc(a[1]); acc(a[2]); acc(a[3]);
+    acc(b[0]); acc(b[1]); acc(b[2]); acc(b[3]);
+    acc(c4[0]); acc(c4[1]); acc(c4[2]); acc(c4[3]);
+    acc(d4[0]); acc(d4[1]); acc(d4[2]); acc(d4[3]);
+  }
+  for (; j < nv; j += 256) { const f32x4 a = rv4[j]; acc(a[0]); acc(a[1]); acc(a[2]); acc(a[3]); }
+  for (int t = head + 4 * nv + tid; t < n; t += 256) acc(row[t]);
+  S1 = block_sum(s1, red, tid);
+  S2 = block_sum(s2, red, tid);
+  N = block_sum(cnt, red, tid);
+  c_out = c;
+}
+
 __global__ __launch_bounds__(256) void row_moments_kernel(const float* __restrict__ d_p, const float* __restrict__ d_i,
                                                            int n, double* __restrict__ mom) {
   __shared__ double red[256];
   const int tid = threadIdx.x, q = blockIdx.x;
   for (int ch = 0; ch < 2; ch++) {
-    const float* row = (ch ? d_i : d_p) + (size_t)q * n;
-    const float r0 = row[0];
-    const double c = (r0 == r0) ? (double)r0 : 0.5;
-    double s1 = 0.0, s2 = 0.0, cnt = 0.0;
-    auto acc = [&](float v) { if (v == v) { const double d = (double)v - c; s1 += d; s2 += d * d; cnt += 1.0; } };
-    int head = (int)((4 - ((reinterpret_cast<size_t>(row) >> 2) & 3)) & 3);
-    if (head > n) head = n;
-    const int nv = (n - head) >> 2;
-    if (tid < head) acc(row[tid]);
-    const f32x4* rv4 = reinterpret_cast<const f32x4*>(row + head);
-    int j = tid;
-    for (; j + 768 < nv; j += 1024) {
-      const f32x4 a = rv4[j], b = rv4[j + 256], c4 = rv4[j + 512], d4 = rv4[j + 768];
-      acc(a[0]); acc(a[1]); acc(a[2]); acc(a[3]);
-      acc(b[0]); acc(b[1]); acc(b[2]); acc(b[3]);
-      acc(c4[0]); acc(c4[1]); acc(c4[2]); acc(c4[3]);
-      acc(d4[0]); acc(d4[1]); acc(d4[2]); acc(d4[3]);
-    }
-    for (; j < nv; j += 256) { const f32x4 a = rv4[j]; acc(a[0]); acc(a[1]); acc(a[2]); acc(a[3]); }
-    for (int t = head + 4 * nv + tid; t < n; t += 256) acc(row[t]);
-    const double S1 = block_sum(s1, red, tid);
-    const double S2 = block_sum(s2, red, tid);
-    const double N = block_sum(cnt, red, tid);
-    if (tid == 0) {
-      double* o = mom + ((size_t)q * 2 + ch) * 3;
-      o[0] = N;
-      o[1] = N > 0.0 ? c + S1 / N : 0.0;
-      o[2] = N > 0.0 ? S2 - S1 * S1 / N : 0.0;
-    }
+    double c, S1, S2, N;
+    moments_channel((ch ? d_i : d_p) + (size_t)q * n, n, red, tid, c, S1, S2, N);
+    if (tid == 0) moments_store(mom + ((size_t)q * 2 + ch) * 3, c, S1, S2, N);
   }
 }
 
@@ -237,6 +249,30 @@
   int last;
 };
 
+template <typename E>
+__device__ __forceinline__ void argmin_rounds(const double* lv, int* lj, int L, int k, double* rv, int* rj, int tid, E&& emit, double& kv, int& kj) {
+  kv = 0.0; kj = -1;
+  for (int t = 0; t < k; t++) {
+    double cv = 0.0;
+    int cj = -1, cs = -1;
+    for (int s = tid; s < L; s += 256)
+      if (lj[s] >= 0 && (cj < 0 || cand_less(lv[s], lj[s], cv, cj))) { cv = lv[s]; cj = lj[s]; cs = s; }
+    rv[tid] = cv; rj[tid] = cj;
+    block_argmin(rv, rj, tid);
+    const double wv = rv[0];
+    const int wj = rj[0];
+    __syncthreads();
+    if (cs >= 0 && cj == wj) lj[cs] = -1;
+    if (tid == 0) emit(t, wv, wj);
+    kv = wv; kj = wj;
+    if (wj < 0) {
+      if (tid == 0) for (int u = t + 1; u < k; u++) emit(u, 0.0, -1);
+      break;
+    }
+    __syncthreads();
+  }
+}
+
 template <int CAP>
 __device__ __forceinline__ void select_row(const float* __restrict__ d_p, const float* __restrict__ d_i,
                                            const float* __restrict__ e_p, const float* __restrict__ e_i,
@@ -244,7 +280,7 @@
                                            int m, int n, const double* __restrict__ mom_all, int G,
                                            int q_row0, int db_row0, int mask_width, double p_weight,
                                            int k, int32_t* __restrict__ idx, float* __restrict__ score, int P,
-                                           double* __restrict__ score64, SelLds<CAP>& W) {
+                                           double* __restrict__ score64, SelLds<CAP>& W, bool have_st = false) {
   double* st = W.st;
   double* rv = W.rv;
   int* rj = W.rj;
@@ -256,7 +292,7 @@
   const int tid = threadIdx.x, q = blockIdx.x;
   const bool plain = (d_i == nullptr);
   const bool two = (e_p != nullptr);
-  if (!plain && tid < (two ? 4 : 2)) {
+  if (!plain && !have_st && tid < (two ? 4 : 2)) {
     double cn = 0.0, mean = 0.0, m2 = 0.0;
     for (int g = 0; g < G; g++) {
       const double* o = (tid < 2 ? mom_all : mom2_all) + (((size_t)g * m + q) * 2 + (tid & 1)) * 3;
@@ -468,24 +504,9 @@
     return;
   }
   if (L <= CAP) {
-    for (int t = 0; t < k; t++) {
-      double cv = 0.0;
-      int cj = -1, cs = -1;
-      for (int s = tid; s < L; s += 256)
-        if (lj[s] >= 0 && (cj < 0 || cand_less(lv[s], lj[s], cv, cj))) { cv = lv[s]; cj = lj[s]; cs = s; }
-      rv[tid] = cv; rj[tid] = cj;
-      block_argmin(rv, rj, tid);
-      const double wv = rv[0];
-      const int wj = rj[0];
-      __syncthreads();
-      if (cs >= 0 && cj == wj) lj[cs] = -1;
-      if (tid == 0) emit(t, wv, wj);
-      if (wj < 0) {
-        if (tid == 0) for (int u = t + 1; u < k; u++) emit(u, 0.0, -1);
-        break;
-      }
-      __syncthreads();
-    }
+    double kv;
+    int kj;
+    argmin_rounds(lv, lj, L, k, rv, rj, tid, emit, kv, kj);
     return;
   }
   double pv = -__builtin_inf(), bv = 0.0;
@@ -757,6 +778,199 @@
   select_row<CAP>(d_p, d_i, e_p, e_i, mom2_all, m, n, mom_all, G, q_row0, db_row0, mask_width, p_weight, k, idx, score, P, score64, L);
 }
 
+__device__ __forceinline__ void chan_first(double nb, double mb, double m2b, double& mean_o, double& sd_o) {
+  double cn = 0.0, mean = 0.0, m2 = 0.0;
+  if (!(nb <= 0.0)) {
+    const double tot = cn + nb, delta = mb - mean;
+    mean += delta * (nb / tot);
+    m2 += m2b + delta * delta * (cn * nb / tot);
+    cn = tot;
+  }
+  mean_o = mean;
+  sd_o = sqrt(m2 / (cn - 1.0));
+}
+
+template <int CAP>
+__global__ FS_BOUNDS void moments_select_kernel(const float* __restrict__ d_p, const float* __restrict__ d_i, int m, int n,
+                                                double* __restrict__ mom, int q_row0, int db_row0, int mask_width, double p_weight, int k,
+                                                int32_t* __restrict__ idx, float* __restrict__ score, double* __restrict__ score64,
+                                                int samp, int rank, unsigned long long* __restrict__ fell) {
+  __shared__ SelLds<CAP> W;
+  constexpr int SEG = CAP / 4;
+  const int tid = threadIdx.x, q = blockIdx.x, wave = tid >> 6;
+  const float* rp = d_p + (size_t)q * n;
+  const float* ri = d_i + (size_t)q * n;
+  const bool listed = n > CAP && !((reinterpret_cast<size_t>(rp) ^ reinterpret_cast<size_t>(ri)) & 15);
+  const int ig = q_row0 + q;
+  auto masked = [&](int j) {
+    int dij = ig - (db_row0 + j);
+    if (dij < 0) dij = -dij;
+    return dij < mask_width;
+  };
+  double cp, ci, S1p, S2p, Np, S1i, S2i, Ni;
+  float tp = __builtin_inff(), ti = __builtin_inff();
+  if (listed) {
+    float mnp = __builtin_inff(), mni = __builtin_inff();
+    for (int u = 0; u < samp; u++) {
+      const int j = tid + 256 * u;
+      const float vp = rp[j], vi = ri[j];
+      if (!masked(j)) { if (vp < mnp) mnp = vp; if (vi < mni) mni = vi; }
+    }
+    const int lane = tid & 63;
+    auto ranked = [&](float mine) -> float {
+      int before = 0;
+#pragma unroll
+      for (int u = 0; u < 64; u++) {
+        const float o = __builtin_bit_cast(float, __builtin_amdgcn_readlane(__builtin_bit_cast(int, mine), u));
+        before += (o < mine || (o == mine && u < lane)) ? 1 : 0;
+      }
+      const unsigned long long hit = __builtin_amdgcn_ballot_w64(mine < __builtin_inff() && before == rank - 1);
+      return hit ? __builtin_bit_cast(float, __builtin_amdgcn_readlane(__builtin_bit_cast(int, mine), __ffsll((long long)hit) - 1)) : __builtin_inff();
+    };
+    const float wtp = ranked(mnp), wti = ranked(mni);
+    float* sm = reinterpret_cast<float*>(W.rv);
+    if (lane == 0) { sm[2 * wave] = wtp; sm[2 * wave + 1] = wti; }
+    __syncthreads();
+    tp = ((sm[0] + sm[2]) + (sm[4] + sm[6])) * 0.25f; ti = ((sm[1] + sm[3]) + (sm[5] + sm[7])) * 0.25f;
+    __syncthreads();
+    const float fp = rp[0] == rp[0] ? rp[0] : 0.5f, fi = ri[0] == ri[0] ? ri[0] : 0.5f;
+    cp = moments_pivot(rp[0]); ci = moments_pivot(ri[0]);
+    double s1p = 0.0, s2p = 0.0, s1i = 0.0, s2i = 0.0;
+    int np = 0, ni = 0;
+    auto acc = [](bool valid, float v, float cf, double c, double& s1, double& s2, int& cnt) {
+      const bool ok = valid && v == v;
+      const double d = (double)(ok ? v : cf) - c;
+      s1 += d; s2 += d * d; cnt += __popcll(__builtin_amdgcn_ballot_w64(ok));
+    };
+    int wcnt = 0;
+    float* lpair = reinterpret_cast<float*>(W.lv) + 2 * wave * SEG;
+    int* lidx = W.lj + wave * SEG;
+    auto step = [&](bool valid, float vp, float vi, int j) {
+      acc(valid, vp, fp, cp, s1p, s2p, np); acc(valid, vi, fi, ci, s1i, s2i, ni);
+      const bool in = valid && (vp <= tp || vi <= ti);
+      const unsigned long long mk = __builtin_amdgcn_ballot_w64(valid && vp <= tp) | __builtin_amdgcn_ballot_w64(valid && vi <= ti);
+      if (mk) {
+        if (in) {
+          const int slot = wcnt + (int)__builtin_amdgcn_mbcnt_hi((unsigned)(mk >> 32), __builtin_amdgcn_mbcnt_lo((unsigned)mk, 0u));
+          if (slot < SEG) { lpair[2 * slot] = vp; lpair[2 * slot + 1] = vi; lidx[slot] = j; }
+        }
+        wcnt += __popcll(mk);
+      }
+    };
+    int head = (int)((4 - ((reinterpret_cast<size_t>(rp) >> 2) & 3)) & 3);
+    const int nv = (n - head) >> 2;
+    const f32x4* rp4 = reinterpret_cast<const f32x4*>(rp + head);
+    const f32x4* ri4 = reinterpret_cast<const f32x4*>(ri + head);
+    if (head > 0) { const bool v = tid < head; step(v, v ? rp[tid] : 0.f, v ? ri[tid] : 0.f, tid); }
+    auto four = [&](bool v, const f32x4& a, const f32x4& b, int j) {
+      const int j0 = head + 4 * j;
+#pragma unroll
+      for (int e = 0; e < 4; e++) step(v, a[e], b[e], j0 + e);
+    };
+    int jb = 0;
+    const int rounds = nv >> 10;
+    if (rounds > 0) {
+      struct Round { f32x4 a0, a1, a2, a3, b0, b1, b2, b3; };
+      auto load = [&](Round& R, int j) {
+        R.a0 = rp4[j]; R.a1 = rp4[j + 256]; R.a2 = rp4[j + 512]; R.a3 = rp4[j + 768];
+        R.b0 = ri4[j]; R.b1 = ri4[j + 256]; R.b2 = ri4[j + 512]; R.b3 = ri4[j + 768];
+      };
+      auto work = [&](const Round& R, int j) {
+        four(true, R.a0, R.b0, j); four(true, R.a1, R.b1, j + 256); four(true, R.a2, R.b2, j + 512); four(true, R.a3, R.b3, j + 768);
+      };
+      Round A, B;
+      int j = tid, r = 0;
+      load(A, j);
+      for (;;) {
+        const bool mb = r + 1 < rounds;
+        load(B, mb ? j + 1024 : j);
+        work(A, j);
+        r++; j += 1024;
+        if (!mb) break;
+        const bool ma = r + 1 < rounds;
+        load(A, ma ? j + 1024 : j);
+        work(B, j);
+        r++; j += 1024;
+        if (!ma) break;
+      }
+      jb = rounds << 10;
+    }
+    const f32x4 z4 = {0.f, 0.f, 0.f, 0.f};
+    for (; jb < nv; jb += 256) {
+      const int j = jb + tid;
+      const bool v = j < nv;
+      const f32x4 a = v ? rp4[j] : z4, b = v ? ri4[j] : z4;
+      four(v, a, b, j);
+    }
+    for (int t0 = head + 4 * nv; t0 < n; t0 += 256) {
+      const int t = t0 + tid;
+      const bool v = t < n;
+      step(v, v ? rp[t] : 0.f, v ? ri[t] : 0.f, t);
+    }
+    if ((tid & 63) == 0) W.ctl[wave] = wcnt;
+    const bool first = (tid & 63) == 0;
+    S1p = block_sum(s1p, W.rv, tid); S2p = block_sum(s2p, W.rv, tid); Np = block_sum(first ? (double)np : 0.0, W.rv, tid);
+    S1i = block_sum(s1i, W.rv, tid); S2i = block_sum(s2i, W.rv, tid); Ni = block_sum(first ? (double)ni : 0.0, W.rv, tid);
+  } else {
+    moments_channel(rp, n, W.rv, tid, cp, S1p, S2p, Np);
+    moments_channel(ri, n, W.rv, tid, ci, S1i, S2i, Ni);
+  }
+  if (tid == 0) {
+    moments_store(mom + (size_t)q * 6, cp, S1p, S2p, Np);
+    moments_store(mom + (size_t)q * 6 + 3, ci, S1i, S2i, Ni);
+  }
+  if (tid < 2) {
+    const double c = tid ? ci : cp, S1 = tid ? S1i : S1p, S2 = tid ? S2i : S2p, N = tid ? Ni : Np;
+    double o[3];
+    moments_store(o, c, S1, S2, N);
+    chan_first(o[0], o[1], o[2], W.st[tid * 2], W.st[tid * 2 + 1]);
+  }
+  if (tid == 0) W.lcnt = 0;
+  __syncthreads();
+  auto emit = [&](int t, double v, int jg) {
+    idx[(size_t)q * k + t] = jg;
+    const float f32 = (jg >= 0) ? (float)v : __builtin_nanf("");
+    score[(size_t)q * k + t] = f32;
+    score64[(size_t)q * k + t] = (double)f32;
+  };
+  if (listed) {
+    const double mp = W.st[0], sp = W.st[1], mi = W.st[2], si = W.st[3];
+    const bool fastdiv = sp > 1e-290 && sp < 1e290 && si > 1e-290 && si < 1e290;
+    const int fill = max(max(W.ctl[0], W.ctl[1]), max(W.ctl[2], W.ctl[3]));
+    if (fastdiv && p_weight > 0.0 && fill <= SEG) {
+      const double rsp = 1.0 / sp, rsi = 1.0 / si;
+      auto F = [&](float vp, float vi) -> double { return p_weight * div_rn((double)vp - mp, sp, rsp) + div_rn((double)vi - mi, si, rsi); };
+      const double Fc = F(tp, ti);
+      const float* pairs = reinterpret_cast<const float*>(W.lv);
+      for (int u = 0; u < CAP / 256; u++) {
+        const int w = (u * 256) / SEG, o = u * 256 - w * SEG;
+        if (o >= W.ctl[w]) continue;
+        const int s = u * 256 + tid;
+        double f = 0.0;
+        int jg = -1;
+        if (o + tid < W.ctl[w]) {
+          const int j = W.lj[s];
+          const double fs = F(pairs[2 * s], pairs[2 * s + 1]);
+          if (fs < Fc && !masked(j)) { f = fs; jg = db_row0 + j; }
+        }
+        __syncthreads();
+        if (jg >= 0) {
+          const int slot = atomicAdd(&W.lcnt, 1);
+          W.lv[slot] = f; W.lj[slot] = jg;
+        }
+      }
+      __syncthreads();
+      double kv;
+      int kj;
+      argmin_rounds(W.lv, W.lj, W.lcnt, k, W.rv, W.rj, tid, emit, kv, kj);
+      if (kj >= 0 && kv < Fc) return;
+      __syncthreads();
+    }
+  }
+  if (n > CAP && tid == 0 && fell) atomicAdd(fell, 1ull);
+  select_row<CAP>(d_p, d_i, nullptr, nullptr, nullptr, m, n, nullptr, 1, q_row0, db_row0, mask_width, p_weight, k, idx, score, 1, score64, W, true);
+}
+
 }
 
 int select_slices(int m, int n) {
@@ -780,6 +994,32 @@
     return;
   }
   hipLaunchKernelGGL(row_moments_kernel, dim3(m), dim3(256), 0, st, d_p, d_i, n, mom);
+}
+
+static bool wave_form(int m, int n, int k) {
+  static const bool wave_rows = !(getenv("PR_SELECT_WAVE") && atoi(getenv("PR_SELECT_WAVE")) == 0);
+  static const int wave_max_n = getenv("PR_SELECT_WAVE_N") ? atoi(getenv("PR_SELECT_WAVE_N")) : 32768;
+  return wave_rows && n <= wave_max_n && k <= 16 && m >= 64;
+}
+
+void launch_moments_select(hipStream_t st, const float* d_p, const float* d_i, int m, int n, double* mom, int q_row0, int db_row0,
+                           int mask_width, double p_weight, int k, int32_t* idx, float* score, double* score64, void* scratch,
+                           unsigned long long* fell) {
+  if (m <= 0) return;
+  static const bool fused = !(getenv("PR_SELECT_FUSED") && atoi(getenv("PR_SELECT_FUSED")) == 0);
+  if (!fused || k > 16 || (scratch ? select_slices(m, n) : 1) > 1 || wave_form(m, n, k)) {
+    launch_row_moments(st, d_p, d_i, m, n, mom, scratch);
+    launch_fuse_select(st, d_p, d_i, m, n, mom, 1, q_row0, db_row0, mask_width, p_weight, k, idx, score, nullptr, nullptr, nullptr, scratch, score64);
+    return;
+  }
+  constexpr double T = FS_CAP * 5.0 / 8.0;
+  int samp = 16;
+  while (samp > 1 && 128.0 * samp * T / n > 80.0) samp >>= 1;
+  const double D = 128.0 * samp * T / n;
+  int rank = (int)std::lround(samp > 1 ? 64.0 * (1.0 - std::exp(-D / 256.0)) : D / 4.0);
+  rank = rank < 1 ? 1 : (rank > 32 ? 32 : rank);
+  hipLaunchKernelGGL(moments_select_kernel<FS_CAP>, dim3(m), dim3(256), 0, st, d_p, d_i, m, n, mom, q_row0, db_row0, mask_width, p_weight, k, idx,
+                     score, score64, samp, rank, fell);
 }
 
 void launch_fuse_select(hipStream_t st, const float* d_p, const float* d_i, int m, int n, const double* mom_all,
@@ -800,9 +1040,7 @@
     hipLaunchKernelGGL(slice_merge_kernel, dim3(m), dim3(256), (size_t)N * 8, st, sidx, ssc, P, m, k, idx, score, score64);
     return;
   }
-  static const bool wave_rows = !(getenv("PR_SELECT_WAVE") && atoi(getenv("PR_SELECT_WAVE")) == 0);
-  static const int wave_max_n = getenv("PR_SELECT_WAVE_N") ? atoi(getenv("PR_SELECT_WAVE_N")) : 32768;
-  if (wave_rows && !e_p && n <= wave_max_n && k <= 16 && m >= 64) {
+  if (!e_p && wave_form(m, n, k)) {
     hipLaunchKernelGGL(fuse_select_wave_kernel, dim3((m + 3) / 4), dim3(256), 0, st, d_p, d_i, m, n, mom_all, G, q_row0, db_row0, mask_width,
                        p_weight, k, idx, score, score64);
     return;
diff --git a/so_dso_place_recognition_amd/csrc/kernels.hpp b/so_dso_place_recognition_amd/csrc/kernels.hpp
--- a/so_dso_place_recognition_amd/csrc/kernels.hpp
+++ b/so_dso_place_recognition_amd/csrc/kernels.hpp
@@ -90,6 +90,8 @@
                         int G, int q_row0, int db_row0, int mask_width, double p_weight, int k, int32_t* idx,
                         float* score, const float* e_p = nullptr, const float* e_i = nullptr, const double* mom2_all = nullptr, void* scratch = nullptr,
                         double* score64 = nullptr );
+void launch_moments_select(hipStream_t st, const float* d_p, const float* d_i, int m, int n, double* mom, int q_row0, int db_row0, int mask_width,
+                           double p_weight, int k, int32_t* idx, float* score, double* score64, void* scratch, unsigned long long* fell);
 
 void launch_nan_fixup(hipStream_t st, float* d_p, float* d_i, int m, int n, const int* qbad, const int* dbad);
 void launch_rerank(hipStream_t st, const void* q_sc, const void* db_sc, int sc_dt, const void* q_m2, const void* db_m2, int m2_dt,
diff --git a/so_dso_place_recognition_amd/csrc/pr_api.cpp b/so_dso_place_recognition_amd/csrc/pr_api.cpp
--- a/so_dso_place_recognition_amd/csrc/pr_api.cpp
+++ b/so_dso_place_recognition_amd/csrc/pr_api.cpp
@@ -29,6 +29,7 @@
   hipEvent_t ev_b = nullptr;
   char* sc_scratch = nullptr;
   void* sel_scratch = nullptr;
+  unsigned long long* d_sel_fell = nullptr;
   double* rr_scratch = nullptr;
   size_t rr_cap = 0;
   hipEvent_t ev_fork = nullptr, ev_join = nullptr;
@@ -230,6 +231,8 @@
     TRY(hipEventCreateWithFlags(&ctx->ev_join, hipEventDisableTiming));
     for (auto& e : ctx->ev_m2) TRY(hipEventCreateWithFlags(&e, hipEventDisableTiming));
     TRY(hipMalloc(&ctx->sel_scratch, pr::select_scratch_bytes()));
+    TRY(hipMalloc((void**)&ctx->d_sel_fell, sizeof(unsigned long long)));
+    TRY(hipMemset(ctx->d_sel_fell, 0, sizeof(unsigned long long)));
     TRY(hipMalloc((void**)&ctx->d_flags, 8 * sizeof(int)));
     TRY(hipMemset(ctx->d_flags, 0, 8 * sizeof(int)));
     TRY(hipMalloc((void**)&ctx->d_svd_rows, (1 + pr::M2DP_SVD_ROWS_CAP) * sizeof(int)));
@@ -347,6 +350,7 @@
   if (ctx->xqspec) (void)hipFree(ctx->xqspec);
   if (ctx->xpart) (void)hipFree(ctx->xpart);
   if (ctx->sel_scratch) (void)hipFree(ctx->sel_scratch);
+  if (ctx->d_sel_fell) (void)hipFree(ctx->d_sel_fell);
   if (ctx->ev_fork) (void)hipEventDestroy(ctx->ev_fork);
   if (ctx->ev_join) (void)hipEventDestroy(ctx->ev_join);
   for (auto& e : ctx->ev_m2) if (e) (void)hipEventDestroy(e);
@@ -844,6 +848,26 @@
   return fuse_select_impl(ctx, d_p, d_i, m, n, mom_all, G, q_row0, db_row0, mask_width, p_weight, k, idx, score, score64);
 }
 
+int pr_moments_select_f64_dev(pr_ctx* ctx, const float* d_p, const float* d_i, int32_t m, int32_t n, double* mom, int32_t q_row0,
+                              int32_t db_row0, int32_t mask_width, double p_weight, int32_t k, int32_t* idx, float* score, double* score64) {
+  if (!ctx || !d_p || !d_i || !mom || !idx || !score || !score64 || m < 0 || n < 1 || k < 1) return PR_EINVAL;
+  if (int rc = set_device(ctx)) return rc;
+  pr::launch_moments_select(ctx->stream, d_p, d_i, m, n, mom, q_row0, db_row0, mask_width, p_weight, k, idx, score, score64, ctx->sel_scratch,
+                            ctx->d_sel_fell);
+  PR_HIP(ctx, hipGetLastError());
+  return PR_OK;
+}
+int pr_select_fallback_rows(pr_ctx* ctx, int64_t* rows) {
+  if (!ctx || !rows) return PR_EINVAL;
+  if (int rc = set_device(ctx)) return rc;
+  unsigned long long h = 0;
+  PR_HIP(ctx, hipMemcpyAsync(&h, ctx->d_sel_fell, sizeof h, hipMemcpyDeviceToHost, ctx->stream));
+  PR_HIP(ctx, hipMemsetAsync(ctx->d_sel_fell, 0, sizeof h, ctx->stream));
+  PR_HIP(ctx, hipStreamSynchronize(ctx->stream));
+  *rows = (int64_t)h;
+  return PR_OK;
+}
+
 static int fuse_select2_impl(pr_ctx* ctx, const float* d_p, const float* d_i, const float* e_p, const float* e_i, int32_t m, int32_t n,
                              const double* mom_all, const double* mom2_all, int32_t G, int32_t q_row0, int32_t db_row0,
                              int32_t mask_width, double p_weight, int32_t k, int32_t* idx, float* score, double* score64) {
@@ -1221,9 +1245,9 @@
       case DISTANCES:
         PR_HIP(ctx, dp.alloc((size_t)m * n * 4));
         if (type != PR_TYPE_DELIGHT) PR_HIP(ctx, di.alloc((size_t)m * n * 4));
+        if (type != PR_TYPE_DELIGHT) PR_HIP(ctx, mom.alloc((size_t)m * 6 * 8));
         return pr_distances_dev(ctx, sq.s, sdb.s, dp.as<float>(), di.as<float>());
     }
-    PR_HIP(ctx, mom.alloc((size_t)m * 6 * 8));
     return pr_row_moments_dev(ctx, dp.as<float>(), di.as<float>(), m, n, mom.as<double>());
   }
 };
@@ -1302,13 +1326,14 @@
   const int kin = rerank_width(k, ctx->sc_mode);
   const size_t o = (size_t)i0 * n;
   Desc &sc = T.t[0], &m2 = T.t[1], &one = sc.type >= 0 ? sc : m2;
-  int rc = sc.type >= 0 && m2.type >= 0
+  const bool both = sc.type >= 0 && m2.type >= 0;
+  int rc = both
       ? pr_fuse_select2_dev(ctx, sc.dp.as<float>() + o, sc.di.as<float>() + o, m2.dp.as<float>() + o, m2.di.as<float>() + o, len, n, T.mom(0, i0),
                             T.mom(1, i0), 1, q_row0, 0, mask_width, p_weight, kin, b.idx.as<int32_t>(), b.sc.as<float>())
-      : pr_fuse_select_dev(ctx, one.dp.as<float>() + o, one.di.as<float>() + o, len, n, one.mom.as<double>() + (size_t)i0 * 6, 1, q_row0, 0,
-                           mask_width, p_weight, kin, b.idx.as<int32_t>(), b.sc.as<float>());
+      : pr_moments_select_f64_dev(ctx, one.dp.as<float>() + o, one.di.as<float>() + o, len, n, one.mom.as<double>() + (size_t)i0 * 6, q_row0, 0,
+                                  mask_width, p_weight, kin, b.idx.as<int32_t>(), b.sc.as<float>(), b.sw.as<double>());
   if (rc) return rc;
-  if ((rc = pr_widen_scores_dev(ctx, b.sc.as<float>(), (int64_t)len * kin, b.sw.as<double>()))) return rc;
+  if (both && (rc = pr_widen_scores_dev(ctx, b.sc.as<float>(), (int64_t)len * kin, b.sw.as<double>()))) return rc;
   if ((rc = T.dev(pr_rerank_dev, ctx, i0, len, n, 1, q_row0, 0, mask_width, p_weight, kin, b.idx.as<int32_t>(), b.sw.as<double>(), k,
                   b.kidx.as<int32_t>(), b.ksc.as<double>())))
     return rc;
@@ -1343,7 +1368,11 @@
     for (int32_t r = 0; r < mf; r++) memcpy(rows[i].data() + (size_t)r * sig, T.t[i].hq + (size_t)F[r] * sig, sig * 8);
     Desc& d = R.add(T.t[i].type, rows[i].data(), nullptr);
     d.db = T.t[i].db;
-    for (int s = CREATE; s <= MOMENTS; s++)
+  }
+  const int last = (T.t[0].type >= 0 && T.t[1].type >= 0) ? MOMENTS : DISTANCES;
+  for (Desc& d : R.t) {
+    if (d.type < 0) continue;
+    for (int s = CREATE; s <= last; s++)
       if (int rc = d.step(ctx, s, mf, n)) return rc;
   }
   std::vector<int32_t> run_end;
@@ -1391,7 +1420,7 @@
   Types T;
   T.add(fused ? PR_TYPE_SC : type, a1, a2);
   if (fused) T.add(PR_TYPE_M2DP, b1, b2);
-  if (int rc = T.prepare(ctx, m, n, plain ? DISTANCES : MOMENTS)) return rc;
+  if (int rc = T.prepare(ctx, m, n, fused ? MOMENTS : DISTANCES)) return rc;
   if (plain) return plain_topk(ctx, T.t[0].dp.as<float>(), m, n, mask_width, p_weight, k, idx, score);
   TopkBufs top;
   if (int rc = top.alloc(ctx, m, rerank_width(k, ctx->sc_mode), k)) return rc;
diff --git a/so_dso_place_recognition_amd/csrc/pr_group.cpp b/so_dso_place_recognition_amd/csrc/pr_group.cpp
--- a/so_dso_place_recognition_amd/csrc/pr_group.cpp
+++ b/so_dso_place_recognition_amd/csrc/pr_group.cpp
@@ -378,16 +378,22 @@
     if (g->timing) G_HIP(g, hipEventRecord(sh.ph[PH_MATCH], sh.stream));
     G_PR(g, sh, pr_distances_dev(sh.ctx, sh.q, sh.db, sh.d_p, sh.d_i));
     if (g->timing) G_HIP(g, hipEventRecord(sh.ph[PH_MOMENTS], sh.stream));
-    G_PR(g, sh, pr_row_moments_dev(sh.ctx, sh.d_p, sh.d_i, m, sh.rows, sh.mom));
+    if (G > 1) G_PR(g, sh, pr_row_moments_dev(sh.ctx, sh.d_p, sh.d_i, m, sh.rows, sh.mom));
   }
   if (int rc = mark(PH_GATHER_A)) return rc;
   std::vector<const void*> src(G);
   std::vector<void*> dst(G);
   for (int r = 0; r < G; r++) { src[r] = g->s[r].mom; dst[r] = g->s[r].mom_all; }
-  if (int rc = exchange(g, src, dst, (size_t)m * 6 * 8)) return rc;
+  if (G > 1)
+    if (int rc = exchange(g, src, dst, (size_t)m * 6 * 8)) return rc;
   if (int rc = mark(PH_SELECT)) return rc;
   for (auto& sh : g->s) {
     G_HIP(g, hipSetDevice(sh.device));
+    if (G == 1) {
+      G_PR(g, sh, pr_moments_select_f64_dev(sh.ctx, sh.d_p, sh.d_i, m, sh.rows, sh.mom_all, 0, sh.row0, mask_width, p_weight, kin, sh.idx_in,
+                                            sh.sc32, sh.sc64));
+      continue;
+    }
     G_PR(g, sh, pr_fuse_select_dev(sh.ctx, sh.d_p, sh.d_i, m, sh.rows, sh.mom_all, G, 0, sh.row0, mask_width, p_weight, kin, sh.idx_in, sh.sc32));
     G_PR(g, sh, pr_widen_scores_dev(sh.ctx, sh.sc32, (int64_t)m * kin, sh.sc64));
   }
diff --git a/so_dso_place_recognition_amd/matcher.py b/so_dso_place_recognition_amd/matcher.py
--- a/so_dso_place_recognition_amd/matcher.py
+++ b/so_dso_place_recognition_amd/matcher.py
@@ -148,10 +148,15 @@
             self._twin, self._twin_of = tw, db
         return self._twin
 
-    def local_select(self, mom_all: torch.Tensor, G: int, mask_width, p_weight, k, db_row0, q_row0):
+    def local_select(self, mom_all: torch.Tensor, G: int, mask_width, p_weight, k, db_row0, q_row0, with_moments: bool = False):
         m, n = self._m, self.n
         stores = self.descs
-        if len(stores) == 1:
+        if with_moments:
+            assert G == 1 and len(stores) == 1 and not self.plain and mom_all.is_contiguous()
+            stores[0]._mom = mom_all
+            lib = self.lib
+            select = lambda h, d_p, d_i, m_, n_, mom, G_, *rest: lib.pr_moments_select_f64_dev(h, d_p, d_i, m_, n_, mom, *rest)
+        elif len(stores) == 1:
             stores[0]._mom = mom_all.contiguous()
             select = self.lib.pr_fuse_select_f64_dev
         else:
@@ -283,8 +288,9 @@
         resolve = ((self.exact_moments, self.exact_select, self.exact_merge, lambda: self._exact_passes(exact_order))
                    if (exact_order and not self.plain and not f16) else None)
         post = (lambda cand_sc, idx, score: self._margin(*self._moms(), self._args[0], p_weight, cand_sc, k, score)) if f16 else None
-        idx, score = sharded_topk(lambda: self.local_phase1(*queries),
-                                  lambda mom_all, G_: self.local_select(mom_all, G_, mask_width, p_weight, k, db_row0, q_row0),
+        one = G == 1 and not force_exchange and not self.plain and len(self.descs) == 1 and self.descs[0] is self
+        idx, score = sharded_topk((lambda: self.local_phase1(*queries, moments=False)) if one else (lambda: self.local_phase1(*queries)),
+                                  lambda mom_all, G_: self.local_select(mom_all, G_, mask_width, p_weight, k, db_row0, q_row0, with_moments=one),
                                   k, group if (G > 1 or force_exchange) else None, G, merge=self.merge, force_exchange=force_exchange,
                                   rerank=None if self.plain else self.local_rerank, finish=self.finish, post=post, resolve=resolve, mark=mark)
         if f16 and f16_fallback:
@@ -470,7 +476,7 @@
         self.n += k
         self.db_sig = self._raw[:self.n * self.rows_per_sig]
 
-    def local_phase1(self, queries: torch.Tensor):
+    def local_phase1(self, queries: torch.Tensor, moments: bool = True):
         self._enter()
         m = self._pack(self.q, queries)
         n = self.n
@@ -488,7 +494,8 @@
             self._leave()
             mom.zero_()
         else:
-            self.ctx.check(lib.pr_row_moments_dev(h, _dptr(d_p), _dptr(d_i), m, n, _dptr(mom)))
+            if moments:
+                self.ctx.check(lib.pr_row_moments_dev(h, _dptr(d_p), _dptr(d_i), m, n, _dptr(mom)))
             self._leave()
         return mom
 
```

Result: faster. 138,700 queries/s, median of 6 (+2.2%).
